# ACEfanatic02/par_raytracer

Hardware: AMD Instinct MI355X
Metric: Mrays/s at 1920x1080x8spp, 1M-tri OBJ (higher is better)
Workload: dtype f32; 1 GPU; C4: synthetic 1,002,528-triangle terrain OBJ (1,024 groups), 1920x1080, 8 spp, bounce_depth 2; seed=1234, triangles=1002528, width=1920, height=1080, spp=8, bounce_depth=2, rays_per_frame=77049910, parallelism=pixel rows sharded in 8-row blocks over 1 GPU(s), pipeline=pool, frames_in_flight=1

## Files before the change

include/prt.h:

```cpp
#ifndef PRT_H_
#define PRT_H_

#include <stddef.h>
#include <stdint.h>

#ifdef __cplusplus
extern "C" {
#endif

#define PRT_ABI_VERSION 5
enum { PRT_ERR_ARGUMENT = -1, PRT_ERR_NO_SCENE = -2, PRT_ERR_HIP = -10, PRT_ERR_IN_FLIGHT = -11, PRT_ERR_EXCEPTION = -12 };


typedef struct prt_material {
    float specular_intensity;
    float index_of_refraction;
    float alpha;
    float ambient_color[4];
    float diffuse_color[4];
    float specular_color[4];
    int32_t ambient_texture;
    int32_t diffuse_texture;
    int32_t specular_texture;
    int32_t alpha_texture;
// ... 180 lines not shown
                                const float * positions, uint32_t position_count, const prt_closest_grads * gout,
                                const prt_point_grads * gin, prt_grad_info * info);
int prt_closest_points_backward_device(prt_ctx * ctx, const prt_point_batch * batch, const int32_t * group, const uint32_t * vertex0,
                                       const float * positions, uint32_t position_count, const prt_closest_grads * gout,
                                       const prt_point_grads * gin, prt_grad_info * info);

typedef struct prt_signed_buffers {
    prt_closest_buffers closest;
    float * signed_dist;
    uint8_t * feature;
} prt_signed_buffers;
int prt_signed_distance(prt_ctx * ctx, const prt_point_batch * batch, const prt_signed_buffers * out, uint32_t flags,
                        prt_counters * counters);
int prt_signed_distance_device(prt_ctx * ctx, const prt_point_batch * batch, const prt_signed_buffers * out, uint32_t flags,
                               prt_counters * counters);

typedef struct prt_sample_request { uint64_t seed; uint64_t first; uint32_t count; } prt_sample_request;
typedef struct prt_sample_buffers {
    float * point;
    float * bw;
    float * normal;
    uint32_t * vertex0;
    int32_t * group;
} prt_sample_buffers;
typedef struct prt_sample_info { double device_ms; double table_ms; double area; uint64_t total_weight;
                                 int32_t unit_exponent; uint32_t live_triangles; } prt_sample_info;
int prt_sample_surface(prt_ctx * ctx, const prt_sample_request * request, const prt_sample_buffers * out, prt_sample_info * info);
int prt_sample_surface_device(prt_ctx * ctx, const prt_sample_request * request, const prt_sample_buffers * out, prt_sample_info * info);

typedef struct prt_sample_grads { const float * point; const float * normal; } prt_sample_grads;
int prt_sample_surface_backward(prt_ctx * ctx, uint32_t count, const int32_t * group, const uint32_t * vertex0, const float * bw,
                                const float * positions, uint32_t position_count, const prt_sample_grads * gout, float * gin_positions,
                                prt_grad_info * info);
int prt_sample_surface_backward_device(prt_ctx * ctx, uint32_t count, const int32_t * group, const uint32_t * vertex0, const float * bw,
                                       const float * positions, uint32_t position_count, const prt_sample_grads * gout, float * gin_positions,
                                       prt_grad_info * info);

typedef struct prt_hemi_batch {
    const float * points;
    const float * normals;
    const float * max_dist;
    uint32_t count;
    uint32_t samples;
    uint64_t seed;
    uint64_t first;
    float ray_bias;
} prt_hemi_batch;
typedef struct prt_hemi_buffers {
    uint32_t * unoccluded;
    float * visibility;
    float * bent;
} prt_hemi_buffers;
int prt_hemisphere_visibility(prt_ctx * ctx, const prt_hemi_batch * batch, const prt_hemi_buffers * out, uint32_t flags,
                              prt_counters * counters);
int prt_hemisphere_visibility_device(prt_ctx * ctx, const prt_hemi_batch * batch, const prt_hemi_buffers * out, uint32_t flags,
                                     prt_counters * counters);

typedef struct prt_multi prt_multi;
prt_multi * prt_multi_create(const int * device_ids, int n_dev);
void prt_multi_destroy(prt_multi * m);
const char * prt_multi_last_error(const prt_multi * m);
int prt_multi_device_count(const prt_multi * m);
int prt_multi_depth(const prt_multi * m);
prt_ctx * prt_multi_context(prt_multi * m, int i);
int prt_multi_upload_scene(prt_multi * m, const prt_scene_desc * scene);
int prt_multi_update_geometry(prt_multi * m, const prt_geometry_update * update);
int prt_multi_render(prt_multi * m, const prt_camera * cam, const prt_params * params, uint32_t width, uint32_t height,
                     float * rgba_out, prt_counters * counters);
int prt_multi_submit(prt_multi * m, const prt_camera * cam, const prt_params * params, uint32_t width, uint32_t height,
                     float * rgba_out, uint64_t * ticket);
int prt_multi_wait(prt_multi * m, uint64_t ticket, prt_counters * counters);

typedef struct prt_scene_info {
    uint32_t triangle_count;
    uint32_t bvh_node_count;
    uint32_t bvh_max_depth;
    uint32_t bvh_node_bytes;
    uint32_t tri_record_bytes;
    uint32_t shade_record_bytes;
    uint64_t device_bytes;
    double bvh_build_ms;
} prt_scene_info;
int prt_get_scene_info(const prt_ctx * ctx, prt_scene_info * info);

typedef struct prt_render_stats {
    uint64_t node_visits, tri_tests;
    uint64_t wave_node_steps, wave_tri_steps, wave_leaf_visits, wave_refills;
    uint64_t deepest_stack;
    uint64_t phase_cycles[5];
    uint64_t parked_rays, parked_shadow_rays;
    uint64_t elided_shadow_rays;
    uint64_t variance_close_calls;
    uint32_t stack_lds_entries, stack_bound;
} prt_render_stats;
int prt_get_render_stats(const prt_ctx * ctx, prt_render_stats * stats);

enum {
    PRT_REGION_ROUND = 0,
    PRT_REGION_TOPUP,
    PRT_REGION_TOPUP_PASS,
    PRT_REGION_TRACE_OUTER,
    PRT_REGION_REFILL,
    PRT_REGION_WALK_PASS,
    PRT_REGION_NODE_STEP,
    PRT_REGION_NODE_DESCEND,
    PRT_REGION_NODE_POP,
    PRT_REGION_NODE_PUSH,
    PRT_REGION_LEAF,
    PRT_REGION_TRI,
    PRT_REGION_FINISH,
    PRT_REGION_PARK,
    PRT_REGION_SHADE_PASS,
    PRT_REGION_SHADE_HIT,
    PRT_REGION_SHADE_MISS,
    PRT_REGION_RADIANCE_STORE,
    PRT_REGION_SHADOW_BLOCK,
    PRT_REGION_SHADOW_EMIT,
    PRT_REGION_WALK_LOOP,
    PRT_REGION_WALK_NEXT_CHILD,
    PRT_REGION_WALK_ENTER,
    PRT_REGION_WALK_RETURN_UP,
    PRT_REGION_FRAME_SAVE,
    PRT_REGION_FRAME_LOAD,
    PRT_REGION_WALK_CHILD_RAY,
    PRT_REGION_OUTPUTS,
    PRT_REGION_WAVE,
    PRT_REGION_LEAF_RAY,
    PRT_REGION_COUNT
};
int prt_get_region_stats(const prt_ctx * ctx, uint64_t * out, uint32_t n);

int prt_debug_check_bvh(const prt_scene_desc * scene, uint64_t * out);
int prt_debug_check_bvh_lbvh(prt_ctx * ctx, const prt_scene_desc * scene, uint64_t * out);
int prt_debug_lbvh_tree(prt_ctx * ctx, uint32_t n_tris, const float * verts9, int32_t * left, int32_t * right, uint32_t * first,
                        uint32_t * last, float * node_box, float * leaf_box, uint32_t * sorted_ids, uint64_t * sorted_keys);
int prt_debug_check_refit(prt_ctx * ctx, const prt_scene_desc * moved_scene, uint64_t * out);

int prt_debug_device_kat(prt_ctx * ctx, int kind, const void * in, size_t in_bytes, void * out, size_t out_bytes,
                         uint32_t n, const prt_camera * cam);

int prt_debug_throw(prt_ctx * ctx, int kind);

#ifdef __cplusplus
}
#endif
#endif
```

par_raytracer_amd/api.py:

```python
from __future__ import annotations

import ctypes as C
from typing import Optional, Sequence, Tuple

import numpy as np

from . import capi
from .capi import PrtCamera, PrtCounters, PrtParams, PrtSceneDesc, PrtGradInfo, PrtSceneInfo, PrtUpdateInfo


class HostScene:

    def __init__(self, directory: str, obj_name: str = "sponza.obj", light_mode: int = 0,
                 camera_position: Sequence[float] = (0.0, 0.0, 0.0)):
        lib = capi.host_lib()
        cp = (C.c_float * 3)(*[float(v) for v in camera_position])
        self._lib = lib
        self._h = lib.prt_host_load_obj(directory.encode(), obj_name.encode(), int(light_mode), cp)
        if not self._h:
            raise RuntimeError("prt_host_load_obj failed: %s" % lib.prt_host_last_error().decode())

    @property
    def handle(self):
        return self._h
# ... 112 lines not shown

        d.positions = ptr("positions", C.c_float); d.position_count = a["positions"].size // 3
        d.normals = ptr("normals", C.c_float); d.normal_count = a["normals"].size // 3
        d.texcoords = ptr("texcoords", C.c_float); d.texcoord_count = a["texcoords"].size // 2
        d.tangents = ptr("tangents", C.c_float)
        d.idx_positions = ptr("idx_positions", C.c_uint32)
        d.idx_texcoords = ptr("idx_texcoords", C.c_uint32)
        d.idx_normals = ptr("idx_normals", C.c_uint32)
        d.index_count = a["idx_positions"].size
        d.groups = ptr("groups", capi.PrtGroup); d.group_count = a["groups"].size // C.sizeof(capi.PrtGroup)
        d.materials = ptr("materials", capi.PrtMaterial); d.material_count = a["materials"].size // C.sizeof(capi.PrtMaterial)
        d.lights = ptr("lights", capi.PrtLight); d.light_count = a["lights"].size // C.sizeof(capi.PrtLight)
        d.spheres = ptr("spheres", capi.PrtBSphere); d.sphere_count = a["spheres"].size // C.sizeof(capi.PrtBSphere)
        d.sphere_group = ptr("sphere_group", C.c_int32)
        dims = a["texture_dims"].reshape(-1, 3)
        self._tex = (capi.PrtTexture * max(1, len(dims)))()
        off = 0
        base = a["texture_bytes"].ctypes.data
        for i, (sx, sy, ch) in enumerate(dims):
            self._tex[i].size_x, self._tex[i].size_y, self._tex[i].channels = int(sx), int(sy), int(ch)
            self._tex[i].texels = C.cast(base + off, C.POINTER(C.c_uint8))
            off += int(sx) * int(sy) * int(ch)
        d.textures = C.cast(self._tex, C.POINTER(capi.PrtTexture)) if len(dims) else C.cast(None, C.POINTER(capi.PrtTexture))
        d.texture_count = len(dims)
        self._desc = d

    @property
    def desc(self):
        return C.pointer(self._desc)


def make_camera(fov: float, width: int, height: int, position: Sequence[float], facing: Sequence[float]) -> PrtCamera:
    cam = PrtCamera()
    p = (C.c_float * 3)(*[float(v) for v in position])
    f = (C.c_float * 3)(*[float(v) for v in facing])
    capi.host_lib().prt_host_make_camera(float(fov), int(width), int(height), p, f, C.byref(cam))
    return cam


def default_params(spp: int, seed: int = 1234, bounce_depth: Optional[int] = None, reflection_samples: Optional[int] = None,
                   spec_samples: Optional[int] = None, pipeline: int = 0, max_spp: int = 0,
                   variance_threshold: float = 0.0) -> PrtParams:
    p = PrtParams()
    capi.host_lib().prt_host_default_params(int(spp), int(seed), C.byref(p))
    if bounce_depth is not None:
        p.bounce_depth = int(bounce_depth)
    if reflection_samples is not None:
        p.reflection_samples = int(reflection_samples)
    if spec_samples is not None:
        p.spec_samples = int(spec_samples)
    p.pipeline = int(pipeline)
    p.max_spp = int(max_spp)
    p.variance_threshold = float(variance_threshold)
    return p


class Renderer:

    def __init__(self, device_id: int = 0):
        lib = capi.hip_lib()
        self._lib = lib
        self._ctx = lib.prt_create(int(device_id))
        if not self._ctx:
            raise RuntimeError("prt_create(%d) failed: %s" % (device_id, lib.prt_last_error(None).decode()))
        self.device_id = device_id

    def _check(self, rc: int, what: str):
        if rc != 0:
            raise RuntimeError("%s failed (%d): %s" % (what, rc, self._lib.prt_last_error(self._ctx).decode()))

    def set_option(self, name: str, value=None) -> None:
        v = None if value is None else str(value).encode()
        self._check(self._lib.prt_set_option(self._ctx, name.encode(), v), "prt_set_option(%s)" % name)

    def upload(self, scene) -> PrtSceneInfo:
        desc = scene.desc if isinstance(scene, (HostScene, FlatDesc)) else scene
        self._check(self._lib.prt_upload_scene(self._ctx, desc), "prt_upload_scene")
        return self.scene_info()

    def scene_info(self) -> PrtSceneInfo:
        info = PrtSceneInfo()
        self._check(self._lib.prt_get_scene_info(self._ctx, C.byref(info)), "prt_get_scene_info")
        return info

    def render_stats(self) -> "capi.PrtRenderStats":
        st = capi.PrtRenderStats()
        self._check(self._lib.prt_get_render_stats(self._ctx, C.byref(st)), "prt_get_render_stats")
        return st

    def region_stats(self) -> dict:
        n = 2 * len(capi.REGION_NAMES)
        out = (C.c_uint64 * n)()
        got = self._lib.prt_get_region_stats(self._ctx, out, n)
        if got != n:
            raise RuntimeError("prt_get_region_stats: the library has %d words, capi.REGION_NAMES %d" % (got, n))
        return {name: (int(out[2 * k]), int(out[2 * k + 1])) for k, name in enumerate(capi.REGION_NAMES)}

    def render(self, cam: PrtCamera, params: PrtParams, width: int, height: int, start_idx: int = 0,
               end_idx: Optional[int] = None) -> Tuple[np.ndarray, PrtCounters]:
        if end_idx is None:
            end_idx = width * height
        out = np.empty((end_idx - start_idx, 4), dtype=np.float32)
        counters = PrtCounters()
        self._check(self._lib.prt_render(self._ctx, C.byref(cam), C.byref(params), width, height, start_idx, end_idx,
                                         out.ctypes.data_as(C.c_void_p), C.byref(counters)), "prt_render")
        return out, counters

    def render_pixels(self, cam: PrtCamera, params: PrtParams, width: int, height: int, pixel_ids) -> Tuple[np.ndarray, PrtCounters]:
        ids = np.ascontiguousarray(pixel_ids, dtype=np.uint32).reshape(-1)
        out = np.empty((ids.size, 4), dtype=np.float32)
        counters = PrtCounters()
        self._check(self._lib.prt_render_pixel_list(self._ctx, C.byref(cam), C.byref(params), width, height,
                                                    ids.ctypes.data_as(C.c_void_p), ids.size,
                                                    out.ctypes.data_as(C.c_void_p), C.byref(counters)), "prt_render_pixel_list")
        return out, counters

    def render_lattice(self, cam, params, width: int, height: int, lattice: int) -> Tuple[np.ndarray, PrtCounters]:
        xs = np.arange(0, width, lattice, dtype=np.uint32)
        ys = np.arange(0, height, lattice, dtype=np.uint32)
        ids = (ys[:, None] * np.uint32(width) + xs[None, :]).reshape(-1)
        out, ctr = self.render_pixels(cam, params, width, height, ids)
        return out.reshape(len(ys), len(xs), 4), ctr

    def render_device(self, cam, params, width, height, start_idx, end_idx, d_ptr: int,
                      want_counters: bool = True) -> Optional[PrtCounters]:
        counters = PrtCounters() if want_counters else None
        self._check(self._lib.prt_render_device(self._ctx, C.byref(cam), C.byref(params), width, height, start_idx,
                                                end_idx, C.c_void_p(d_ptr),
                                                C.byref(counters) if want_counters else None), "prt_render_device")
        return counters

    def shard_rows(self, height: int, block_rows: int, rank: int, nranks: int) -> int:
        return int(self._lib.prt_shard_rows(height, block_rows, rank, nranks))

    def render_shard_device(self, cam, params, width, height, block_rows, rank, nranks, d_ptr: int,
                            want_counters: bool = True) -> Optional[PrtCounters]:
        counters = PrtCounters() if want_counters else None
        self._check(self._lib.prt_render_shard_device(self._ctx, C.byref(cam), C.byref(params), width, height,
                                                      block_rows, rank, nranks, C.c_void_p(d_ptr),
                                                      C.byref(counters) if want_counters else None),
                    "prt_render_shard_device")
        return counters

    def render_shard(self, cam, params, width, height, block_rows, rank, nranks) -> Tuple[np.ndarray, PrtCounters]:
        rows = self.shard_rows(height, block_rows, rank, nranks)
        out = np.empty((rows, width, 4), dtype=np.float32)
        counters = PrtCounters()
        self._check(self._lib.prt_render_shard(self._ctx, C.byref(cam), C.byref(params), width, height, block_rows,
                                               rank, nranks, out.ctypes.data_as(C.c_void_p), C.byref(counters)),
                    "prt_render_shard")
        return out, counters

    def device_kat(self, kind: int, records: np.ndarray, out_shape, out_dtype, cam: Optional[PrtCamera] = None) -> np.ndarray:
        rec = np.ascontiguousarray(records)
        out = np.zeros(out_shape, dtype=out_dtype)
        self._check(self._lib.prt_debug_device_kat(self._ctx, int(kind), rec.ctypes.data_as(C.c_void_p), rec.nbytes,
                                                   out.ctypes.data_as(C.c_void_p), out.nbytes, rec.shape[0],
                                                   C.byref(cam) if cam is not None else None), "prt_debug_device_kat")
        return out

    def _arrays(self, first):
        def fits(got, shape):
            return len(got) == len(shape) and all(s is None or s == g for g, s in zip(got, shape))

        def shown(shape):
            return "(%s)" % ", ".join("n" if s is None else str(s) for s in shape) if None in shape else str(shape)
# ... 352 lines not shown
```

par_raytracer_amd/capi.py:

```python
from __future__ import annotations

import ctypes as C
import os
from typing import Optional

import numpy as np

PKG_DIR = os.path.dirname(os.path.abspath(__file__))
REPO_ROOT = os.path.dirname(PKG_DIR)

c_float3 = C.c_float * 3
c_float4 = C.c_float * 4


class PrtMaterial(C.Structure):
    _fields_ = [("specular_intensity", C.c_float), ("index_of_refraction", C.c_float), ("alpha", C.c_float),
                ("ambient_color", c_float4), ("diffuse_color", c_float4), ("specular_color", c_float4),
                ("ambient_texture", C.c_int32), ("diffuse_texture", C.c_int32), ("specular_texture", C.c_int32),
                ("alpha_texture", C.c_int32), ("bump_texture", C.c_int32)]


class PrtLight(C.Structure):
    _fields_ = [("type", C.c_int32), ("color", c_float4), ("position", c_float3), ("facing", c_float3),
                ("falloff", C.c_float)]


class PrtGroup(C.Structure):
    _fields_ = [("first_index", C.c_uint32), ("index_count", C.c_uint32), ("material", C.c_int32)]


class PrtBSphere(C.Structure):
    _fields_ = [("center", c_float3), ("radius", C.c_float), ("c0", C.c_uint32), ("c1", C.c_uint32)]


class PrtTexture(C.Structure):
    _fields_ = [("size_x", C.c_uint32), ("size_y", C.c_uint32), ("channels", C.c_uint32),
                ("texels", C.POINTER(C.c_uint8))]


class PrtSceneDesc(C.Structure):
    _fields_ = [("positions", C.POINTER(C.c_float)), ("position_count", C.c_uint32),
                ("normals", C.POINTER(C.c_float)), ("normal_count", C.c_uint32),
                ("texcoords", C.POINTER(C.c_float)), ("texcoord_count", C.c_uint32),
                ("tangents", C.POINTER(C.c_float)),
                ("idx_positions", C.POINTER(C.c_uint32)), ("idx_texcoords", C.POINTER(C.c_uint32)),
                ("idx_normals", C.POINTER(C.c_uint32)), ("index_count", C.c_uint32),
                ("groups", C.POINTER(PrtGroup)), ("group_count", C.c_uint32),
                ("materials", C.POINTER(PrtMaterial)), ("material_count", C.c_uint32),
                ("textures", C.POINTER(PrtTexture)), ("texture_count", C.c_uint32),
                ("lights", C.POINTER(PrtLight)), ("light_count", C.c_uint32),
                ("spheres", C.POINTER(PrtBSphere)), ("sphere_group", C.POINTER(C.c_int32)),
                ("sphere_count", C.c_uint32)]


class PrtCamera(C.Structure):
    _fields_ = [("tan_a2", C.c_float), ("aspect", C.c_float), ("inv_width", C.c_float), ("inv_height", C.c_float),
                ("position", c_float3), ("forward", c_float3), ("right", c_float3), ("up", c_float3)]


class PrtParams(C.Structure):
    _fields_ = [("ray_bias", C.c_float), ("reflection_samples", C.c_uint32), ("spec_samples", C.c_uint32),
                ("bounce_depth", C.c_uint32), ("background_color", c_float4), ("spp", C.c_uint32),
                ("pipeline", C.c_uint32), ("seed", C.c_uint64), ("max_spp", C.c_uint32), ("variance_threshold", C.c_float)]


class PrtCounters(C.Structure):
    _fields_ = [("ray_count", C.c_uint64), ("node_visits", C.c_uint64), ("tri_tests", C.c_uint64),
                ("shaded_hits", C.c_uint64), ("render_ms", C.c_double), ("trace_kernel_ms", C.c_double),
                ("trace_kernel_launches", C.c_uint32), ("pipeline", C.c_uint32)]

    def as_dict(self):
        return {n: getattr(self, n) for n, _ in self._fields_}


class PrtSceneInfo(C.Structure):
    _fields_ = [("triangle_count", C.c_uint32), ("bvh_node_count", C.c_uint32), ("bvh_max_depth", C.c_uint32),
                ("bvh_node_bytes", C.c_uint32), ("tri_record_bytes", C.c_uint32), ("shade_record_bytes", C.c_uint32),
                ("device_bytes", C.c_uint64), ("bvh_build_ms", C.c_double)]

    def as_dict(self):
        return {n: getattr(self, n) for n, _ in self._fields_}


class PrtRenderStats(C.Structure):
    _fields_ = [("node_visits", C.c_uint64), ("tri_tests", C.c_uint64), ("wave_node_steps", C.c_uint64),
                ("wave_tri_steps", C.c_uint64), ("wave_leaf_visits", C.c_uint64), ("wave_refills", C.c_uint64),
                ("deepest_stack", C.c_uint64), ("phase_cycles", C.c_uint64 * 5), ("parked_rays", C.c_uint64),
                ("parked_shadow_rays", C.c_uint64), ("elided_shadow_rays", C.c_uint64), ("variance_close_calls", C.c_uint64), ("stack_lds_entries", C.c_uint32), ("stack_bound", C.c_uint32)]


class PrtRayBatch(C.Structure):
    _fields_ = [("origins", C.c_void_p), ("directions", C.c_void_p), ("tmax", C.c_void_p), ("count", C.c_uint32),
                ("ray_bias", C.c_float)]


class PrtHitBuffers(C.Structure):
    _fields_ = [("t", C.c_void_p), ("bw", C.c_void_p), ("vertex0", C.c_void_p), ("group", C.c_void_p),
                ("position", C.c_void_p), ("normal", C.c_void_p), ("occluded", C.c_void_p)]


class PrtPointBatch(C.Structure):
    _fields_ = [("points", C.c_void_p), ("max_dist2", C.c_void_p), ("count", C.c_uint32)]


class PrtClosestBuffers(C.Structure):
    _fields_ = [("dist2", C.c_void_p), ("point", C.c_void_p), ("bw", C.c_void_p), ("vertex0", C.c_void_p), ("group", C.c_void_p)]


class PrtSignedBuffers(C.Structure):
    _fields_ = [("closest", PrtClosestBuffers), ("signed_dist", C.c_void_p), ("feature", C.c_void_p)]


class PrtGeometryUpdate(C.Structure):
    _fields_ = [("positions", C.c_void_p), ("position_count", C.c_uint32), ("normals", C.c_void_p), ("normal_count", C.c_uint32),
                ("tangents", C.c_void_p), ("spheres", C.POINTER(PrtBSphere)), ("sphere_group", C.POINTER(C.c_int32)),
                ("sphere_count", C.c_uint32)]


class PrtUpdateInfo(C.Structure):
    _fields_ = [("device_ms", C.c_double), ("levels", C.c_uint32), ("node_count", C.c_uint32), ("abs_max", C.c_float)]

    def as_dict(self):
        return {n: getattr(self, n) for n, _ in self._fields_}


class PrtHitGrads(C.Structure):
    _fields_ = [("t", C.c_void_p), ("bw", C.c_void_p), ("position", C.c_void_p), ("normal", C.c_void_p)]


class PrtQueryGrads(C.Structure):
    _fields_ = [("positions", C.c_void_p), ("origins", C.c_void_p), ("directions", C.c_void_p)]


class PrtClosestGrads(C.Structure):
    _fields_ = [("dist2", C.c_void_p), ("point", C.c_void_p), ("bw", C.c_void_p)]


class PrtPointGrads(C.Structure):
    _fields_ = [("positions", C.c_void_p), ("points", C.c_void_p)]


class PrtGradInfo(C.Structure):
    _fields_ = [("device_ms", C.c_double), ("hit_rays", C.c_uint32), ("skipped_rays", C.c_uint32), ("unit_exponent", C.c_int32),
                ("max_contribution", C.c_float)]

    def as_dict(self):
        return {n: getattr(self, n) for n, _ in self._fields_}


class PrtSampleRequest(C.Structure):
    _fields_ = [("seed", C.c_uint64), ("first", C.c_uint64), ("count", C.c_uint32)]


class PrtSampleBuffers(C.Structure):
    _fields_ = [("point", C.c_void_p), ("bw", C.c_void_p), ("normal", C.c_void_p), ("vertex0", C.c_void_p), ("group", C.c_void_p)]


class PrtSampleInfo(C.Structure):
    _fields_ = [("device_ms", C.c_double), ("table_ms", C.c_double), ("area", C.c_double), ("total_weight", C.c_uint64),
                ("unit_exponent", C.c_int32), ("live_triangles", C.c_uint32)]

    def as_dict(self):
        return {n: getattr(self, n) for n, _ in self._fields_}


class PrtSampleGrads(C.Structure):
    _fields_ = [("point", C.c_void_p), ("normal", C.c_void_p)]


class PrtHemiBatch(C.Structure):
    _fields_ = [("points", C.c_void_p), ("normals", C.c_void_p), ("max_dist", C.c_void_p), ("count", C.c_uint32), ("samples", C.c_uint32),
                ("seed", C.c_uint64), ("first", C.c_uint64), ("ray_bias", C.c_float)]


class PrtHemiBuffers(C.Structure):
    _fields_ = [("unoccluded", C.c_void_p), ("visibility", C.c_void_p), ("bent", C.c_void_p)]


QUERY_CLOSEST, QUERY_OCCLUDED = 0, 1
PIPELINE_DEFAULT, PIPELINE_MEGAKERNEL, PIPELINE_WAVEFRONT, PIPELINE_PERSISTENT, PIPELINE_POOL = 0, 1, 2, 3, 4
FLAG_COUNT_VISITS = 0x100
FLAG_TRYOUT = 0x200
BUILD_EXPERIMENTAL, BUILD_BVH4 = 1, 2

PRT_SYMBOLS = ["prt_create", "prt_destroy", "prt_last_error", "prt_abi_version", "prt_set_option", "prt_build_flags", "prt_upload_scene", "prt_render",
               "prt_render_device", "prt_shard_rows", "prt_render_shard_device", "prt_render_shard", "prt_render_pixel_list", "prt_get_scene_info", "prt_get_render_stats", "prt_debug_check_bvh", "prt_debug_check_bvh_lbvh", "prt_debug_lbvh_tree", "prt_debug_device_kat",
               "prt_multi_create", "prt_multi_destroy", "prt_multi_last_error", "prt_multi_device_count", "prt_multi_context",
               "prt_multi_upload_scene", "prt_multi_render", "prt_multi_depth", "prt_multi_submit", "prt_multi_wait", "prt_debug_throw",
               "prt_trace_rays", "prt_trace_rays_device", "prt_get_region_stats",
               "prt_update_geometry", "prt_update_geometry_device", "prt_multi_update_geometry", "prt_debug_check_refit",
               "prt_trace_rays_backward", "prt_trace_rays_backward_device",
               "prt_closest_points", "prt_closest_points_device",
               "prt_closest_points_backward", "prt_closest_points_backward_device",
               "prt_signed_distance", "prt_signed_distance_device",
               "prt_sample_surface", "prt_sample_surface_device",
               "prt_sample_surface_backward", "prt_sample_surface_backward_device",
               "prt_hemisphere_visibility", "prt_hemisphere_visibility_device"]
REGION_NAMES = ["round", "topup", "topup_pass", "trace_outer", "refill", "walk_pass", "node_step", "node_descend", "node_pop", "node_push", "leaf",
                "tri", "finish", "park", "shade_pass", "shade_hit", "shade_miss", "radiance_store", "shadow_block", "shadow_emit", "walk_loop",
                "walk_next_child", "walk_enter", "walk_return_up", "frame_save", "frame_load", "walk_child_ray", "outputs", "wave", "leaf_ray"]
PRT_HOST_SYMBOLS = ["prt_host_load_obj", "prt_host_free_scene", "prt_host_scene_desc", "prt_host_scene_hierarchy_seconds",
                    "prt_host_scene_parse_seconds", "prt_host_last_error", "prt_host_make_camera",
                    "prt_host_default_params", "prt_host_render", "prt_host_render_error", "prt_host_write_image", "prt_host_tonemap",
                    "prt_host_load_texture", "prt_host_free_texture", "prt_host_debug_throw"]


class LibraryMissing(RuntimeError):
    pass


def _load(path: str, what: str) -> C.CDLL:
    if not os.path.exists(path):
        raise LibraryMissing("%s not built: %s is missing.  Run `make` (or __graft_entry__.build()) at the repo root; "
                             "there is no fallback implementation." % (what, path))
    return C.CDLL(path, mode=C.RTLD_GLOBAL)


_hip: Optional[C.CDLL] = None
_host: Optional[C.CDLL] = None


def hip_lib() -> C.CDLL:
    global _hip
    if _hip is None:
        lib = _load(os.path.join(PKG_DIR, os.path.basename(os.environ.get("PRT_HIP_LIB", "libprt_hip.so"))), "HIP extension")
        lib.prt_create.restype = C.c_void_p
        lib.prt_create.argtypes = [C.c_int]
        lib.prt_destroy.argtypes = [C.c_void_p]
        lib.prt_last_error.restype = C.c_char_p
        lib.prt_last_error.argtypes = [C.c_void_p]
        lib.prt_abi_version.restype = C.c_int
        lib.prt_build_flags.restype = C.c_int
        lib.prt_set_option.argtypes = [C.c_void_p, C.c_char_p, C.c_char_p]
        lib.prt_upload_scene.argtypes = [C.c_void_p, C.POINTER(PrtSceneDesc)]
        lib.prt_render.argtypes = [C.c_void_p, C.POINTER(PrtCamera), C.POINTER(PrtParams), C.c_uint32, C.c_uint32,
                                   C.c_uint32, C.c_uint32, C.c_void_p, C.POINTER(PrtCounters)]
        lib.prt_render_device.argtypes = [C.c_void_p, C.POINTER(PrtCamera), C.POINTER(PrtParams), C.c_uint32, C.c_uint32,
                                          C.c_uint32, C.c_uint32, C.c_void_p, C.POINTER(PrtCounters)]
        lib.prt_shard_rows.restype = C.c_uint32
        lib.prt_shard_rows.argtypes = [C.c_uint32] * 4
        lib.prt_render_shard_device.argtypes = [C.c_void_p, C.POINTER(PrtCamera), C.POINTER(PrtParams), C.c_uint32,
                                                C.c_uint32, C.c_uint32, C.c_uint32, C.c_uint32, C.c_void_p,
                                                C.POINTER(PrtCounters)]
        lib.prt_render_shard.argtypes = lib.prt_render_shard_device.argtypes
        lib.prt_render_pixel_list.argtypes = [C.c_void_p, C.POINTER(PrtCamera), C.POINTER(PrtParams), C.c_uint32, C.c_uint32,
                                              C.c_void_p, C.c_uint32, C.c_void_p, C.POINTER(PrtCounters)]
        lib.prt_get_scene_info.argtypes = [C.c_void_p, C.POINTER(PrtSceneInfo)]
        lib.prt_get_render_stats.argtypes = [C.c_void_p, C.POINTER(PrtRenderStats)]
        if hasattr(lib, "prt_get_region_stats"):
            lib.prt_get_region_stats.argtypes = [C.c_void_p, C.POINTER(C.c_uint64), C.c_uint32]
        lib.prt_debug_check_bvh.argtypes = [C.POINTER(PrtSceneDesc), C.POINTER(C.c_uint64)]
        lib.prt_debug_check_bvh_lbvh.argtypes = [C.c_void_p, C.POINTER(PrtSceneDesc), C.POINTER(C.c_uint64)]
        if hasattr(lib, "prt_debug_lbvh_tree"):
            lib.prt_debug_lbvh_tree.argtypes = [C.c_void_p, C.c_uint32] + [C.c_void_p] * 9
        lib.prt_debug_device_kat.argtypes = [C.c_void_p, C.c_int, C.c_void_p, C.c_size_t, C.c_void_p, C.c_size_t, C.c_uint32,
                                             C.POINTER(PrtCamera)]
        lib.prt_multi_create.restype = C.c_void_p
        lib.prt_multi_create.argtypes = [C.POINTER(C.c_int), C.c_int]
        lib.prt_multi_destroy.argtypes = [C.c_void_p]
        lib.prt_multi_last_error.restype = C.c_char_p
        lib.prt_multi_last_error.argtypes = [C.c_void_p]
        lib.prt_multi_device_count.argtypes = [C.c_void_p]
        lib.prt_multi_context.restype = C.c_void_p
        lib.prt_multi_context.argtypes = [C.c_void_p, C.c_int]
        lib.prt_multi_upload_scene.argtypes = [C.c_void_p, C.POINTER(PrtSceneDesc)]
        lib.prt_multi_render.argtypes = [C.c_void_p, C.POINTER(PrtCamera), C.POINTER(PrtParams), C.c_uint32, C.c_uint32,
                                         C.c_void_p, C.POINTER(PrtCounters)]
        lib.prt_multi_depth.argtypes = [C.c_void_p]
        lib.prt_multi_submit.argtypes = [C.c_void_p, C.POINTER(PrtCamera), C.POINTER(PrtParams), C.c_uint32, C.c_uint32,
                                         C.c_void_p, C.POINTER(C.c_uint64)]
        lib.prt_multi_wait.argtypes = [C.c_void_p, C.c_uint64, C.POINTER(PrtCounters)]
        lib.prt_debug_throw.argtypes = [C.c_void_p, C.c_int]
        lib.prt_trace_rays.argtypes = [C.c_void_p, C.c_int, C.POINTER(PrtRayBatch), C.POINTER(PrtHitBuffers), C.c_uint32,
                                       C.POINTER(PrtCounters)]
        lib.prt_trace_rays_device.argtypes = lib.prt_trace_rays.argtypes
        if hasattr(lib, "prt_update_geometry"):
            lib.prt_update_geometry.argtypes = [C.c_void_p, C.POINTER(PrtGeometryUpdate), C.POINTER(PrtUpdateInfo)]
            lib.prt_update_geometry_device.argtypes = lib.prt_update_geometry.argtypes
            lib.prt_multi_update_geometry.argtypes = [C.c_void_p, C.POINTER(PrtGeometryUpdate)]
            lib.prt_debug_check_refit.argtypes = [C.c_void_p, C.POINTER(PrtSceneDesc), C.POINTER(C.c_uint64)]
        if hasattr(lib, "prt_trace_rays_backward"):
            lib.prt_trace_rays_backward.argtypes = [C.c_void_p, C.POINTER(PrtRayBatch), C.c_void_p, C.c_void_p, C.c_void_p, C.c_uint32,
                                                    C.POINTER(PrtHitGrads), C.POINTER(PrtQueryGrads), C.POINTER(PrtGradInfo)]
            lib.prt_trace_rays_backward_device.argtypes = lib.prt_trace_rays_backward.argtypes
        if hasattr(lib, "prt_closest_points"):
            lib.prt_closest_points.argtypes = [C.c_void_p, C.POINTER(PrtPointBatch), C.POINTER(PrtClosestBuffers), C.c_uint32,
                                               C.POINTER(PrtCounters)]
            lib.prt_closest_points_device.argtypes = lib.prt_closest_points.argtypes
        if hasattr(lib, "prt_closest_points_backward"):
            lib.prt_closest_points_backward.argtypes = [C.c_void_p, C.POINTER(PrtPointBatch), C.c_void_p, C.c_void_p, C.c_void_p, C.c_uint32,
                                                        C.POINTER(PrtClosestGrads), C.POINTER(PrtPointGrads), C.POINTER(PrtGradInfo)]
            lib.prt_closest_points_backward_device.argtypes = lib.prt_closest_points_backward.argtypes
        if hasattr(lib, "prt_signed_distance"):
            lib.prt_signed_distance.argtypes = [C.c_void_p, C.POINTER(PrtPointBatch), C.POINTER(PrtSignedBuffers), C.c_uint32,
                                                C.POINTER(PrtCounters)]
            lib.prt_signed_distance_device.argtypes = lib.prt_signed_distance.argtypes
        if hasattr(lib, "prt_sample_surface"):
            lib.prt_sample_surface.argtypes = [C.c_void_p, C.POINTER(PrtSampleRequest), C.POINTER(PrtSampleBuffers), C.POINTER(PrtSampleInfo)]
            lib.prt_sample_surface_device.argtypes = lib.prt_sample_surface.argtypes
            lib.prt_sample_surface_backward.argtypes = [C.c_void_p, C.c_uint32, C.c_void_p, C.c_void_p, C.c_void_p, C.c_void_p, C.c_uint32,
                                                        C.POINTER(PrtSampleGrads), C.c_void_p, C.POINTER(PrtGradInfo)]
            lib.prt_sample_surface_backward_device.argtypes = lib.prt_sample_surface_backward.argtypes
        if hasattr(lib, "prt_hemisphere_visibility"):
            lib.prt_hemisphere_visibility.argtypes = [C.c_void_p, C.POINTER(PrtHemiBatch), C.POINTER(PrtHemiBuffers), C.c_uint32,
                                                      C.POINTER(PrtCounters)]
            lib.prt_hemisphere_visibility_device.argtypes = lib.prt_hemisphere_visibility.argtypes
        _hip = lib
    return _hip


def host_lib() -> C.CDLL:
    global _host
    if _host is None:
        hip_lib()
        lib = _load(os.path.join(PKG_DIR, "libprt_host.so"), "host library")
        lib.prt_host_load_obj.restype = C.c_void_p
        lib.prt_host_load_obj.argtypes = [C.c_char_p, C.c_char_p, C.c_int, C.POINTER(C.c_float)]
        lib.prt_host_free_scene.argtypes = [C.c_void_p]
        lib.prt_host_scene_desc.restype = C.POINTER(PrtSceneDesc)
        lib.prt_host_scene_desc.argtypes = [C.c_void_p]
        lib.prt_host_scene_hierarchy_seconds.restype = C.c_double
        lib.prt_host_scene_hierarchy_seconds.argtypes = [C.c_void_p]
        lib.prt_host_scene_parse_seconds.restype = C.c_double
        lib.prt_host_scene_parse_seconds.argtypes = [C.c_void_p]
        lib.prt_host_last_error.restype = C.c_char_p
        lib.prt_host_make_camera.argtypes = [C.c_float, C.c_uint32, C.c_uint32, C.POINTER(C.c_float), C.POINTER(C.c_float),
                                             C.POINTER(PrtCamera)]
        lib.prt_host_default_params.argtypes = [C.c_uint32, C.c_uint64, C.POINTER(PrtParams)]
        lib.prt_host_render.argtypes = [C.c_void_p, C.POINTER(PrtCamera), C.POINTER(PrtParams), C.c_uint32, C.c_uint32,
                                        C.c_int, C.c_void_p, C.POINTER(PrtCounters)]
        lib.prt_host_render_error.restype = C.c_char_p
# ... 17 lines not shown
```

par_raytracer_amd/csrc/bvh_build.cpp:

```cpp
#include "bvh_build.h"
#include "prt_options.h"

#include <algorithm>
#include <atomic>
#include <cfloat>
#include <cmath>
#include <cstdlib>
#include <cstring>
#include <chrono>
#include <cstdio>
#include <stdexcept>
#include <thread>

namespace prt {
namespace {

struct Box {
    float lo[3], hi[3];
    void reset() { for (int a = 0; a < 3; ++a) { lo[a] = FLT_MAX; hi[a] = -FLT_MAX; } }
    void grow(const Box & b) { for (int a = 0; a < 3; ++a) { lo[a] = std::min(lo[a], b.lo[a]); hi[a] = std::max(hi[a], b.hi[a]); } }
    void grow(const float * p) { for (int a = 0; a < 3; ++a) { lo[a] = std::min(lo[a], p[a]); hi[a] = std::max(hi[a], p[a]); } }
    float half_area() const {
        float dx = hi[0] - lo[0], dy = hi[1] - lo[1], dz = hi[2] - lo[2];
        if (dx < 0.0f) return 0.0f;
// ... 406 lines not shown
                } else if (used) {
                    imask |= 1u << s;
                }
                for (int a = 0; a < 3; ++a) {
                    d[8 + 2 * a + (s >> 2)] |= qlo[a] << (8 * (s & 3u));
                    d[14 + 2 * a + (s >> 2)] |= qhi[a] << (8 * (s & 3u));
                }
            } else {
                for (int a = 0; a < 3; ++a) {
                    d[4 + a] |= qlo[a] << (8 * s);
                    d[7 + a] |= qhi[a] << (8 * s);
                }
                if (!used) d[10 + s] = (uint32_t)~(int32_t)(n_tris << 2);
                else if (leaf) d[10 + s] = (uint32_t)~(int32_t)((b.pool[w.kid[s]].first << 2) | (b.pool[w.kid[s]].count - 1));
                else d[10 + s] = next_child++;
            }
        }
        if (eight) {
            d[3] = g.ebyte[0] << 23 | imask | lmask << 8;
            d[4] = w.child_base;
            d[5] = w.tri_base;
            d[6] = g.ebyte[1] << 23 | c0 | c1 << 8;
            d[7] = g.ebyte[2] << 23 | w.axis;
        } else {
            d[3] = g.ebyte[0] << 23;
            d[14] = g.ebyte[1] << 23;
            d[15] = g.ebyte[2] << 23;
        }
    }
    out->node_count = n_nodes;
    out->max_depth = max_depth;
    out->stack_bound = eight ? max_depth + 2 : 3 * max_depth + 2;
    if (b.opt.debug) fprintf(stderr, "[prt] BVH back end (collapse to %d-wide, quantise, reorder): %.1f ms\n", width, std::chrono::duration<double, std::milli>(std::chrono::steady_clock::now() - t0).count());
}

void build_sah_binary(Builder & b, const float * verts, uint32_t n_tris, uint32_t leaf_max, uint32_t threads, float trav_cost,
                      float * scene_lo, float * scene_hi) {
    if (leaf_max < 1) leaf_max = 1;
    if (leaf_max > 4) leaf_max = 4;
    b.leaf_max = leaf_max;
    b.trav_cost = trav_cost;
    b.prims.resize(n_tris);
    Box scene;
    scene.reset();
    for (uint32_t i = 0; i < n_tris; ++i) {
        Prim & p = b.prims[i];
        p.box.reset();
        p.box.grow(verts + 9 * (size_t)i);
        p.box.grow(verts + 9 * (size_t)i + 3);
        p.box.grow(verts + 9 * (size_t)i + 6);
        for (int a = 0; a < 3; ++a) p.c[a] = 0.5f * p.box.lo[a] + 0.5f * p.box.hi[a];
        p.id = i;
        scene.grow(p.box);
    }
    for (int a = 0; a < 3; ++a) { scene_lo[a] = n_tris ? scene.lo[a] : 0.0f; scene_hi[a] = n_tris ? scene.hi[a] : 0.0f; }
    b.pool.resize(n_tris ? 2 * (size_t)n_tris : 1);
    b.next_node = 1;
    b.max_depth = 0;
    b.threads_free = (int)(threads > 1 ? threads - 1 : 0);
    const auto t_build = std::chrono::steady_clock::now();
    if (n_tris) {
        b.build(0, 0, n_tris, 0);
    } else {
        TmpNode & n = b.pool[0];
        n.box.reset();
        for (int a = 0; a < 3; ++a) n.box.lo[a] = n.box.hi[a] = 0.0f;
        n.left = n.right = -1;
        n.first = 0;
        n.count = 1;
        n.depth = 0;
    }
    if (b.opt.debug) fprintf(stderr, "[prt] binned-SAH binary build, %u triangles, %u threads: %.1f ms\n", n_tris, threads, std::chrono::duration<double, std::milli>(std::chrono::steady_clock::now() - t_build).count());
}

}

void build_bvh_wide(int width, const float * verts, uint32_t n_tris, uint32_t leaf_max, uint32_t threads, BvhWide * out, float trav_cost,
                    const BvhBuildOptions * opt) {
    *out = BvhWide();
    Builder b;
    b.configure(opt);
    build_sah_binary(b, verts, n_tris, leaf_max, threads, trav_cost, out->scene_lo, out->scene_hi);
    finish_wide(b, n_tris, width, out);
}

namespace {
void radix_tree_to_binary(Builder & b, uint32_t n_tris, uint32_t leaf_max, const int32_t * left, const int32_t * right,
                          const uint32_t * first, const uint32_t * last, const float * node_box, const float * leaf_box,
                          const uint32_t * sorted_ids, float * scene_lo, float * scene_hi) {
    if (leaf_max < 1) leaf_max = 1;
    if (leaf_max > 4) leaf_max = 4;
    b.leaf_max = leaf_max;
    b.prims.resize(n_tris);
    Box scene;
    scene.reset();
    for (uint32_t i = 0; i < n_tris; ++i) {
        Prim & p = b.prims[i];
        for (int a = 0; a < 3; ++a) { p.box.lo[a] = leaf_box[6 * (size_t)i + a]; p.box.hi[a] = leaf_box[6 * (size_t)i + 3 + a]; p.c[a] = 0.0f; }
        p.id = sorted_ids[i];
        scene.grow(p.box);
    }
    for (int a = 0; a < 3; ++a) { scene_lo[a] = n_tris ? scene.lo[a] : 0.0f; scene_hi[a] = n_tris ? scene.hi[a] : 0.0f; }
    b.pool.resize(n_tris ? 2 * (size_t)n_tris : 1);
    b.next_node = 1;
    b.max_depth = 0;
    b.threads_free = 0;
    auto make_leaf = [&](TmpNode & n, const Box & box, uint32_t f, uint32_t c, uint32_t depth) {
        n.box = box; n.left = n.right = -1; n.first = f; n.count = c; n.depth = depth;
    };
    if (n_tris == 0) {
        Box zero = { { 0, 0, 0 }, { 0, 0, 0 } };
        make_leaf(b.pool[0], zero, 0, 1, 0);
    } else if (n_tris <= leaf_max || n_tris == 1) {
        make_leaf(b.pool[0], scene, 0, n_tris, 0);
    } else if (b.opt.lbvh_plain) {
        struct Todo { uint32_t tmp; int32_t src; uint32_t depth; };
        std::vector<Todo> todo;
        todo.push_back(Todo{ 0u, 0, 0u });
        while (!todo.empty()) {
            const Todo t = todo.back();
            todo.pop_back();
            TmpNode & n = b.pool[t.tmp];
            if (t.src < 0) {
                const uint32_t pos = (uint32_t)~t.src;
                make_leaf(n, b.prims[pos].box, pos, 1, t.depth);
                continue;
            }
            Box box;
            for (int a = 0; a < 3; ++a) { box.lo[a] = node_box[6 * (size_t)t.src + a]; box.hi[a] = node_box[6 * (size_t)t.src + 3 + a]; }
            const uint32_t cnt = last[t.src] - first[t.src] + 1u;
            if (cnt <= leaf_max) { make_leaf(n, box, first[t.src], cnt, t.depth); continue; }
            n.box = box;
            n.depth = t.depth;
            n.first = n.count = 0;
            const uint32_t l = b.alloc(), r = b.alloc();
            n.left = (int32_t)l;
            n.right = (int32_t)r;
            todo.push_back(Todo{ l, left[t.src], t.depth + 1 });
            todo.push_back(Todo{ r, right[t.src], t.depth + 1 });
        }
    } else {
        uint32_t cluster_max = 64;
        if (b.opt.lbvh_cluster >= 0) cluster_max = (uint32_t)std::max(4ll, std::min(1ll << 20, b.opt.lbvh_cluster));
        for (uint32_t i = 0; i < n_tris; ++i)
            for (int a = 0; a < 3; ++a) b.prims[i].c[a] = 0.5f * b.prims[i].box.lo[a] + 0.5f * b.prims[i].box.hi[a];
        struct Cluster { Box box; float c[3]; uint32_t first, count; };
        std::vector<Cluster> clusters;
        {
            std::vector<int32_t> stack;
            stack.push_back(0);
            while (!stack.empty()) {
                const int32_t src = stack.back();
                stack.pop_back();
                Cluster c;
                if (src < 0) {
                    const uint32_t pos = (uint32_t)~src;
                    c.box = b.prims[pos].box; c.first = pos; c.count = 1;
                } else {
                    const uint32_t cnt = last[src] - first[src] + 1u;
                    if (cnt > cluster_max) { stack.push_back(right[src]); stack.push_back(left[src]); continue; }
                    for (int a = 0; a < 3; ++a) { c.box.lo[a] = node_box[6 * (size_t)src + a]; c.box.hi[a] = node_box[6 * (size_t)src + 3 + a]; }
                    c.first = first[src]; c.count = cnt;
                }
                for (int a = 0; a < 3; ++a) c.c[a] = 0.5f * c.box.lo[a] + 0.5f * c.box.hi[a];
                clusters.push_back(c);
            }
// ... 101 lines not shown
```

par_raytracer_amd/csrc/bvh_build.h:

```cpp
#pragma once

#include <cstdint>
#include <vector>

namespace prt { struct BvhBuildOptions; }

namespace prt {

struct BvhWide {
    std::vector<uint32_t> nodes;
    std::vector<uint32_t> tri_order;
    uint32_t node_dwords = 0;
    uint32_t node_count = 0;
    uint32_t max_depth = 0;
    uint32_t stack_bound = 0;
    float scene_lo[3] = { 0, 0, 0 }, scene_hi[3] = { 0, 0, 0 };
};
enum { BVH4_NODE_DWORDS = 16, BVH8_NODE_DWORDS = 20 };

typedef BvhWide Bvh4Result;

typedef BvhWide Bvh8Result;

void build_bvh_wide(int width, const float * verts, uint32_t n_tris, uint32_t leaf_max, uint32_t threads, BvhWide * out,
                    float trav_cost = 1.0f, const BvhBuildOptions * opt = nullptr);

void build_bvh_wide_from_radix_tree(int width, uint32_t n_tris, uint32_t leaf_max, const int32_t * left, const int32_t * right,
                                    const uint32_t * first, const uint32_t * last, const float * node_box, const float * leaf_box,
                                    const uint32_t * sorted_ids, BvhWide * out, const BvhBuildOptions * opt = nullptr);

const char * validate_bvh_links(const BvhWide & bvh, uint32_t n_tris);

void check_bvh_wide(const float * verts, uint32_t n_tris, const BvhWide & bvh, uint64_t * out);

}
```

par_raytracer_amd/csrc/dev_scene.h:

```cpp
#pragma once

#include "../../include/prt.h"
#include "dev_math.h"

namespace prt {

struct DevMaterial {
    float ambient[3];
    float specular_intensity;
    float diffuse[3];
    float index_of_refraction;
    float specular[3];
    float alpha;
    int flags;
    unsigned int tex[3];
};

enum { DEV_TEX_NONE = 0xFFFFu };

struct DevTexture {
    unsigned int first_texel;
    unsigned int size_x, size_y;
    unsigned int pad;
};

struct DevLight {
    float color[3];
    int type;
    float position[3];
    float falloff;
    float facing[3];
    float pad;
};

struct DevScene {
    const float4 * nodes;
    const float4 * tris;
    const float4 * shade;
    const unsigned int * tri_rank;
    const DevMaterial * materials;
    const DevLight * lights;
    const float4 * diffuse_dirs;
    const float4 * spec_dirs;
    unsigned int light_count;
    unsigned int material_count;
    unsigned int spec_samples;
    unsigned int tri_count;
    unsigned int node_count;
    const DevTexture * textures;
    const unsigned int * texels;
    const float * srgb_lut;
    const float4 * tri_uv;
    const float4 * tri_tan;
    const float4 * ref_spheres;
    unsigned int tie_widen_max;
    unsigned long long * near_tie_unresolved;
};

struct DevCamera {
    f3 position;
    f3 forward;
    f3 right_scaled;
    f3 up_scaled;
    float inv_width, inv_height;
};

struct DevParams {
    float ray_bias;
    unsigned int reflection_samples, spec_samples, bounce_depth;
    f3 background;
    unsigned int spp;
    unsigned long long seed;
    unsigned int width, height;
    float box_pad;
    unsigned int first_pixel, shard_block_rows, shard_rank, shard_nranks;
    const unsigned int * pixel_list;
    int * stack_spill;
    unsigned int stack_lds_entries, stack_spill_stride;
    int * exact_stack;
    unsigned int exact_stack_stride;
    unsigned int local_base;
    unsigned int tile_pixels;
    unsigned int work_reverse_n;
    unsigned int work_scatter_n, work_scatter_mul;
    unsigned int elide_dead_shadow_rays;
    unsigned int max_spp;
    float variance_threshold;
};

PRT_HD unsigned int local_of_work(unsigned int wi, unsigned int width, unsigned int tile_pixels, unsigned int reverse_n = 0u,
                                  unsigned int scatter_n = 0u, unsigned int scatter_mul = 1u) {
    if (reverse_n) wi = reverse_n - 1u - wi;
    if (wi >= tile_pixels) return wi;
    if (scatter_n) wi = (((wi >> 3) * scatter_mul) % scatter_n) * 8u + (wi & 7u);
    const unsigned int band_px = 8u * width;
    const unsigned int b = wi / band_px, q = wi - b * band_px;
    const unsigned int t = q >> 6, i = q & 63u;
    return b * band_px + (i >> 3) * width + t * 8u + (i & 7u);
}

PRT_HD unsigned int pixel_of_local(const DevParams & P, unsigned int lp) {
    lp += P.local_base;
    if (P.pixel_list) return P.pixel_list[lp];
    lp = local_of_work(lp, P.width, P.tile_pixels, P.work_reverse_n, P.work_scatter_n, P.work_scatter_mul);
    if (P.shard_nranks <= 1) return P.first_pixel + lp;
    const unsigned int row = lp / P.width, x = lp - row * P.width;
    const unsigned int blk = row / P.shard_block_rows, r = row - blk * P.shard_block_rows;
    const unsigned int y = (blk * P.shard_nranks + P.shard_rank) * P.shard_block_rows + r;
    return y * P.width + x;
}

struct DevCounters {
    unsigned long long ray_count;
    unsigned long long node_visits;
    unsigned long long tri_tests;
    unsigned long long shaded_hits;
// ... 48 lines not shown
```

par_raytracer_amd/csrc/dev_trace.h:

```cpp
#pragma once

#if defined(PRT_BVH8)
#include "dev_trace8.h"
#else
#include "dev_trace4.h"
#endif

namespace prt {

template <bool ANY_LENGTH, class STK>
PRT_D void trav_start(TravRay & r, f3 o, f3 d, int kind, float pad, const STK & stk) {
    if (ANY_LENGTH) {
        f3 w = (o + d) - o;
        if (w.x == 0.0f && w.y == 0.0f && w.z == 0.0f) w = d;
        float m = fmaxf(fmaxf(fabsf(w.x), fabsf(w.y)), fabsf(w.z));
        if (m < 9.5367431640625e-7f) {
            const int k = -ilogbf(m);
            w = mk3(ldexpf(w.x, k), ldexpf(w.y, k), ldexpf(w.z, k));
            m = ldexpf(m, k);
        }
        const float tiny = m * 9.094947017729282e-13f;
        if (fabsf(w.x) < tiny) w.x = copysignf(tiny, w.x);
        if (fabsf(w.y) < tiny) w.y = copysignf(tiny, w.y);
        if (fabsf(w.z) < tiny) w.z = copysignf(tiny, w.z);
        trav_init(r, o, w, kind, pad, stk);
        r.d = d;
        return;
    }
    trav_init(r, o, d, kind, pad, stk);
}

template <class STK, bool COUNT, bool ANY_LENGTH = false>
PRT_D HitRec resolve_near_ties(const DevScene & sc, f3 o, f3 d, float pad, float min_t, const STK & stk, TraceStats & st) {
    TravRay r;
    HitRec result = hit_miss();
    const f3 qp = o - (o + d);
    float bound = min_t * PRT_TIE_NEAR;
    for (unsigned int widen = 0; ; ++widen) {
        const bool last = widen >= sc.tie_widen_max;
        const float moat = bound * 1.00000095367431640625f;
        bool occupied = false;
        float best = 3.402823466e+38f;
        result.tri = -1;
        unsigned int next_rank = 0;
        RefSphereWalk walk;
        walk.reset();
        for (;;) {
            unsigned int c_rank = 0xFFFFFFFFu;
            int c_tri = -1;
            trav_start<ANY_LENGTH>(r, o, d, TRACE_CLOSEST, pad, stk);
            r.best.t = moat;
            for (;;) {
                while (trav_walking(r)) trav_node_step<STK, COUNT>(sc, r, stk, st, pad);
                if (trav_done(r)) break;
                unsigned int first, count;
                trav_leaf_range(r, first, count);
                for (unsigned int i = 0; i < count; ++i) {
                    const unsigned int ti = first + i;
                    const float4 * tp = sc.tris + 3 * (size_t)ti;
                    const float4 r0 = tp[0], r1 = tp[1], r2 = tp[2];
                    float t, dd, v, w;
                    if (!tri_geom(o, qp, mk3(r0.x, r0.y, r0.z), mk3(r0.w, r1.x, r1.y), mk3(r1.z, r1.w, r2.x), mk3(r2.y, r2.z, r2.w), t, dd, v, w)) continue;
                    const float th = t * (1.0f / dd);
                    if (th > bound) { if (th <= moat) occupied = true; continue; }
                    const unsigned int rk = sc.tri_rank[ti];
                    if (rk >= next_rank && rk < c_rank) { c_rank = rk; c_tri = (int)ti; }
                }
                trav_leaf_next(r, stk);
            }
            if (c_tri < 0 || (occupied && !last)) break;
            const float4 * tp = sc.tris + 3 * (size_t)c_tri;
            const float4 r0 = tp[0], r1 = tp[1], r2 = tp[2];
            float t, v, w;
            if (walk.offers(sc, o, d, c_rank, best) &&
                tri_test_ref(o, qp, mk3(r0.x, r0.y, r0.z), mk3(r0.w, r1.x, r1.y), mk3(r1.z, r1.w, r2.x), mk3(r2.y, r2.z, r2.w), best, t, v, w)) {
                best = t;
                result.t = t; result.v = v; result.w = w; result.tri = c_tri;
            }
            next_rank = c_rank + 1u;
        }
        if (!occupied) break;
        if (last) {
            if (sc.near_tie_unresolved) atomicAdd(sc.near_tie_unresolved, 1ull);
            break;
        }
        bound = moat * PRT_TIE_NEAR;
    }
    return result;
}

template <class STK, bool COUNT, bool ANY_LENGTH = false>
PRT_D HitRec trace_ray(const DevScene & sc, f3 o, f3 d, int kind, float pad, const STK & stk, TraceStats & st) {
    TravRay r;
    trav_start<ANY_LENGTH>(r, o, d, kind, pad, stk);
    for (;;) {
        while (trav_walking(r)) trav_node_step<STK, COUNT>(sc, r, stk, st, pad);
        if (trav_done(r)) break;
        if (trav_leaf<STK, COUNT>(sc, r, stk, st)) return r.best;
    }
    if (trav_wants_resolve(r, stk)) return resolve_near_ties<STK, COUNT, ANY_LENGTH>(sc, o, d, pad, r.best.t, stk, st);
    return r.best;
}

PRT_D bool ray_overflows(float scene_max, f3 o, f3 d) {
    const float D = fmaxf(fmaxf(fabsf(d.x), fabsf(d.y)), fabsf(d.z)), O = fmaxf(fmaxf(fabsf(o.x), fabsf(o.y)), fabsf(o.z));
    const float s = fmaxf(scene_max, 1.17549435e-38f);
    const int es = ilogbf(s) + 1, eo = ilogbf(fmaxf(O, s)) + 2;
    const int ed = ilogbf(fmaxf(fmaxf(D, O * 1.1920929e-7f), 1.17549435e-38f)) + 2;
    const int top = (ed > eo ? ed : eo) + 2 * es + 5, mixed = ed + eo + es + 4;
    return (top > mixed ? top : mixed) >= 127;
}

template <bool COUNT>
PRT_D HitRec scan_closest(const DevScene & sc, const unsigned int * slot_of_rank, f3 o, f3 d, TraceStats & st) {
    const f3 qp = o - (o + d);
    HitRec h = hit_miss();
    RefSphereWalk walk;
    walk.reset();
    for (unsigned int rank = 0; rank < sc.tri_count; ++rank) {
        if (!walk.offers(sc, o, d, rank, h.t)) {
            if (walk.skip_until > rank) rank = walk.skip_until - 1u;
            continue;
        }
        const unsigned int ti = slot_of_rank[rank];
        const float4 * tp = sc.tris + 3 * (size_t)ti;
        const float4 r0 = tp[0], r1 = tp[1], r2 = tp[2];
        float t, v, w;
        if (COUNT) st.tris++;
        if (tri_test_ref(o, qp, mk3(r0.x, r0.y, r0.z), mk3(r0.w, r1.x, r1.y), mk3(r1.z, r1.w, r2.x), mk3(r2.y, r2.z, r2.w), h.t, t, v, w)) {
            h.t = t; h.v = v; h.w = w; h.tri = (int)ti;
        }
    }
    return h;
}

template <bool COUNT>
PRT_D HitRec scan_any_below(const DevScene & sc, f3 o, f3 d, float tmax, TraceStats & st) {
    const f3 qp = o - (o + d);
    HitRec h = hit_miss();
    for (unsigned int ti = 0; ti < sc.tri_count; ++ti) {
        const float4 * tp = sc.tris + 3 * (size_t)ti;
        const float4 r0 = tp[0], r1 = tp[1], r2 = tp[2];
        float t, dd, v, w;
        if (COUNT) st.tris++;
        if (!tri_geom(o, qp, mk3(r0.x, r0.y, r0.z), mk3(r0.w, r1.x, r1.y), mk3(r1.z, r1.w, r2.x), mk3(r2.y, r2.z, r2.w), t, dd, v, w)) continue;
        if (t > 3.402823466e+38f * dd) continue;
        const float th = t * (1.0f / dd);
        if (th < tmax) { h.t = th; h.tri = (int)ti; return h; }
    }
    return h;
}

template <class STK, bool COUNT>
PRT_D HitRec query_any_below(const DevScene & sc, f3 o, f3 d, float tmax, float pad, const STK & stk, TraceStats & st) {
    TravRay r;
    trav_start<true>(r, o, d, TRACE_ANY, pad, stk);
    r.best.t = tmax;
    for (;;) {
        while (trav_walking(r)) trav_node_step<STK, COUNT>(sc, r, stk, st, pad);
        if (trav_done(r)) break;
        if (trav_leaf<STK, COUNT>(sc, r, stk, st)) break;
    }
    return r.best;
}

template <class STK, bool COUNT>
PRT_D HitRec query_any_unculled(const DevScene & sc, f3 o, f3 d, float tmax, float pad, const STK & stk, TraceStats & st) {
    TravRay r;
    trav_start<true>(r, o, d, TRACE_ANY, pad, stk);
    r.best.t = __uint_as_float(0x7F800000u);
    const f3 qp = o - (o + d);
    HitRec h = hit_miss();
    for (;;) {
        while (trav_walking(r)) trav_node_step<STK, COUNT>(sc, r, stk, st, pad);
        if (trav_done(r)) break;
        unsigned int first, count;
        trav_leaf_range(r, first, count);
// ... 17 lines not shown
```

par_raytracer_amd/csrc/dev_trace4.h:

```cpp
#pragma once

#include "dev_trace_common.h"

namespace prt {

struct TravRay {
    f3 o, d;
    float ix, iy, iz;
    float pnx, pny, pnz;
    HitRec best;
    int node, sp, kind;
};


enum { TRAV_SENTINEL = (int)0x80000000, TRAV_FLAG_NEAR = 1, TRAV_FLAG_OVERFLOW = 2, TRAV_SENTINEL_LAST = (int)0x80000003 };
PRT_D bool trav_done(int node) { return node <= TRAV_SENTINEL_LAST; }

typedef int StackEntry;
enum { STACK_ENTRY_INTS = 1, BVH_NODE_BYTES = 64, STACK_LDS_CAP_DEFAULT = 24 };

template <int BLOCK>
struct LdsStack {
    int * col;
    unsigned int cap;
    PRT_D void attach(int * lds, unsigned int tid) { col = lds + tid; }
    PRT_D int * frame_col() const { return col; }
    PRT_D bool push(int sp, int v) const {
        if ((unsigned int)sp < cap) { col[sp * BLOCK] = v; return true; }
        return false;
    }
    PRT_D int pop(int sp) const { return col[sp * BLOCK]; }
    PRT_D void flag(int bit) const { col[0] |= bit; }
};

template <int BLOCK>
struct LdsSpillStack {
    int * col;
    unsigned int cap;
    PRT_D void attach(int * lds, unsigned int tid) { col = lds + tid; }
    PRT_D int * frame_col() const { return col; }
    PRT_D void set_spill(int * base, unsigned int lanes) { spill = base; spill_stride = lanes; }
    int * spill;
    unsigned int spill_stride;
    PRT_D size_t spill_index(int sp) const {
        return (size_t)((unsigned int)sp - cap) * spill_stride + (blockIdx.x * (unsigned int)BLOCK + threadIdx.x);
    }
    PRT_D bool push(int sp, int v) const {
        if ((unsigned int)sp < cap) col[sp * BLOCK] = v;
        else spill[spill_index(sp)] = v;
        return true;
    }
    PRT_D int pop(int sp) const {
        if ((unsigned int)sp < cap) return col[sp * BLOCK];
        return spill[spill_index(sp)];
    }
    PRT_D void flag(int bit) const { col[0] |= bit; }
};

struct GlobalStack {
    int * col;
    size_t stride;
    PRT_D void attach(int * base, size_t lane, size_t lanes) { col = base + lane; stride = lanes; }
    PRT_D bool push(int sp, int v) const { col[(size_t)sp * stride] = v; return true; }
    PRT_D int pop(int sp) const { return col[(size_t)sp * stride]; }
    PRT_D void flag(int bit) const { col[0] |= bit; }
};

PRT_D void trav_idle(TravRay & r) { r.node = TRAV_SENTINEL; r.sp = 0; r.kind = 0; }
PRT_D bool trav_walking(const TravRay & r) { return r.node >= 0; }
PRT_D bool trav_done(const TravRay & r) { return trav_done(r.node); }

template <class STK> PRT_D int trav_end_flags(const TravRay & r, const STK &) { return trav_done(r.node) ? (r.node & 3) : 0; }
template <class STK> PRT_D bool trav_wants_resolve(const TravRay & r, const STK & stk) { return r.kind == TRACE_CLOSEST && (trav_end_flags(r, stk) & TRAV_FLAG_NEAR) != 0 && r.best.tri >= 0; }
template <class STK> PRT_D bool trav_needs_slow_path(const TravRay & r, const STK & stk) { return (trav_end_flags(r, stk) & TRAV_FLAG_OVERFLOW) != 0 || trav_wants_resolve(r, stk); }

template <class STK>
PRT_D void trav_pop(TravRay & r, const STK & stk) {
    r.sp--;
    r.node = stk.pop(r.sp);
}
PRT_D void trav_leaf_range(const TravRay & r, unsigned int & first, unsigned int & count) {
    const unsigned int leaf = (unsigned int)~r.node;
    first = leaf >> 2;
    count = (leaf & 3u) + 1u;
}
template <class STK> PRT_D void trav_leaf_next(TravRay & r, const STK & stk) { trav_pop(r, stk); }
template <class STK>
PRT_D void trav_push(TravRay & r, const STK & stk, int link) {
    if (stk.push(r.sp, link)) r.sp++;
    else stk.flag(TRAV_FLAG_OVERFLOW);
}

template <class STK>
PRT_D void trav_init(TravRay & r, f3 o, f3 d, int kind, float pad, const STK & stk) {
    r.o = o;
    r.d = d;
    const float tiny = 1e-30f;
    float dx = fabsf(d.x) < tiny ? (d.x < 0.0f ? -tiny : tiny) : d.x;
    float dy = fabsf(d.y) < tiny ? (d.y < 0.0f ? -tiny : tiny) : d.y;
    float dz = fabsf(d.z) < tiny ? (d.z < 0.0f ? -tiny : tiny) : d.z;
    r.ix = 1.0f / dx; r.iy = 1.0f / dy; r.iz = 1.0f / dz;
    r.pnx = (dx < 0.0f ? o.x - pad : o.x + pad) * r.ix;
    r.pny = (dy < 0.0f ? o.y - pad : o.y + pad) * r.iy;
    r.pnz = (dz < 0.0f ? o.z - pad : o.z + pad) * r.iz;
    r.best = hit_miss();
    r.kind = kind;
    stk.push(0, TRAV_SENTINEL);
    r.sp = 1;
    r.node = 0;
}

PRT_D void cswap(float & ka, float & kb, int & la, int & lb) {
    const bool sw = kb < ka;
    const float k0 = sw ? kb : ka, k1 = sw ? ka : kb;
    const int l0 = sw ? lb : la, l1 = sw ? la : lb;
    ka = k0; kb = k1; la = l0; lb = l1;
}

template <class STK, bool COUNT>
PRT_D void trav_node_step(const DevScene & sc, TravRay & r, const STK & stk, TraceStats & st, float pad) {
    const uint4 * np = reinterpret_cast<const uint4 *>(reinterpret_cast<const char *>(sc.nodes) + ((unsigned int)r.node << 6));
    const uint4 w0 = np[0], w1 = np[1], w2 = np[2], w3 = np[3];
    if (COUNT) { st.nodes++; if (first_active_lane()) st.wnodes++; if ((unsigned int)r.sp > st.max_sp) st.max_sp = (unsigned int)r.sp; }
    const float kx = __uint_as_float(w0.w) * r.ix;
    const float ky = __uint_as_float(w3.z) * r.iy;
    const float kz = __uint_as_float(w3.w) * r.iz;
    const float ox = __uint_as_float(w0.x), oy = __uint_as_float(w0.y), oz = __uint_as_float(w0.z);
    const float pad2 = pad + pad;
    const float cnx = __builtin_fmaf(ox, r.ix, -r.pnx), cfx = __builtin_fmaf(pad2, fabsf(r.ix), cnx);
    const float cny = __builtin_fmaf(oy, r.iy, -r.pny), cfy = __builtin_fmaf(pad2, fabsf(r.iy), cny);
    const float cnz = __builtin_fmaf(oz, r.iz, -r.pnz), cfz = __builtin_fmaf(pad2, fabsf(r.iz), cnz);
    const bool sx = r.ix < 0.0f, sy = r.iy < 0.0f, sz = r.iz < 0.0f;
    const unsigned int qnx = sx ? w1.w : w1.x, qfx = sx ? w1.x : w1.w;
    const unsigned int qny = sy ? w2.x : w1.y, qfy = sy ? w1.y : w2.x;
    const unsigned int qnz = sz ? w2.y : w1.z, qfz = sz ? w1.z : w2.y;
    float key[4];
    int link[4] = { (int)w2.z, (int)w2.w, (int)w3.x, (int)w3.y };
    const float inf = __uint_as_float(0x7F800000u);
#pragma unroll
    for (int k = 0; k < 4; ++k) {
        const float nx = __builtin_fmaf((float)((qnx >> (8 * k)) & 0xFFu), kx, cnx);
        const float fx = __builtin_fmaf((float)((qfx >> (8 * k)) & 0xFFu), kx, cfx);
        const float ny = __builtin_fmaf((float)((qny >> (8 * k)) & 0xFFu), ky, cny);
        const float fy = __builtin_fmaf((float)((qfy >> (8 * k)) & 0xFFu), ky, cfy);
        const float nz = __builtin_fmaf((float)((qnz >> (8 * k)) & 0xFFu), kz, cnz);
        const float fz = __builtin_fmaf((float)((qfz >> (8 * k)) & 0xFFu), kz, cfz);
        const float tmin = fmaxf(fmaxf(fmaxf(nx, ny), nz), 0.0f);
        const float tmax = fminf(fminf(fminf(fx, fy), fz), r.best.t);
        key[k] = tmin <= tmax ? tmin : inf;
    }
    cswap(key[0], key[1], link[0], link[1]);
    cswap(key[2], key[3], link[2], link[3]);
    cswap(key[0], key[2], link[0], link[2]);
    cswap(key[1], key[3], link[1], link[3]);
    cswap(key[1], key[2], link[1], link[2]);
    if (key[0] < inf) {
        if (COUNT && first_active_lane()) st.wdescend++;
        if (COUNT) {
            const unsigned long long p3 = __ballot(key[3] < inf), p2 = __ballot(key[2] < inf), p1 = __ballot(key[1] < inf);
            if (first_active_lane()) st.wpush += (unsigned int)(p3 != 0ull) + (unsigned int)(p2 != 0ull) + (unsigned int)(p1 != 0ull);
        }
        if (key[3] < inf) trav_push(r, stk, link[3]);
        if (key[2] < inf) trav_push(r, stk, link[2]);
        if (key[1] < inf) trav_push(r, stk, link[1]);
        r.node = link[0];
    } else {
        if (COUNT && r.best.tri >= 0) st.culled++;
        if (COUNT && first_active_lane()) st.wpop++;
        trav_pop(r, stk);
    }
}

template <class STK, bool COUNT>
PRT_D bool trav_leaf(const DevScene & sc, TravRay & r, const STK & stk, TraceStats & st) {
    const f3 qp = r.o - (r.o + r.d);
    const unsigned int leaf = (unsigned int)~r.node;
    const unsigned int first = leaf >> 2, count = (leaf & 3u) + 1u;
    if (COUNT) { if (first_active_lane()) st.wleaves++; }
    int next_node = stk.pop(r.sp - 1);
    bool flagged = false;
    for (unsigned int i = 0; i < count; ++i) {
        const unsigned int ti = first + i;
        const float4 * tp = reinterpret_cast<const float4 *>(reinterpret_cast<const char *>(sc.tris) + ti * 48u);
        const float4 r0 = tp[0], r1 = tp[1], r2 = tp[2];
#if defined(__HIP_DEVICE_COMPILE__)
        asm volatile("" :: "v"(r0.x), "v"(r0.y), "v"(r0.z));
#endif
        if (COUNT) { st.tris++; if (first_active_lane()) st.wtris++; }
        float t, v, w;
        bool near;
        const bool hit = tri_test(r.o, r.d, qp, mk3(r0.x, r0.y, r0.z), mk3(r0.w, r1.x, r1.y), mk3(r1.z, r1.w, r2.x),
                                  mk3(r2.y, r2.z, r2.w), r.best.t, t, v, w, near);
// ... 20 lines not shown
```

par_raytracer_amd/csrc/dev_trace8.h:

```cpp
#pragma once

#include "dev_trace_common.h"

namespace prt {

typedef int2 StackEntry;
enum { STACK_ENTRY_INTS = 2, BVH_NODE_BYTES = 80, STACK_LDS_CAP_DEFAULT = 13 };

struct TravRay {
    f3 o, d;
    float ix, iy, iz;
    float pnx, pny, pnz;
    HitRec best;
    int node;
    unsigned int tbase;
    unsigned int tbits;
    int sp, kind;
};

enum { TRAV_SENTINEL = (int)0x80000000, TRAV_FLAG_NEAR = 1, TRAV_FLAG_OVERFLOW = 2, TRAV_SENTINEL_LAST = (int)0x80000003 };

template <int BLOCK>
struct LdsStack {
    int * col;
    unsigned int cap;
    PRT_D void attach(int * lds, unsigned int tid) { col = lds + tid; }
    PRT_D int * frame_col() const { return col; }
    PRT_D bool put(int sp, int2 v) const {
        if ((unsigned int)sp < cap) { col[(2 * sp) * BLOCK] = v.x; col[(2 * sp + 1) * BLOCK] = v.y; return true; }
        return false;
    }
    PRT_D int2 get(int sp) const { return make_int2(col[(2 * sp) * BLOCK], col[(2 * sp + 1) * BLOCK]); }
    PRT_D void flag(int bit) const { col[0] |= bit; }
    PRT_D int marker() const { return col[0]; }
};

template <int BLOCK>
struct LdsSpillStack {
    int * col;
    unsigned int cap;
    int2 * spill;
    unsigned int spill_stride;
    PRT_D void attach(int * lds, unsigned int tid) { col = lds + tid; }
    PRT_D int * frame_col() const { return col; }
    PRT_D void set_spill(int * base, unsigned int lanes) { spill = reinterpret_cast<int2 *>(base); spill_stride = lanes; }
    PRT_D size_t spill_index(int sp) const {
        return (size_t)((unsigned int)sp - cap) * spill_stride + (blockIdx.x * (unsigned int)BLOCK + threadIdx.x);
    }
    PRT_D bool put(int sp, int2 v) const {
        if ((unsigned int)sp < cap) { col[(2 * sp) * BLOCK] = v.x; col[(2 * sp + 1) * BLOCK] = v.y; }
        else spill[spill_index(sp)] = v;
        return true;
    }
    PRT_D int2 get(int sp) const {
        if ((unsigned int)sp < cap) return make_int2(col[(2 * sp) * BLOCK], col[(2 * sp + 1) * BLOCK]);
        return spill[spill_index(sp)];
    }
    PRT_D void flag(int bit) const { col[0] |= bit; }
    PRT_D int marker() const { return col[0]; }
};

struct GlobalStack {
    int2 * col;
    size_t stride;
    PRT_D void attach(int * base, size_t lane, size_t lanes) { col = reinterpret_cast<int2 *>(base) + lane; stride = lanes; }
    PRT_D bool put(int sp, int2 v) const { col[(size_t)sp * stride] = v; return true; }
    PRT_D int2 get(int sp) const { return col[(size_t)sp * stride]; }
    PRT_D void flag(int bit) const { col[0].x |= bit; }
    PRT_D int marker() const { return col[0].x; }
};

PRT_D void trav_idle(TravRay & r) { r.node = TRAV_SENTINEL; r.tbits = 0u; r.tbase = 0u; r.sp = 0; r.kind = 0; }
PRT_D bool trav_walking(const TravRay & r) { return (r.tbits & 0xFFu) == 0u && r.node >= 0; }
PRT_D bool trav_done(const TravRay & r) { return (r.tbits & 0xFFu) == 0u && r.node < 0; }

template <class STK> PRT_D int trav_end_flags(const TravRay & r, const STK & stk) {
    return ((r.kind & TRACE_ANY) && r.best.tri >= 0) ? 0 : (stk.marker() & 3);
}
template <class STK> PRT_D bool trav_wants_resolve(const TravRay & r, const STK & stk) {
    return !(r.kind & TRACE_ANY) && r.best.tri >= 0 && (stk.marker() & TRAV_FLAG_NEAR) != 0;
}
template <class STK> PRT_D bool trav_needs_slow_path(const TravRay & r, const STK & stk) {
    const int f = trav_end_flags(r, stk);
    return (f & TRAV_FLAG_OVERFLOW) != 0 || (!(r.kind & TRACE_ANY) && r.best.tri >= 0 && (f & TRAV_FLAG_NEAR) != 0);
}

template <class STK>
PRT_D void trav_init(TravRay & r, f3 o, f3 d, int kind, float pad, const STK & stk) {
    r.o = o;
    r.d = d;
    const float tiny = 1e-30f;
    float dx = fabsf(d.x) < tiny ? (d.x < 0.0f ? -tiny : tiny) : d.x;
    float dy = fabsf(d.y) < tiny ? (d.y < 0.0f ? -tiny : tiny) : d.y;
    float dz = fabsf(d.z) < tiny ? (d.z < 0.0f ? -tiny : tiny) : d.z;
    r.ix = 1.0f / dx; r.iy = 1.0f / dy; r.iz = 1.0f / dz;
    r.pnx = (dx < 0.0f ? o.x - pad : o.x + pad) * r.ix;
    r.pny = (dy < 0.0f ? o.y - pad : o.y + pad) * r.iy;
    r.pnz = (dz < 0.0f ? o.z - pad : o.z + pad) * r.iz;
    r.best = hit_miss();
    const int oct = (dx < 0.0f ? 1 : 0) | (dy < 0.0f ? 2 : 0) | (dz < 0.0f ? 4 : 0);
    r.kind = kind | oct << 4;
    stk.put(0, make_int2(TRAV_SENTINEL, 0));
    r.sp = 1;
    r.node = 0;
    r.tbase = 0u;
    r.tbits = 0u;
}

template <class STK, bool COUNT>
PRT_D void trav_node_step(const DevScene & sc, TravRay & r, const STK & stk, TraceStats & st, float pad) {
    const uint4 * np = reinterpret_cast<const uint4 *>(reinterpret_cast<const char *>(sc.nodes) + (unsigned int)r.node * (unsigned int)BVH_NODE_BYTES);
    const uint4 q0 = np[0], q1 = np[1], q2 = np[2], q3 = np[3], q4 = np[4];
    if (COUNT) { st.nodes++; if (first_active_lane()) st.wnodes++; if ((unsigned int)r.sp > st.max_sp) st.max_sp = (unsigned int)r.sp; }
    const float kx = __uint_as_float(q0.w & 0x7F800000u) * r.ix;
    const float ky = __uint_as_float(q1.z & 0x7F800000u) * r.iy;
    const float kz = __uint_as_float(q1.w & 0x7F800000u) * r.iz;
    const float pad2 = pad + pad;
    const float cnx = __builtin_fmaf(__uint_as_float(q0.x), r.ix, -r.pnx), cfx = __builtin_fmaf(pad2, fabsf(r.ix), cnx);
    const float cny = __builtin_fmaf(__uint_as_float(q0.y), r.iy, -r.pny), cfy = __builtin_fmaf(pad2, fabsf(r.iy), cny);
    const float cnz = __builtin_fmaf(__uint_as_float(q0.z), r.iz, -r.pnz), cfz = __builtin_fmaf(pad2, fabsf(r.iz), cnz);
    const bool sx = r.ix < 0.0f, sy = r.iy < 0.0f, sz = r.iz < 0.0f;
    const unsigned int qnx[2] = { sx ? q3.z : q2.x, sx ? q3.w : q2.y }, qfx[2] = { sx ? q2.x : q3.z, sx ? q2.y : q3.w };
    const unsigned int qny[2] = { sy ? q4.x : q2.z, sy ? q4.y : q2.w }, qfy[2] = { sy ? q2.z : q4.x, sy ? q2.w : q4.y };
    const unsigned int qnz[2] = { sz ? q4.z : q3.x, sz ? q4.w : q3.y }, qfz[2] = { sz ? q3.x : q4.z, sz ? q3.y : q4.w };
    unsigned int m = 0u;
#pragma unroll
    for (int j = 7; j >= 0; --j) {
        const int h = j >> 2, k = j & 3;
        const float nx = __builtin_fmaf((float)((qnx[h] >> (8 * k)) & 0xFFu), kx, cnx);
        const float fx = __builtin_fmaf((float)((qfx[h] >> (8 * k)) & 0xFFu), kx, cfx);
        const float ny = __builtin_fmaf((float)((qny[h] >> (8 * k)) & 0xFFu), ky, cny);
        const float fy = __builtin_fmaf((float)((qfy[h] >> (8 * k)) & 0xFFu), ky, cfy);
        const float nz = __builtin_fmaf((float)((qnz[h] >> (8 * k)) & 0xFFu), kz, cnz);
        const float fz = __builtin_fmaf((float)((qfz[h] >> (8 * k)) & 0xFFu), kz, cfz);
        const float tmin = fmaxf(fmaxf(fmaxf(nx, ny), nz), 0.0f);
        const float tmax = fminf(fminf(fminf(fx, fy), fz), r.best.t);
#if defined(__HIP_DEVICE_COMPILE__)
        asm("v_cmp_le_f32 vcc, %1, %2\n\tv_addc_co_u32 %0, vcc, %0, %0, vcc" : "+v"(m) : "v"(tmin), "v"(tmax) : "vcc");
#else
        m = (m << 1) | (tmin <= tmax ? 1u : 0u);
#endif
    }
    const unsigned int imask = q0.w & 0xFFu;
    r.tbase = q1.y;
    r.tbits = (m & ~imask) | (q0.w & 0xFF00u) | (q1.z << 16);
    const unsigned int mi = m & imask;
    unsigned int gbase = q1.x, gbits = imask | mi << 8 | (q1.w & 3u) << 16;
    int at = r.sp;
    if (COUNT) {
        const unsigned long long down = __ballot(mi != 0u), all = __ballot(true);
        if (first_active_lane()) { st.wdescend += down != 0ull; st.wpop += down != all; }
    }
    if (mi == 0u) {
        if (COUNT && r.best.tri >= 0 && (m & ~imask) == 0u) st.culled++;
        at = r.sp - 1;
        const int2 e = stk.get(at);
        if (e.x <= TRAV_SENTINEL_LAST) {
            r.node = TRAV_SENTINEL;
            r.sp = at;
            return;
        }
        gbase = (unsigned int)e.x;
        gbits = (unsigned int)e.y;
    }
    const unsigned int rest8 = (gbits >> 8) & 0xFFu;
    const bool backwards = (((unsigned int)r.kind >> 4) >> ((gbits >> 16) & 3u)) & 1u;
    const unsigned int s = backwards ? 31u - (unsigned int)__clz((int)rest8) : (unsigned int)(__ffs((int)rest8) - 1);
    r.node = (int)(gbase + (unsigned int)__popc(gbits & ((1u << s) - 1u) & 0xFFu));
    gbits &= ~(0x100u << s);
    if (COUNT) {
        const unsigned long long pushing = __ballot(((gbits >> 8) & 0xFFu) != 0u);
        if (first_active_lane()) st.wpush += pushing != 0ull;
    }
    if ((gbits >> 8) & 0xFFu) {
        if (stk.put(at, make_int2((int)gbase, (int)gbits))) r.sp = at + 1;
        else { stk.flag(TRAV_FLAG_OVERFLOW); r.sp = at; }
    } else {
        r.sp = at;
    }
}

PRT_D void trav_leaf_range(const TravRay & r, unsigned int & first, unsigned int & count) {
    const unsigned int s = (unsigned int)(__ffs((int)(r.tbits & 0xFFu)) - 1);
    const unsigned int below = (1u << s) - 1u;
    const unsigned int ones = (unsigned int)__popc(r.tbits & (below << 8 | below << 16));
    const unsigned int twos = (unsigned int)__popc(r.tbits & (below << 24));
    first = r.tbase + ones + 2u * twos;
// ... 39 lines not shown
```

par_raytracer_amd/csrc/kernels_pool.h:

```cpp
#pragma once

#include "kernels_wave.h"

namespace prt {

struct PoolBuffers {
    float4 * cq;
    float4 * hits;
    float4 * sq;
    unsigned int * head;
    unsigned int cap, scap;
    unsigned int topup_min;
    unsigned int topup_max;
    float4 * park;
    float4 * spark;
    unsigned int * park_count;
    unsigned int park_cap, spark_cap;
    unsigned int adopt;
    unsigned int lcap;
    unsigned int * fin;
    float4 * scratch;
    float4 * jobsum;
    float4 * final_rgb;
    unsigned long long * wave_times;
// ... 299 lines not shown
                if (cnt <= want) fetch_done = true; else cnt = want;
                const DevCamera cam = A.cam;
                region_count<COUNT>(rg, PRT_REGION_TOPUP);
                for (unsigned int k = ulane; k < cnt; k += ULANES) {
                    region_count<COUNT>(rg, PRT_REGION_TOPUP_PASS);
                    const unsigned int sid = base + k;
                    const unsigned int gsid = B.sample_base + sid;
                    SampleState S;
                    Frame fr;
                    u64 * ring = RING && RINGMEM != 0 ? B.ring + (size_t)sid * B.ring_step : nullptr;
                    if (ADAPT) {
                        sample_begin<RING>(cam, P, pixel_of_local(P, gsid), 0u, S, fr, ring, B.ring_stride);
                        Q.jobsum[sid] = make_float4(0.0f, 0.0f, 0.0f, as_f(0));
                    } else {
                        sample_begin<RING>(cam, P, pixel_of_local(P, gsid / P.spp), gsid % P.spp, S, fr, ring, B.ring_stride);
                    }
                    B.rng[sid] = make_ulonglong2(S.rng.chain, S.rng.prev);
                    if (RING && RINGMEM != 0) B.rng_aux[sid] = make_ulonglong2(S.rng.seed0, (u64)S.rng.k);
                    co[n_c + k] = make_float4(fr.ray_o.x, fr.ray_o.y, fr.ray_o.z, as_f((int)sid));
                    cd[n_c + k] = make_float4(fr.ray_d.x, fr.ray_d.y, fr.ray_d.z, as_f((int)WF_PENDING_FRESH_BIT << 8));
                    ct[n_c + k] = make_float4(1.0f, 1.0f, 1.0f, 0.0f);
                }
                n_c += cnt;
            }
            }
          }
        }
        if (COUNT && fetch_done && wt_dry == 0ull) wt_dry = wall_clock64();
        const unsigned int total = n_c + n_s;
        if (total == 0u && n_f == 0u) {
            if (fetch_done) break;
            continue;
        }
        pool_sync<SHARED>();
        if (lead_wave) rays += total;
        const unsigned long long ph_t1 = COUNT ? __builtin_readcyclecounter() : 0ull;

        {
            const PoolArgs A = pool_args(args);
            const DevScene & sc = A.sc;
            const DevParams & P = A.P;
            const WaveBuffers & B = A.B;
            const int keep_min = A.keep_min, node_min = A.node_min, node_frac = A.node_frac;
            PRT_POOL_LISTS(A);
            const DevLight * lights = sc.light_count <= (unsigned int)LDS_LIGHTS ? s_lights : sc.lights;
            TravRay r;
            trav_idle(r);
            int ray = -1;
            float4 payload = make_float4(0, 0, 0, 0);
            int sample = 0;
            unsigned int next = 0;
            bool dry = total == 0u;
            for (;;) {
                region_count<COUNT>(rg, PRT_REGION_TRACE_OUTER);
                const unsigned long long idle = __ballot(ray < 0);
                if (idle != 0ull && !dry) {
                    if (COUNT && lane == 0) st.wrefills++;
                    const unsigned int prefix = __builtin_amdgcn_mbcnt_hi((unsigned int)(idle >> 32), __builtin_amdgcn_mbcnt_lo((unsigned int)idle, 0u));
                    const unsigned int n_idle = (unsigned int)__popcll(idle);
                    if (SHARED) {
                        unsigned int b = 0;
                        if (lane == 0) b = atomicAdd(&s_ctl[PCTL_TRACE_NEXT], n_idle);
                        next = (unsigned int)__builtin_amdgcn_readfirstlane((int)b);
                        if (next > total) next = total;
                    }
                    const unsigned int avail = total - next;
                    const unsigned int take = n_idle < avail ? n_idle : avail;
                    if (ray < 0 && prefix < take) {
                        region_count<COUNT>(rg, PRT_REGION_REFILL);
                        const unsigned int idx = next + prefix;
                        float4 ro, rd;
                        int kind;
                        if (idx < n_c) {
                            ro = co[idx];
                            rd = cd[idx];
                            kind = WF_KIND_CLOSEST;
                        } else {
                            const unsigned int j = idx - n_c;
                            ro = sq_o[j];
                            payload = sq_c[j];
                            if (payload.w < 0.0f) {
                                const DevLight & L = lights[(unsigned int)(-payload.w) - 1u];
                                const f3 lv = mk3(L.facing[0], L.facing[1], L.facing[2]) * -1.0f;
                                rd = make_float4(lv.x, lv.y, lv.z, 0.0f);
                                kind = WF_KIND_SHADOW_ANY;
                            } else {
                                rd = sq_d[j];
                                kind = WF_KIND_SHADOW_DIST;
                            }
                        }
                        sample = as_i(ro.w);
                        const f3 d = mk3(rd.x, rd.y, rd.z);
                        const f3 ob = mk3(ro.x, ro.y, ro.z) + d * P.ray_bias;
                        trav_init(r, ob, d, kind == WF_KIND_SHADOW_ANY ? TRACE_ANY : TRACE_CLOSEST, P.box_pad, stack);
                        ray = (int)idx;
                    }
                    next += take;
                    dry = next == total;
                }
                const int leave_below = dry ? 1 : keep_min;
                if (__ballot(ray >= 0) == 0ull) break;

                while (ray >= 0) {
                    region_count<COUNT>(rg, PRT_REGION_WALK_PASS);
                    const int walkers = __popcll(__ballot(trav_walking(r)));
                    const int wfrac = (walkers * node_frac) >> 3;
                    const int nmin = node_min < wfrac ? node_min : wfrac;
                    const unsigned int with_ray = COUNT ? (unsigned int)__popcll(__ballot(true)) : 0u;
                    while (trav_walking(r)) {
                        trav_node_step<Stack, COUNT>(sc, r, stack, st, P.box_pad);
                        if (COUNT && first_active_lane()) { st.wrays += with_ray; if (dry) { dry_steps += 1ull; dry_rays += with_ray; } }
                        if (__popcll(__ballot(trav_walking(r))) < nmin) break;
                    }
                    bool fin = trav_done(r);
                    if (!fin && !trav_walking(r)) fin = trav_leaf<Stack, COUNT>(sc, r, stack, st);
                    if (fin) {
                        region_count<COUNT>(rg, PRT_REGION_FINISH);
                        if (EXACT && trav_wants_resolve(r, stack)) r.best = resolve_near_ties<Stack, COUNT>(sc, r.o, r.d, P.box_pad, r.best.t, stack, st);
                        if (!EXACT && trav_needs_slow_path(r, stack)) {
                            region_count<COUNT>(rg, PRT_REGION_PARK);
                            if (ADAPT && (unsigned int)ray < n_c && ((unsigned int)as_i(cd[ray].w) >> 8 & POOL_SPEC_PENDING_BIT)) {
                                hits[ray] = make_float4(0.0f, 0.0f, 0.0f, as_f(POOL_CANCELLED_MARK));
                            } else if ((unsigned int)ray < n_c) {
                                const unsigned int slot = atomicAdd(A.Q.park_count, 1u);
                                if (slot < A.Q.park_cap) {
                                    const float4 t4 = ct[ray];
                                    A.Q.park[slot] = co[ray];
                                    A.Q.park[(size_t)A.Q.park_cap + slot] = cd[ray];
                                    A.Q.park[2u * (size_t)A.Q.park_cap + slot] = make_float4(t4.x, t4.y, t4.z, as_f(POOL_PARK_CLOSEST));
                                }
                                hits[ray] = make_float4(0.0f, 0.0f, 0.0f, as_f(POOL_PARKED_MARK));
                            } else {
                                const unsigned int slot = atomicAdd(A.Q.park_count + 1, 1u);
                                if (slot < A.Q.spark_cap) {
                                    A.Q.spark[slot] = sq_o[(unsigned int)ray - n_c];
                                    A.Q.spark[(size_t)A.Q.spark_cap + slot] = payload;
                                    A.Q.spark[2u * (size_t)A.Q.spark_cap + slot] = make_float4(r.d.x, r.d.y, r.d.z, 0.0f);
                                }
                                if (ADAPT) {
                                    float * const w = &A.Q.jobsum[sample].w;
                                    *w = as_f(as_i(*w) | (int)0x80000000);
                                }
                            }
                        } else if ((unsigned int)ray < n_c) {
                            hits[ray] = make_float4(r.best.t, r.best.v, r.best.w, as_f(r.best.tri));
                        } else {
                            const bool lit = r.best.tri < 0 || (payload.w >= 0.0f && r.best.t * r.best.t <= payload.w);
                            if (lit) {
                                accum_add(B.accum + sample, mk3(payload.x, payload.y, payload.z));
                            }
                        }
                        ray = -1;
                        break;
                    }
                    if (__popcll(__ballot(true)) < leave_below) break;
                }
            }
        }
        pool_sync<SHARED>();
        const unsigned long long ph_t2 = COUNT ? __builtin_readcyclecounter() : 0ull;

        {
            const PoolArgs A = pool_args(args);
            const DevScene & sc = A.sc;
            const DevParams & P = A.P;
            const WaveBuffers & B = A.B;
            const PoolBuffers & Q = A.Q;
            PRT_POOL_LISTS(A);
            unsigned int * const fin = ADAPT ? Q.fin + (size_t)wave * cap : nullptr;
            ShadeTables tb;
            tb.diffuse = LDSTAB ? s_diffuse : sc.diffuse_dirs;
            tb.materials = sc.material_count <= (unsigned int)LDS_MATS ? s_mats : sc.materials;
            tb.lights = sc.light_count <= (unsigned int)LDS_LIGHTS ? s_lights : sc.lights;
            const int nxt = cur ^ 1;
            PoolEmit<ADAPT, SHARED, COUNT, FORKS, FORKS ? BLOCK : 0> emit;
            emit.may_fork = false; emit.col = stack.frame_col(); emit.m_l = 0;
            emit.rg = rg;
// ... 240 lines not shown
                if (ADAPT) n_spec = emit.s_cnt[3];
                if (FORKS) {
                    n_l = emit.s_cnt[3];
                    if (threadIdx.x == 0) s_ctl[PCTL_FORK_RES] = 0u;
                }
            } else {
                n_c = emit.m_c;
                n_s = emit.m_s;
                n_f = emit.m_f;
                if (FORKS) n_l = emit.m_l;
            }
            cur = nxt;
        }
        if (!SHARED) pool_fence();
        if (COUNT) {
            const unsigned long long ph_t3 = __builtin_readcyclecounter();
            ph_topup += ph_t1 - ph_t0; ph_trace += ph_t2 - ph_t1; ph_shade += ph_t3 - ph_t2;
        }
    }

    if (lane == 0) {
        atomicAdd(&s_red[0], rays);
        atomicAdd(&s_red[1], (unsigned long long)shaded_w);
        if (elided_w) atomicAdd(&ctr->elided_shadow_rays, (unsigned long long)elided_w);
    }
    __syncthreads();
    if (threadIdx.x == 0) {
        if (s_red[0]) atomicAdd(&ctr->ray_count, s_red[0]);
        if (s_red[1]) atomicAdd(&ctr->shaded_hits, s_red[1]);
    }
    if (COUNT) {
        trace_stats_flush<true>(ctr, st);
        atomicAdd(&ctr->culled, (unsigned long long)st.culled);
        atomicAdd(&ctr->wave_node_step_rays, (unsigned long long)st.wrays);
        atomicAdd(&ctr->region[2 * PRT_REGION_NODE_DESCEND], (unsigned long long)st.wdescend);
        atomicAdd(&ctr->region[2 * PRT_REGION_NODE_POP], (unsigned long long)st.wpop);
        atomicAdd(&ctr->region[2 * PRT_REGION_NODE_PUSH], (unsigned long long)st.wpush);
        for (unsigned int k = threadIdx.x; k < 2u * PRT_REGION_COUNT; k += BLOCK) if (s_rg[k]) atomicAdd(&ctr->region[k], (unsigned long long)s_rg[k]);
        if (dry_steps) { atomicAdd(&ctr->drain_node_steps, dry_steps); atomicAdd(&ctr->drain_node_step_rays, dry_rays); }
        if (lane == 0) {
            atomicAdd(&ctr->phase_cycles[0], ph_topup);
            atomicAdd(&ctr->phase_cycles[1], ph_trace);
            atomicAdd(&ctr->phase_cycles[2], ph_shade);
            const unsigned long long ph_all = __builtin_readcyclecounter() - ph_begin;
            atomicAdd(&ctr->phase_cycles[3], ph_all);
            if (!EXACT) {
                unsigned long long * const wt = ((PoolArgsPtr)args)->Q.wave_times;
                if (wt) {
                    unsigned long long * const w3 = as_global(wt) + 3u * (size_t)(slot_id >> 6);
                    w3[0] = wt_begin; w3[1] = wt_dry; w3[2] = wall_clock64();
                }
                atomicMax(&ctr->wave_cycles_max, ph_all);
                atomicAdd(&ctr->wave_cycles_sum, ph_all);
                atomicAdd(&ctr->wave_count, 1ull);
            }
            if (ADAPT) atomicAdd(&ctr->phase_cycles[4], ph_final);
        }
    }
}

#undef PRT_POOL_LISTS

template <bool COUNT>
__global__ __launch_bounds__(256) void k_pool_parked_shadows(const PoolArgs * args, DevCounters * ctr) {
    const PoolArgs A = pool_args(args);
    const DevScene & sc = A.sc;
    const DevParams & P = A.P;
    const unsigned int gid = blockIdx.x * blockDim.x + threadIdx.x;
    const unsigned int n = A.Q.park_count[1] < A.Q.spark_cap ? A.Q.park_count[1] : A.Q.spark_cap;
    if (gid == 0) {
        atomicMax(&ctr->park_peak[0], (unsigned long long)A.Q.park_count[0]);
        atomicMax(&ctr->park_peak[1], (unsigned long long)A.Q.park_count[1]);
        if (A.Q.park_count[0] > A.Q.park_cap) atomicMax(&ctr->park_over[0], (unsigned long long)A.Q.park_count[0]);
        if (A.Q.park_count[1] > A.Q.spark_cap) atomicMax(&ctr->park_over[1], (unsigned long long)A.Q.park_count[1]);
    }
    TraceStats st;
    GlobalStack slow;
    slow.attach(P.exact_stack, gid, P.exact_stack_stride);
    for (unsigned int i = gid; i < n; i += gridDim.x * blockDim.x) {
        const float4 ro = A.Q.spark[i], pay = A.Q.spark[(size_t)A.Q.spark_cap + i], rd = A.Q.spark[2u * (size_t)A.Q.spark_cap + i];
        const int sample = as_i(ro.w);
        const f3 d = mk3(rd.x, rd.y, rd.z);
        const f3 ob = mk3(ro.x, ro.y, ro.z) + d * P.ray_bias;
        const HitRec h = trace_ray<GlobalStack, COUNT>(sc, ob, d, pay.w < 0.0f ? TRACE_ANY : TRACE_CLOSEST, P.box_pad, slow, st);
        if (shadow_lit(h, pay.w)) accum_add(A.B.accum + sample, mk3(pay.x, pay.y, pay.z));
    }
    if (COUNT) trace_stats_flush<false>(ctr, st);
}

}
```

par_raytracer_amd/csrc/kernels_wave.h:

```cpp
#pragma once

#include "../../include/prt_key.h"
#include "dev_shade.h"
#include "dev_texture.h"
#include "dev_wave_loop.h"

namespace prt {

enum { WF_KIND_CLOSEST = 0, WF_KIND_SHADOW_ANY = 1, WF_KIND_SHADOW_DIST = 2 };
enum { WF_STAGE_REFL = 0, WF_STAGE_SPEC = 1, WF_STAGE_ALPHA = 2, WF_STAGE_DONE = 3 };
enum { WF_PENDING_FRESH_BIT = 0x400000 };
enum { WF_PENDING_LEAF_BIT = 0x200000 };

struct WaveBuffers {
    Accum * accum;
    ulonglong2 * rng;
    ulonglong2 * rng_aux;
    u64 * ring;
    unsigned int ring_step, ring_stride;
    float4 * frames;
    float4 * rq_o[2];
    float4 * rq_d[2];
    float4 * rq_t[2];
    float4 * hits;
    float4 * sq_o;
    float4 * sq_c;
    float4 * sq_d;
    unsigned int * counts;
    unsigned int * overflow;
    unsigned int n_samples;
    unsigned int sample_base;
};

PRT_D unsigned int wave_append(unsigned int * counter, bool pred) {
    const unsigned long long mask = __ballot(pred);
    if (mask == 0ull) return 0u;
    const unsigned int n = (unsigned int)__popcll(mask);
    const unsigned int prefix = __builtin_amdgcn_mbcnt_hi((unsigned int)(mask >> 32), __builtin_amdgcn_mbcnt_lo((unsigned int)mask, 0u));
    const int leader = __ffsll((long long)mask) - 1;
    unsigned int base = 0;
    if ((int)lane_id() == leader) base = atomicAdd(counter, n);
    base = (unsigned int)__shfl((int)base, leader);
    return base + prefix;
}

template <int NW>
PRT_D unsigned int block_append(unsigned int * counter, bool pred, unsigned int * s_cnt ) {
    const unsigned long long mask = __ballot(pred);
    const unsigned int n = (unsigned int)__popcll(mask);
    const unsigned int prefix = __builtin_amdgcn_mbcnt_hi((unsigned int)(mask >> 32), __builtin_amdgcn_mbcnt_lo((unsigned int)mask, 0u));
    const unsigned int wave = threadIdx.x >> 6;
    if (lane_id() == 0) s_cnt[wave] = n;
    __syncthreads();
    if (threadIdx.x == 0) {
        unsigned int total = 0;
        for (int w = 0; w < NW; ++w) { const unsigned int c = s_cnt[w]; s_cnt[w] = total; total += c; }
        s_cnt[NW] = total ? atomicAdd(counter, total) : 0u;
    }
    __syncthreads();
    const unsigned int slot = s_cnt[NW] + s_cnt[wave] + prefix;
    __syncthreads();
    return slot;
}

PRT_D float4 shadow_entry_dir(const DevLight * lights, float4 payload, const float4 * sq_d, unsigned int j, int & kind) {
    if (payload.w < 0.0f) {
        const DevLight & L = lights[(unsigned int)(-payload.w) - 1u];
        const f3 lv = mk3(L.facing[0], L.facing[1], L.facing[2]) * -1.0f;
        kind = WF_KIND_SHADOW_ANY;
        return make_float4(lv.x, lv.y, lv.z, 0.0f);
    }
    kind = WF_KIND_SHADOW_DIST;
    return sq_d[j];
}
PRT_D bool shadow_lit(const HitRec & h, float w) { return h.tri < 0 || (w >= 0.0f && h.t * h.t <= w); }

template <bool RING>
__global__ __launch_bounds__(256) void k_raygen(DevCamera cam, DevParams P, WaveBuffers B) {
    const unsigned int sid = blockIdx.x * blockDim.x + threadIdx.x;
    if (sid >= B.n_samples) return;
    const unsigned int gsid = B.sample_base + sid;
    const unsigned int pixel = pixel_of_local(P, gsid / P.spp);
    const unsigned int samp = gsid % P.spp;
    SampleState S;
    Frame cur;
    u64 * ring = RING ? B.ring + (size_t)sid * B.ring_step : nullptr;
    sample_begin<RING>(cam, P, pixel, samp, S, cur, ring, B.ring_stride);
    B.rng[sid] = make_ulonglong2(S.rng.chain, S.rng.prev);
    if (RING) B.rng_aux[sid] = make_ulonglong2(S.rng.seed0, (u64)S.rng.k);
    B.rq_o[0][sid] = make_float4(cur.ray_o.x, cur.ray_o.y, cur.ray_o.z, as_f((int)sid));
    B.rq_d[0][sid] = make_float4(cur.ray_d.x, cur.ray_d.y, cur.ray_d.z, as_f((int)WF_PENDING_FRESH_BIT << 8));
    B.rq_t[0][sid] = make_float4(1.0f, 1.0f, 1.0f, 0.0f);
}

struct TraceEntry {
    f3 ob, d;
    int kind, sample;
};
PRT_D TraceEntry trace_entry(const DevScene & sc, const DevParams & P, const WaveBuffers & B, int cur, unsigned int n_closest,
                             unsigned int idx, float4 & payload) {
    float4 ro, rd;
    TraceEntry e;
    if (idx < n_closest) {
        ro = B.rq_o[cur][idx];
        rd = B.rq_d[cur][idx];
        e.kind = WF_KIND_CLOSEST;
    } else {
        const unsigned int j = idx - n_closest;
        ro = B.sq_o[j];
        payload = B.sq_c[j];
        rd = shadow_entry_dir(sc.lights, payload, B.sq_d, j, e.kind);
    }
    e.sample = as_i(ro.w);
    e.d = mk3(rd.x, rd.y, rd.z);
    e.ob = mk3(ro.x, ro.y, ro.z) + e.d * P.ray_bias;
    return e;
}
PRT_D int trace_entry_mode(const TraceEntry & e) { return e.kind == WF_KIND_SHADOW_ANY ? TRACE_ANY : TRACE_CLOSEST; }
PRT_D void trace_entry_emit(const WaveBuffers & B, unsigned int n_closest, unsigned int idx, const HitRec & best, float4 payload, int sample) {
    if (idx < n_closest) B.hits[idx] = make_float4(best.t, best.v, best.w, as_f(best.tri));
    else if (shadow_lit(best, payload.w)) accum_add(B.accum + sample, mk3(payload.x, payload.y, payload.z));
}

template <int BLOCK, bool COUNT>
struct TraceJob : RaySteps<BLOCK, COUNT> {
    const DevParams & P;
    const WaveBuffers & B;
    int cur;
    unsigned int n_closest;
    float4 payload;
    int sample;
    PRT_D bool start(unsigned int idx, TravRay & r, const LdsStack<BLOCK> & stack) {
        const TraceEntry e = trace_entry(this->sc, P, B, cur, n_closest, idx, payload);
        sample = e.sample;
        trav_init(r, e.ob, e.d, trace_entry_mode(e), this->pad, stack);
        return true;
    }
    PRT_D void finish(unsigned int idx, const TravRay & r, const LdsStack<BLOCK> & stack) const {
        if (trav_needs_slow_path(r, stack)) B.overflow[atomicAdd(B.counts + 3, 1u)] = idx;
        else trace_entry_emit(B, n_closest, idx, r.best, payload, sample);
    }
};

template <int BLOCK, bool COUNT>
__global__ __launch_bounds__(BLOCK, 6) void k_trace(DevScene sc, DevParams P, WaveBuffers B, int cur, unsigned int n_closest,
                                                  unsigned int n_shadow, int keep_min, int node_min, unsigned int chunk, int multi_light,
                                                  DevCounters * ctr) {
    extern __shared__ int s_stack[];
    LdsStack<BLOCK> stack;
    stack.attach(s_stack, threadIdx.x);
    stack.cap = P.stack_lds_entries;
    TraceStats st;
    TraceJob<BLOCK, COUNT> job = { { sc, P.box_pad }, P, B, cur, n_closest, make_float4(0, 0, 0, 0), 0 };
    wave_loop<BLOCK, COUNT>(job, stack, st, B.counts + 2, n_closest + n_shadow, keep_min, node_min, chunk);
    if (COUNT) {
        trace_stats_flush<true>(ctr, st);
        atomicAdd(&ctr->culled, (unsigned long long)st.culled);
    }
}

template <bool COUNT>
__global__ __launch_bounds__(256) void k_trace_exact(DevScene sc, DevParams P, WaveBuffers B, int cur, unsigned int n_closest,
                                                         int multi_light, DevCounters * ctr) {
    exact_list_walk<COUNT>(B.overflow, B.counts[3], P.exact_stack, P.exact_stack_stride, ctr, [&](unsigned int idx, const GlobalStack & slow, TraceStats & st) {
        float4 payload = make_float4(0, 0, 0, 0);
        const TraceEntry e = trace_entry(sc, P, B, cur, n_closest, idx, payload);
        const HitRec best = trace_ray<GlobalStack, COUNT>(sc, e.ob, e.d, trace_entry_mode(e), P.box_pad, slow, st);
        trace_entry_emit(B, n_closest, idx, best, payload, e.sample);
    });
}

struct WFrame {
    f3 hit_p, hit_n, ray_d, T_in, hit_pos, kd, ks;
    float alpha, w_diffuse;
    int mat, stage, idx;
};

template <int STRIDE>
struct LdsF {
    int * p;
    PRT_D operator float() const { return as_f(*p); }
    PRT_D LdsF & operator=(float v) { *p = as_i(v); return *this; }
    PRT_D LdsF & operator=(const LdsF & o) { *p = *o.p; return *this; }
};
template <int STRIDE>
struct LdsI {
    int * p;
    PRT_D operator int() const { return *p; }
    PRT_D LdsI & operator=(int v) { *p = v; return *this; }
    PRT_D LdsI & operator=(const LdsI & o) { *p = *o.p; return *this; }
    PRT_D int operator++(int) { const int v = *p; *p = v + 1; return v; }
};
template <int STRIDE>
struct LdsF3 {
    int * p;
    PRT_D operator f3() const { return mk3(as_f(p[0]), as_f(p[STRIDE]), as_f(p[2 * STRIDE])); }
    PRT_D LdsF3 & operator=(f3 v) { p[0] = as_i(v.x); p[STRIDE] = as_i(v.y); p[2 * STRIDE] = as_i(v.z); return *this; }
    PRT_D LdsF3 & operator=(const LdsF3 & o) { return *this = (f3)o; }
};
struct NoF3 {
    PRT_D NoF3 & operator=(f3) { return *this; }
    PRT_D operator f3() const { return mk3(0.0f, 0.0f, 0.0f); }
};
template <int STRIDE, bool POS> struct WFramePos { LdsF3<STRIDE> hit_pos; PRT_D void place(int * col) { hit_pos.p = col + 23 * STRIDE; } };
template <int STRIDE> struct WFramePos<STRIDE, false> { NoF3 hit_pos; PRT_D void place(int *) {} };
template <int STRIDE, bool POS>
struct WFrameLds : WFramePos<STRIDE, POS> {
    LdsF3<STRIDE> hit_p, hit_n, ray_d, T_in, kd, ks;
    LdsF<STRIDE> alpha, w_diffuse;
    LdsI<STRIDE> mat, stage, idx;
    PRT_D explicit WFrameLds(int * col) {
        hit_p.p = col; hit_n.p = col + 3 * STRIDE; ray_d.p = col + 6 * STRIDE; T_in.p = col + 9 * STRIDE;
        kd.p = col + 12 * STRIDE; ks.p = col + 15 * STRIDE;
        alpha.p = col + 18 * STRIDE; w_diffuse.p = col + 19 * STRIDE;
        mat.p = col + 20 * STRIDE; stage.p = col + 21 * STRIDE; idx.p = col + 22 * STRIDE;
        this->place(col);
    }
};
enum { WFRAME_LDS_DWORDS = 26, WFRAME_LDS_DWORDS_NOPOS = 23 };
enum { WFL_HIT_P = 0, WFL_HIT_N = 3, WFL_RAY_D = 6, WFL_T_IN = 9, WFL_KD = 12, WFL_KS = 15, WFL_W_DIFFUSE = 19, WFL_MAT = 20 };
enum { WF_FORK_GROUP = 6 };

template <bool POS, bool TEX, class FrameT>
PRT_D void wframe_save(const WaveBuffers & B, int level, unsigned int s, const FrameT & fr) {
    WFrame f;
    f.hit_p = fr.hit_p; f.hit_n = fr.hit_n; f.ray_d = fr.ray_d; f.T_in = fr.T_in; f.hit_pos = fr.hit_pos; f.kd = fr.kd; f.ks = fr.ks;
    f.alpha = fr.alpha; f.w_diffuse = fr.w_diffuse; f.mat = fr.mat; f.stage = fr.stage; f.idx = fr.idx;
    constexpr int FR4 = TEX ? 7 : POS ? 5 : 4;
    float4 * p = B.frames + ((size_t)level * FR4) * B.n_samples + s;
    p[0] = make_float4(f.hit_p.x, f.hit_p.y, f.hit_p.z, as_f(f.mat));
    p[(size_t)B.n_samples] = make_float4(f.hit_n.x, f.hit_n.y, f.hit_n.z, as_f(f.stage | (f.idx << 8)));
    p[(size_t)B.n_samples * 2] = make_float4(f.ray_d.x, f.ray_d.y, f.ray_d.z, f.alpha);
    p[(size_t)B.n_samples * 3] = make_float4(f.T_in.x, f.T_in.y, f.T_in.z, f.w_diffuse);
    if (POS) p[(size_t)B.n_samples * 4] = make_float4(f.hit_pos.x, f.hit_pos.y, f.hit_pos.z, 0.0f);
    if (TEX) {
        p[(size_t)B.n_samples * 5] = make_float4(f.kd.x, f.kd.y, f.kd.z, 0.0f);
        p[(size_t)B.n_samples * 6] = make_float4(f.ks.x, f.ks.y, f.ks.z, 0.0f);
    }
}

template <bool POS, bool TEX, class FrameT>
PRT_D void wframe_load(const WaveBuffers & B, int level, unsigned int s, FrameT & fr) {
    WFrame f;
    constexpr int FR4 = TEX ? 7 : POS ? 5 : 4;
    const float4 * p = B.frames + ((size_t)level * FR4) * B.n_samples + s;
    const float4 a = p[0], b = p[(size_t)B.n_samples], c = p[(size_t)B.n_samples * 2], d = p[(size_t)B.n_samples * 3];
    f.hit_p = mk3(a.x, a.y, a.z); f.mat = as_i(a.w);
    f.hit_n = mk3(b.x, b.y, b.z); f.stage = as_i(b.w) & 0xFF; f.idx = as_i(b.w) >> 8;
    f.ray_d = mk3(c.x, c.y, c.z); f.alpha = c.w;
    f.T_in = mk3(d.x, d.y, d.z); f.w_diffuse = d.w;
// ... 451 lines not shown
```

par_raytracer_amd/csrc/prt_api.hip:

```cpp
#include <hip/hip_runtime.h>

#include <algorithm>
#include <chrono>
#include <cmath>
#include <cstdio>
#include <cstring>
#include <condition_variable>
#include <mutex>
#include <new>
#include <stdexcept>
#include <string>
#include <thread>
#include <vector>

#include "../../include/prt.h"
#include "bvh_build.h"
#include "prt_options.h"
#include "dev_scene.h"
#include "tex_upload.h"
#include "kernels_wave.h"
#include "kernels_pool.h"
#include "kernels_resolve.h"
#include "bvh_lbvh.h"
#include "kernels_debug.h"
// ... 13 lines not shown
#ifndef PRT_ADAPT_WAVES
#define PRT_ADAPT_WAVES 4
#endif
#ifndef PRT_POOL_FORK_DEFAULT
#define PRT_POOL_FORK_DEFAULT 1
#endif
#ifndef PRT_POOL_SHARED_DEFAULT
#define PRT_POOL_SHARED_DEFAULT 1
#endif
#ifndef PRT_POOL_BLOCK
#define PRT_POOL_BLOCK 256
#endif
#ifndef PRT_QGRAD_MERGE_DEFAULT
#define PRT_QGRAD_MERGE_DEFAULT 1
#endif
#ifndef PRT_DEEP_WAVES
#define PRT_DEEP_WAVES PRT_POOL_WAVES
#endif
#ifndef PRT_POOL_WAVES
#define PRT_POOL_WAVES 5
#endif

enum { BVH_WIDTH = BVH_NODE_BYTES == 4 * BVH8_NODE_DWORDS ? 8 : 4 };

namespace {

std::string g_create_error;

#define HIP_TRY(ctx, call)                                                                                   \
    do {                                                                                                     \
        hipError_t e_ = (call);                                                                              \
        if (e_ != hipSuccess) {                                                                              \
            (ctx)->error = std::string(#call) + ": " + hipGetErrorString(e_);                                \
            return -10;                                                                                      \
        }                                                                                                    \
    } while (0)

template <typename T>
struct DevBuf {
    T * p = nullptr;
    size_t n = 0;
    bool borrowed = false;
    void borrow(const DevBuf & o) { release(); p = o.p; n = o.n; borrowed = o.p != nullptr; }
    hipError_t ensure(size_t count) {
        if (count <= n && p) return hipSuccess;
        if (p && !borrowed) (void)hipFree(p);
        borrowed = false;
        p = nullptr;
        n = 0;
        hipError_t e = hipMalloc((void **)&p, std::max<size_t>(count, 1) * sizeof(T));
        if (e == hipSuccess) n = count;
        return e;
    }
    hipError_t upload(const std::vector<T> & v) {
        hipError_t e = ensure(v.size());
        if (e != hipSuccess || v.empty()) return e;
        return hipMemcpy(p, v.data(), v.size() * sizeof(T), hipMemcpyHostToDevice);
    }
    void release() {
        if (p && !borrowed) (void)hipFree(p);
        borrowed = false;
        p = nullptr;
        n = 0;
    }
    size_t bytes() const { return n * sizeof(T); }
};

}

enum { PRT_MAX_CHAINS = 8 };

struct prt_ctx {
    int device = 0;
    PrtOptions opt;
    hipStream_t stream = nullptr;
    hipEvent_t ev[4] = { nullptr, nullptr, nullptr, nullptr };
    std::string error;
    bool has_scene = false;

    DevBuf<float4> nodes, tris, shade, diffuse_dirs, spec_dirs;
    DevBuf<unsigned int> tri_rank;
    DevBuf<DevMaterial> materials;
    DevBuf<DevLight> lights;
    DevScene scene;
    prt_scene_info info;
    float scene_abs_max = 0.0f;
    bool any_translucent = false;
    bool point_lights = false;
    bool textured = false;
    struct TuneEntry { uint64_t key[6]; unsigned int pipeline; };
    std::vector<TuneEntry> tuned;
    uint64_t scene_epoch = 0;
    DevBuf<DevTexture> textures;
    std::vector<DevTexture> kat_textures;
    DevBuf<unsigned int> texels;
    DevBuf<float> srgb_lut;
    DevBuf<float4> tri_uv, tri_tan;
    DevBuf<float4> ref_spheres;
    std::vector<float> material_ns;
    unsigned int spec_table_samples = 0;

    DevBuf<float4> sample_rgb;
    DevBuf<float4> frame_out;
    DevBuf<DevCounters> counters;
    DevBuf<unsigned long long> ring_ws;
    DevBuf<unsigned int> pixel_list;
    struct ChainWs {
        DevBuf<float4> f4;
        DevBuf<ulonglong2> rng;
        DevBuf<unsigned int> counts;
        DevBuf<unsigned int> overflow;
        DevBuf<int> slow_stack;
        hipStream_t stream = nullptr;
        hipEvent_t ev_t0 = nullptr, ev_t1 = nullptr, ev_done = nullptr, ev_first = nullptr;
        unsigned int * host_counts = nullptr;
    } chain[PRT_MAX_CHAINS];
    DevBuf<unsigned int> wf_counts;
    DevBuf<float4> pool_f4;
    prt_render_stats last_stats;
    uint64_t last_regions[2 * PRT_REGION_COUNT] = {};
    DevBuf<float4> pool_park;
    size_t pool_park_cap = 1u << 18, pool_spark_cap = 1u << 18;
    DevCounters * host_counters = nullptr;
    DevBuf<unsigned int> pool_fin;
    DevBuf<PoolArgs> pool_args;
    DevBuf<unsigned long long> wave_times;
    unsigned int wave_times_n = 0;
    DevBuf<float4> adapt_f4;
    int cu_count = 0;
    int reserved_cus = 0;
    unsigned int stack_bound = 0;
    DevBuf<int> stack_spill;
    std::vector<uint32_t> q_tri_order;
    std::vector<prt_group> q_groups;
    DevBuf<uint2> q_leaf_map;
    DevBuf<unsigned int> q_slot_of_rank;
    DevBuf<unsigned int> q_work;
    DevBuf<unsigned int> q_slow;
    DevBuf<int> q_exact_stack;
    DevBuf<float> q_io;
    DevBuf<unsigned char> q_occ;
    DevBuf<unsigned char> q_hemi_flags;
    std::vector<uint32_t> rf_idx_positions, rf_idx_normals;
    std::vector<unsigned int> rf_level_first;
    uint32_t rf_position_count = 0, rf_normal_count = 0;
    bool rf_bumped = false;
    DevBuf<unsigned int> rf_table;
    DevBuf<RefitBox> rf_boxes;
    DevBuf<unsigned int> rf_bounds;
    DevBuf<float> rf_in;
    DevBuf<unsigned int> qg_idx;
    DevBuf<unsigned int> qg_runs;
    DevBuf<long long> qg_acc;
    DevBuf<unsigned int> qg_words;
    DevBuf<float> qg_io;
    uint64_t geom_generation = 0;
    uint64_t sg_generation = 0;
    DevBuf<unsigned int> sg_adj;
    DevBuf<long long> sg_acc;
    uint32_t sg_edge_count = 0;
    uint64_t sm_generation = 0;
    DevBuf<unsigned int> sm_slot_of_input;
    DevBuf<double> sm_weight;
    DevBuf<unsigned long long> sm_prefix, sm_tile_sum, sm_words;
    unsigned long long sm_host_words[SAMPLE_WORDS] = {};
    unsigned long long sm_read_words[SAMPLE_WORDS] = {};
// ... 450 lines not shown
}

void launch_resolve(hipStream_t stream, const void * samples, float4 * out, unsigned int n_px, unsigned int spp, ResolveMap map) {
    const unsigned int grid2 = (unsigned int)(((unsigned long long)n_px * spp + 255ull) / 256ull);
    switch (spp) {
        case 2: hipLaunchKernelGGL((k_resolve_pow2<2, true>), dim3(grid2), dim3(256), 0, stream, samples, out, n_px, map); break;
        case 4: hipLaunchKernelGGL((k_resolve_pow2<4, true>), dim3(grid2), dim3(256), 0, stream, samples, out, n_px, map); break;
        case 8: hipLaunchKernelGGL((k_resolve_pow2<8, true>), dim3(grid2), dim3(256), 0, stream, samples, out, n_px, map); break;
        case 16: hipLaunchKernelGGL((k_resolve_pow2<16, true>), dim3(grid2), dim3(256), 0, stream, samples, out, n_px, map); break;
        case 32: hipLaunchKernelGGL((k_resolve_pow2<32, true>), dim3(grid2), dim3(256), 0, stream, samples, out, n_px, map); break;
        case 64: hipLaunchKernelGGL((k_resolve_pow2<64, true>), dim3(grid2), dim3(256), 0, stream, samples, out, n_px, map); break;
        default: hipLaunchKernelGGL(k_resolve<true>, dim3((n_px + 255) / 256), dim3(256), 0, stream, samples, out, n_px, spp, map);
    }
}

int build_bvh_lbvh(prt_ctx * ctx, const float * verts, uint32_t n_tris, uint32_t leaf_max, BvhWide * bvh) {
    float lo[3], hi[3];
    lbvh_scene_bounds(verts, n_tris, lo, hi);
    LbvhTree tree;
    double device_ms = 0.0;
    HIP_TRY(ctx, build_lbvh_tree(verts, n_tris, lo, hi, ctx->stream, &tree, &device_ms));
    build_bvh_wide_from_radix_tree(BVH_WIDTH, n_tris, leaf_max, tree.left.data(), tree.right.data(), tree.first.data(), tree.last.data(),
                                   tree.node_box.data(), tree.leaf_box.data(), tree.sorted_ids.data(), bvh, &ctx->opt.bvh);
    if (ctx->opt.debug_util) fprintf(stderr, "[prt] LBVH: %u triangles, radix tree on the device in %.2f ms\n", n_tris, device_ms);
    return 0;
}

int render_pixels(prt_ctx * ctx, const prt_camera * cam_in, const prt_params * params, uint32_t width, uint32_t height,
                  const PixelSet & px, float4 * d_out, prt_counters * counters);

int render_pixels_once(prt_ctx * ctx, const prt_camera * cam_in, const prt_params * params, uint32_t width, uint32_t height,
                       const PixelSet & px, float4 * d_out, prt_counters * counters, bool * park_overflow) {
    *park_overflow = false;
    if (!ctx->has_scene) { ctx->error = "prt_render: no scene uploaded"; return -2; }
    if (!cam_in || !params || !width || !height) { ctx->error = "prt_render: null camera / params or empty image"; return -1; }
    if (params->spp == 0 || params->spp > 65535) { ctx->error = "prt_render: spp must be in 1..65535 (prt_key.h packs the sample in 16 bits)"; return -1; }
    if (params->bounce_depth > 16) { ctx->error = "prt_render: bounce_depth > 16 not supported"; return -1; }
    if ((uint64_t)width * height >= (1ull << 32)) { ctx->error = "prt_render: image has 2^32 pixels or more"; return -1; }
    if (px.n_pixels == 0) {
        if (counters) { memset(counters, 0, sizeof(*counters)); counters->pipeline = params->pipeline & PRT_PIPELINE_MASK; }
        return 0;
    }
    HIP_TRY(ctx, hipSetDevice(ctx->device));
    hipStream_t stream = ctx->stream;

    if (std::max(1u, params->spec_samples) != ctx->spec_table_samples) {
        HIP_TRY(ctx, hipStreamSynchronize(stream));
        int rc = build_spec_table(ctx, params->spec_samples);
        if (rc) return rc;
        HIP_TRY(ctx, hipDeviceSynchronize());
    }

    DevCamera cam;
    cam.position = ld3(cam_in->position);
    cam.forward = ld3(cam_in->forward);
    cam.right_scaled = ld3(cam_in->right) * cam_in->tan_a2 * cam_in->aspect;
    cam.up_scaled = ld3(cam_in->up) * cam_in->tan_a2;
    cam.inv_width = cam_in->inv_width;
    cam.inv_height = cam_in->inv_height;

    DevParams P;
    P.ray_bias = params->ray_bias;
    P.reflection_samples = params->reflection_samples;
    P.spec_samples = params->spec_samples;
    P.bounce_depth = params->bounce_depth;
    P.background = mk3(params->background_color[0], params->background_color[1], params->background_color[2]);
    P.spp = params->spp;
    P.seed = params->seed;
    const bool adaptive = params->max_spp > params->spp;
    P.max_spp = adaptive ? params->max_spp : params->spp;
    P.variance_threshold = params->variance_threshold > 0.0f ? params->variance_threshold : 0.01f;
    P.width = width;
    P.height = height;
    float extent = ctx->scene_abs_max;
    for (int a = 0; a < 3; ++a) extent = std::max(extent, fabsf(cam_in->position[a]));
    P.box_pad = extent * (1.0f / 65536.0f);
    P.first_pixel = px.first_pixel;
    P.shard_block_rows = std::max(1u, px.block_rows);
    P.shard_rank = px.rank;
    P.shard_nranks = std::max(1u, px.nranks);
    P.pixel_list = px.d_pixel_list;
    const PrtOptions & opt = ctx->opt;
    ctx->scene.tie_widen_max = (unsigned int)std::max(0ll, std::min(64ll, opt.tie_widen_max));
    P.elide_dead_shadow_rays = opt.trace_dead_shadow_rays ? 0u : 1u;
    P.tile_pixels = 0;
    if (!px.d_pixel_list && width % 8u == 0u && !opt.no_tiles) {
        const bool rows = px.nranks > 1 ? std::max(1u, px.block_rows) % 8u == 0u : px.first_pixel % width == 0u;
        if (rows) P.tile_pixels = px.n_pixels / (8u * width) * (8u * width);
    }

    P.work_reverse_n = (opt.work_reverse > 0 && !px.d_pixel_list) ? px.n_pixels : 0u;
    P.work_scatter_n = 0; P.work_scatter_mul = 1;
    if (opt.work_scatter > 0 && !px.d_pixel_list && P.tile_pixels >= 64u) {
        const unsigned int n = P.tile_pixels / 8u;
        unsigned long long mul = std::max<unsigned long long>(3ull, (unsigned long long)((double)n * 0.6180339887));
        mul = std::min<unsigned long long>(mul, 0xFFFFFFFFull / n);
        if (!(mul & 1ull)) mul -= 1ull;
        auto gcd = [](unsigned long long a, unsigned long long b) { while (b) { const unsigned long long t = a % b; a = b; b = t; } return a; };
        while (mul > 1ull && gcd(mul, n) != 1ull) mul -= 2ull;
        if (mul > 1ull) { P.work_scatter_n = n; P.work_scatter_mul = (unsigned int)mul; }
    }
    const bool count_visits = (params->pipeline & PRT_FLAG_COUNT_VISITS) != 0;
    const bool ring = adaptive || ctx->any_translucent || ctx->textured || max_rng_draws(P.bounce_depth, P.reflection_samples, P.spec_samples) > 15;

    unsigned int pipeline = params->pipeline & PRT_PIPELINE_MASK;
    if (adaptive) {
        if (pipeline != PRT_PIPELINE_DEFAULT && pipeline != PRT_PIPELINE_POOL) { ctx->error = "prt_render: adaptive sampling (max_spp > spp) runs on PRT_PIPELINE_POOL (or DEFAULT) only"; return -1; }
        if (params->max_spp > 4096) { ctx->error = "prt_render: max_spp above 4096 is not supported"; return -1; }
        pipeline = PRT_PIPELINE_POOL;
    }
    if (pipeline == PRT_PIPELINE_DEFAULT) {
        const unsigned long long ns = (unsigned long long)px.n_pixels * params->spp;
        if (opt.pool_max_samples >= 0) {
            pipeline = ns <= (unsigned long long)opt.pool_max_samples ? PRT_PIPELINE_POOL : PRT_PIPELINE_WAVEFRONT;
        } else if (!(params->pipeline & PRT_FLAG_TRYOUT) || ns <= (1ull << 20)) {
            pipeline = PRT_PIPELINE_POOL;
        } else {
            prt_ctx::TuneEntry e;
            e.key[0] = ctx->scene_epoch;
            e.key[1] = (uint64_t)px.n_pixels | (uint64_t)params->spp << 32;
            e.key[2] = (uint64_t)width | (uint64_t)height << 32;
            e.key[3] = (uint64_t)params->bounce_depth | (uint64_t)params->reflection_samples << 32;
            e.key[4] = (uint64_t)params->spec_samples | (uint64_t)px.nranks << 32;
            e.key[5] = (uint64_t)px.block_rows | (uint64_t)(px.d_pixel_list ? 1 : 0) << 32;
            for (const prt_ctx::TuneEntry & t : ctx->tuned)
                if (!memcmp(t.key, e.key, sizeof(e.key))) pipeline = t.pipeline;
            if (pipeline == PRT_PIPELINE_DEFAULT) {
                PixelSet trial = px;
                const bool whole = ns <= (64ull << 20);
                if (!whole) trial.n_pixels = (uint32_t)std::max<unsigned long long>(64, ((32ull << 20) / params->spp) / 64 * 64);
                const unsigned int cand[2] = { PRT_PIPELINE_POOL, PRT_PIPELINE_WAVEFRONT };
                double ms[2] = { 0.0, 0.0 };
                prt_counters c;
                for (int run = 0; run < 4; ++run) {
                    prt_params pp = *params;
                    pp.pipeline = (params->pipeline & ~(uint32_t)PRT_PIPELINE_MASK) | cand[run & 1];
                    int rc = render_pixels(ctx, cam_in, &pp, width, height, trial, d_out, &c);
                    if (rc) return rc;
                    ms[run & 1] = c.render_ms;
                }
                e.pipeline = ms[0] <= 0.97 * ms[1] ? PRT_PIPELINE_POOL : PRT_PIPELINE_WAVEFRONT;
                if (ctx->tuned.size() >= 64) ctx->tuned.erase(ctx->tuned.begin());
                ctx->tuned.push_back(e);
                if (opt.debug_util) fprintf(stderr, "[prt] default pipeline try-out: pool %.3f ms, wavefront %.3f ms\n", ms[0], ms[1]);
                (void)whole;
                pipeline = e.pipeline;
            }
        }
    }
    if (pipeline == PRT_PIPELINE_MEGAKERNEL || pipeline == PRT_PIPELINE_PERSISTENT) {
        ctx->error = "prt_render: the experimental pipelines (MEGAKERNEL, PERSISTENT) are not built into this library";
        return -1;
    }
    if (pipeline != PRT_PIPELINE_WAVEFRONT && pipeline != PRT_PIPELINE_POOL) { ctx->error = "prt_render: unknown pipeline"; return -1; }

    const bool ring_eff = ring || pipeline == PRT_PIPELINE_POOL;

    const unsigned int unit_spp = adaptive ? 1u : P.spp;
    const unsigned long long total_samples = (unsigned long long)px.n_pixels * unit_spp;
    unsigned int pass_pixels = px.n_pixels;
    {
        const unsigned long long lv = std::max(1u, P.bounce_depth), fr4 = ctx->textured ? 7 : ring_eff ? 5 : 4, nl = std::max(1u, ctx->scene.light_count);
        unsigned long long per_sample = 32 + (ring ? 128 : 0);
        if (pipeline == PRT_PIPELINE_WAVEFRONT) per_sample += (lv * fr4 + 7 + 3 * nl) * 16 + (ring ? 32 : 16) + 4 * (1 + nl);
        if (pipeline == PRT_PIPELINE_POOL) per_sample += lv * fr4 * 16 + 32;
        if (adaptive) per_sample += ((unsigned long long)P.max_spp + 2) * 16;
// ... 598 lines not shown
        for (uint32_t slot = 0; slot < n_tris; ++slot) {
            const uint32_t t = ctx->q_tri_order[slot];
            for (uint32_t c = 0; c < 3; ++c) {
                table[(size_t)slot * REFIT_TABLE_WORDS + c] = ctx->rf_idx_positions[3 * (size_t)t + c];
                table[(size_t)slot * REFIT_TABLE_WORDS + 3 + c] = ctx->rf_idx_normals[3 * (size_t)t + c];
            }
        }
        hipError_t e = ctx->rf_table.upload(table);
        if (e != hipSuccess) { ctx->rf_table.release(); ctx->error = std::string("prt_update_geometry: table upload: ") + hipGetErrorString(e); return -10; }
    }
    HIP_TRY(ctx, ctx->rf_boxes.ensure(n_nodes));
    HIP_TRY(ctx, ctx->rf_bounds.ensure(2));
    const bool with_tangents = u->tangents && ctx->rf_bumped && ctx->tri_tan.p;
    RefitArgs A;
    memset(&A, 0, sizeof(A));
    A.positions = u->positions;
    A.normals = u->normals;
    A.tangents = with_tangents ? u->tangents : nullptr;
    if (!device) {
        const size_t np = 3 * (size_t)u->position_count, nn = u->normals ? 3 * (size_t)u->normal_count : 0;
        const size_t nt = with_tangents ? 3 * (size_t)ctx->rf_normal_count : 0;
        HIP_TRY(ctx, ctx->rf_in.ensure(np + nn + nt));
        float * p = ctx->rf_in.p;
        HIP_TRY(ctx, hipMemcpyAsync(p, u->positions, np * sizeof(float), hipMemcpyHostToDevice, stream));
        A.positions = p; p += np;
        if (nn) { HIP_TRY(ctx, hipMemcpyAsync(p, u->normals, nn * sizeof(float), hipMemcpyHostToDevice, stream)); A.normals = p; p += nn; }
        if (nt) { HIP_TRY(ctx, hipMemcpyAsync(p, u->tangents, nt * sizeof(float), hipMemcpyHostToDevice, stream)); A.tangents = p; }
    }
    A.table = ctx->rf_table.p;
    A.n_tris = n_tris;
    A.node_count = n_nodes;
    A.nodes = ctx->nodes.p; A.tris = ctx->tris.p; A.shade = ctx->shade.p;
    A.tri_tan = with_tangents ? ctx->tri_tan.p : nullptr;
    A.boxes = ctx->rf_boxes.p;
    A.bounds = ctx->rf_bounds.p;

    HIP_TRY(ctx, hipEventRecord(ctx->ev[0], stream));
    HIP_TRY(ctx, hipMemsetAsync(A.bounds, 0, 2 * sizeof(unsigned int), stream));
    {
        const unsigned int want = (3u * n_tris + 255u) / 256u;
        const unsigned int grid = std::max(1u, std::min(want, (unsigned int)std::max(1, ctx->cu_count) * 8u));
        hipLaunchKernelGGL(k_refit_bounds, dim3(grid), dim3(256), 0, stream, A);
        HIP_TRY(ctx, hipGetLastError());
    }
    unsigned int bounds[2] = { 0u, 0u };
    HIP_TRY(ctx, hipMemcpyAsync(bounds, A.bounds, sizeof(bounds), hipMemcpyDeviceToHost, stream));
    HIP_TRY(ctx, hipStreamSynchronize(stream));
    if (bounds[1]) { ctx->error = "prt_update_geometry: vertex coordinate is not finite or exceeds 1e18"; return -1; }
    float abs_max;
    memcpy(&abs_max, &bounds[0], 4);

#define REFIT_TRY(call)                                                                                      \
    do {                                                                                                     \
        hipError_t e_ = (call);                                                                              \
        if (e_ != hipSuccess) {                                                                              \
            ctx->error = std::string(#call) + ": " + hipGetErrorString(e_);                                  \
            ctx->has_scene = false;                                                                          \
            return -10;                                                                                      \
        }                                                                                                    \
    } while (0)
    const bool had_spheres = ctx->scene.ref_spheres != nullptr;
    const size_t old_sphere_bytes = had_spheres ? ctx->ref_spheres.bytes() : 0;
    hipLaunchKernelGGL(k_refit_records, dim3((n_tris + 255u) / 256u), dim3(256), 0, stream, A);
    REFIT_TRY(hipGetLastError());
    for (uint32_t l = levels; l-- > 0;) {
        const unsigned int first = ctx->rf_level_first[l], count = ctx->rf_level_first[l + 1] - first;
        hipLaunchKernelGGL(k_refit_level<BVH_WIDTH>, dim3((count + 63u) / 64u), dim3(64), 0, stream, A, first, count);
        REFIT_TRY(hipGetLastError());
    }
    REFIT_TRY(hipMemcpyAsync(ctx->tri_rank.p, rank.data(), rank.size() * sizeof(unsigned int), hipMemcpyHostToDevice, stream));
    ctx->q_slot_of_rank.release();
    if (!ref_spheres.empty()) {
        REFIT_TRY(ctx->ref_spheres.ensure(ref_spheres.size()));
        REFIT_TRY(hipMemcpyAsync(ctx->ref_spheres.p, ref_spheres.data(), ref_spheres.size() * sizeof(float4), hipMemcpyHostToDevice, stream));
    }
    REFIT_TRY(hipEventRecord(ctx->ev[1], stream));
    REFIT_TRY(hipStreamSynchronize(stream));
    float ms = 0.0f;
    REFIT_TRY(hipEventElapsedTime(&ms, ctx->ev[0], ctx->ev[1]));
#undef REFIT_TRY
    ctx->scene.ref_spheres = ref_spheres.empty() ? nullptr : ctx->ref_spheres.p;
    ctx->info.device_bytes = ctx->info.device_bytes - old_sphere_bytes + (ref_spheres.empty() ? 0 : ctx->ref_spheres.bytes());
    ctx->scene_abs_max = abs_max;
    ctx->tuned.clear();
    ctx->geom_generation++;
    if (info) { info->device_ms = ms; info->abs_max = abs_max; }
    return 0;
}


unsigned int grad_grid(const prt_ctx * ctx, uint32_t count) {
    return std::max(1u, std::min((count + 255u) / 256u, (unsigned int)std::max(1, ctx->cu_count) * 8u));
}

int grad_prepare(prt_ctx * ctx, const char * what, size_t np, bool want_positions) {
    if (ctx->rf_idx_positions.size() != 3 * (size_t)ctx->scene.tri_count) { ctx->error = std::string(what) + ": the scene's index buffer is not available"; return -2; }
    if (!ctx->qg_idx.p || !ctx->qg_runs.p) {
        std::vector<unsigned int> runs(2 * ctx->q_groups.size());
        for (size_t g = 0; g < ctx->q_groups.size(); ++g) { runs[2 * g] = ctx->q_groups[g].first_index; runs[2 * g + 1] = ctx->q_groups[g].index_count; }
        HIP_TRY(ctx, ctx->qg_idx.upload(ctx->rf_idx_positions));
        HIP_TRY(ctx, ctx->qg_runs.upload(runs));
        HIP_TRY(ctx, hipDeviceSynchronize());
    }
    HIP_TRY(ctx, ctx->qg_words.ensure(QGRAD_WORDS));
    if (want_positions) HIP_TRY(ctx, ctx->qg_acc.ensure(np));
    return 0;
}

struct GradScan { unsigned int words[QGRAD_WORDS]; float m; int unit_exponent; };

int grad_scan_verdict(prt_ctx * ctx, const char * what, const char * queries, uint32_t count, hipStream_t stream, GradScan * out) {
    HIP_TRY(ctx, hipGetLastError());
    memset(out, 0, sizeof(*out));
    HIP_TRY(ctx, hipMemcpyAsync(out->words, ctx->qg_words.p, sizeof(out->words), hipMemcpyDeviceToHost, stream));
    HIP_TRY(ctx, hipStreamSynchronize(stream));
    if (out->words[QGRAD_W_INVALID]) {
        char msg[240];
        snprintf(msg, sizeof(msg), "%s: %u %s name a triangle the scene does not have (group out of range, vertex0 not a multiple of 3 or past its "
                 "group's run)", what, out->words[QGRAD_W_INVALID], queries);
        ctx->error = msg;
        return -1;
    }
    memcpy(&out->m, &out->words[QGRAD_W_MAX], 4);
    out->unit_exponent = out->m > 0.0f ? qgrad_unit_exponent(out->m, count) : 0;
    return 0;
}

int grad_resolve(prt_ctx * ctx, bool adds, float * g_positions, uint32_t position_count, int unit_exponent, hipStream_t stream) {
    const size_t np = 3 * (size_t)position_count;
    if (adds) {
        QGradArgs R;
        memset(&R, 0, sizeof(R));
        R.g_positions = g_positions; R.acc = ctx->qg_acc.p; R.position_count = position_count; R.unit_exponent = unit_exponent;
        hipLaunchKernelGGL(k_qgrad_resolve, dim3((unsigned int)((np + 255) / 256)), dim3(256), 0, stream, R);
        HIP_TRY(ctx, hipGetLastError());
    } else if (g_positions && np) {
        HIP_TRY(ctx, hipMemsetAsync(g_positions, 0, np * sizeof(float), stream));
    }
    HIP_TRY(ctx, hipEventRecord(ctx->ev[1], stream));
    return 0;
}

int grad_fill_info(prt_ctx * ctx, const GradScan & scan, prt_grad_info * info) {
    if (!info) return 0;
    float ms = 0.0f;
    HIP_TRY(ctx, hipEventElapsedTime(&ms, ctx->ev[0], ctx->ev[1]));
    info->device_ms = ms;
    info->hit_rays = scan.words[QGRAD_W_HIT];
    info->skipped_rays = scan.words[QGRAD_W_SKIPPED];
    info->unit_exponent = scan.unit_exponent;
    info->max_contribution = scan.m;
    return 0;
}

struct RayGrad {
    typedef QGradArgs Args;
    const prt_ray_batch * b;
    const int32_t * group;
    const uint32_t * vertex0;
    const float * positions;
    const prt_hit_grads * gout;
    const prt_query_grads * gin;
    static const char * required() { return "null origins, directions, group, vertex0 or positions"; }
    static const char * items() { return "rays"; }
    bool complete() const { return b->origins && b->directions && group && vertex0 && positions; }
    float * want_positions() const { return gin ? gin->positions : nullptr; }
// ... 602 lines not shown
    ctx->q_tri_order.clear();
    ctx->q_groups.clear();
    ctx->rf_table.release();
    ctx->qg_idx.release(); ctx->qg_runs.release(); ctx->qg_acc.release();
    ctx->sg_adj.release(); ctx->sg_acc.release();
    ctx->sg_edge_count = 0;
    ctx->sm_slot_of_input.release(); ctx->sm_weight.release(); ctx->sm_prefix.release(); ctx->sm_tile_sum.release();
    ctx->sm_generation = 0;
    ctx->rf_idx_positions.clear();
    ctx->rf_idx_normals.clear();
    ctx->rf_level_first.clear();
    const uint32_t n_tris = s->index_count / 3;
    if (n_tris >= (1u << 26)) { ctx->error = "prt_upload_scene: 2^26 triangles or more (the traversal addresses nodes and triangles by 32-bit byte offsets)"; return -1; }

    std::vector<int32_t> tri_material(n_tris, 0);
    std::vector<uint8_t> covered(n_tris, 0);
    for (uint32_t g = 0; g < s->group_count; ++g) {
        const prt_group & pg = s->groups[g];
        if (pg.first_index % 3 || pg.index_count % 3 || (uint64_t)pg.first_index + pg.index_count > s->index_count) {
            ctx->error = "prt_upload_scene: group index range is not a whole run of triangles inside the index buffers";
            return -1;
        }
        if (pg.material < 0 || (uint32_t)pg.material >= s->material_count) { ctx->error = "prt_upload_scene: group material out of range"; return -1; }
        for (uint32_t t = pg.first_index / 3; t < (pg.first_index + pg.index_count) / 3; ++t) { tri_material[t] = pg.material; covered[t] = 1; }
    }
    for (uint32_t t = 0; t < n_tris; ++t)
        if (!covered[t]) { ctx->error = "prt_upload_scene: triangle not covered by any group"; return -1; }
    for (uint32_t i = 0; i < s->index_count; ++i) {
        if (s->idx_positions[i] >= s->position_count || s->idx_normals[i] >= s->normal_count ||
            s->idx_texcoords[i] >= s->texcoord_count) {
            ctx->error = "prt_upload_scene: vertex index out of range (the reference would read out of bounds here)";
            return -1;
        }
    }
    bool textured = false, bumped = false;
    for (uint32_t m = 0; m < s->material_count; ++m) {
        const prt_material & pm = s->materials[m];
        const int32_t slots[5] = { pm.ambient_texture, pm.diffuse_texture, pm.specular_texture, pm.alpha_texture, pm.bump_texture };
        for (int k = 0; k < 5; ++k) {
            if (slots[k] < 0) continue;
            textured = true;
            if (k == 4) bumped = true;
            if (!s->textures || (uint32_t)slots[k] >= s->texture_count) { ctx->error = "prt_upload_scene: material texture slot out of range"; return -1; }
            const prt_texture & t = s->textures[slots[k]];
            if (!t.texels || t.size_x < 2 || t.size_y < 2 || t.channels < 1 || t.channels > 4) {
                ctx->error = "prt_upload_scene: texture needs texels, 1..4 channels and at least 2 x 2 texels";
                return -1;
            }
        }
    }
    if (textured && s->texture_count >= DEV_TEX_NONE) { ctx->error = "prt_upload_scene: more than 65534 textures"; return -1; }
    if (bumped && !s->tangents) { ctx->error = "prt_upload_scene: a material has a bump map but the scene has no tangents"; return -1; }

    auto t0 = std::chrono::steady_clock::now();
    std::vector<float> verts((size_t)n_tris * 9);
    for (uint32_t t = 0; t < n_tris; ++t)
        for (int c = 0; c < 3; ++c) memcpy(&verts[(size_t)t * 9 + 3 * c], s->positions + 3 * (size_t)s->idx_positions[3 * t + c], 12);
    for (size_t i = 0; i < verts.size(); ++i)
        if (!(fabsf(verts[i]) < 1e18f)) { ctx->error = "prt_upload_scene: vertex coordinate is not finite or exceeds 1e18"; return -1; }
    BvhWide bvh;
    unsigned int hw = std::max(1u, std::thread::hardware_concurrency());
    unsigned int leaf_max = BVH_LEAF_MAX;
    if (ctx->opt.leaf_max >= 0) leaf_max = (unsigned int)std::max(1ll, std::min(4ll, ctx->opt.leaf_max));
    const float trav_cost = (float)ctx->opt.sah_trav_cost;
    if (ctx->opt.bvh_builder_lbvh) {
        int rc = build_bvh_lbvh(ctx, verts.data(), n_tris, leaf_max, &bvh);
        if (rc) return rc;
    } else {
        build_bvh_wide(BVH_WIDTH, verts.data(), n_tris, leaf_max, std::min(hw, 16u), &bvh, trav_cost, &ctx->opt.bvh);
    }
    double build_ms = std::chrono::duration<double, std::milli>(std::chrono::steady_clock::now() - t0).count();
    if (const char * bad = validate_bvh_links(bvh, n_tris)) { ctx->error = std::string("prt_upload_scene: the builder produced a broken tree - ") + bad; return -9; }

    std::vector<uint32_t> rank_of_input;
    std::vector<float4> ref_spheres;
    reference_ranks(s->groups, s->group_count, s->spheres, s->sphere_group, s->sphere_count, n_tris, rank_of_input, ref_spheres);

    const uint32_t n_rec = n_tris + 1;
    std::vector<float4> tris((size_t)n_rec * 3, make_float4(0, 0, 0, 0)), shade((size_t)n_rec * 4, make_float4(0, 0, 0, 0));
    std::vector<unsigned int> rank(n_rec, 0);
    std::vector<float4> tri_uv(textured ? (size_t)n_rec * 2 : 0, make_float4(0, 0, 0, 0));
    std::vector<float4> tri_tan(bumped ? (size_t)n_rec * 3 : 0, make_float4(0, 0, 0, 0));
    float abs_max = 0.0f;
    for (uint32_t slot = 0; slot < n_tris; ++slot) {
        const uint32_t t = bvh.tri_order[slot];
        const f3 a = ld3(&verts[(size_t)t * 9]), b = ld3(&verts[(size_t)t * 9 + 3]), c = ld3(&verts[(size_t)t * 9 + 6]);
        const f3 ab = b - a, ac = c - a;
        const f3 n = cross3(ab, ac);
        tris[(size_t)slot * 3 + 0] = make_float4(a.x, a.y, a.z, ab.x);
        tris[(size_t)slot * 3 + 1] = make_float4(ab.y, ab.z, ac.x, ac.y);
        tris[(size_t)slot * 3 + 2] = make_float4(ac.z, n.x, n.y, n.z);
        const float * n0 = s->normals + 3 * (size_t)s->idx_normals[3 * t + 0];
        const float * n1 = s->normals + 3 * (size_t)s->idx_normals[3 * t + 1];
        const float * n2 = s->normals + 3 * (size_t)s->idx_normals[3 * t + 2];
        const float * u0 = s->texcoords + 2 * (size_t)s->idx_texcoords[3 * t + 0];
        const float * u1 = s->texcoords + 2 * (size_t)s->idx_texcoords[3 * t + 1];
        const float * u2 = s->texcoords + 2 * (size_t)s->idx_texcoords[3 * t + 2];
        float mbits;
        int32_t mi = tri_material[t];
        memcpy(&mbits, &mi, 4);
        shade[(size_t)slot * 4 + 0] = make_float4(n0[0], n0[1], n0[2], n1[0]);
        shade[(size_t)slot * 4 + 1] = make_float4(n1[1], n1[2], n2[0], n2[1]);
        shade[(size_t)slot * 4 + 2] = make_float4(n2[2], n.x, n.y, n.z);
        shade[(size_t)slot * 4 + 3] = make_float4(0.0f, 0.0f, 0.0f, mbits);
        if (textured) tex_pack_uv(u0, u1, u2, &tri_uv[(size_t)slot * 2]);
        if (bumped) {
            const float * g0 = s->tangents + 3 * (size_t)s->idx_normals[3 * t + 0];
            const float * g1 = s->tangents + 3 * (size_t)s->idx_normals[3 * t + 1];
            const float * g2 = s->tangents + 3 * (size_t)s->idx_normals[3 * t + 2];
            tex_pack_tangents(g0, g1, g2, &tri_tan[(size_t)slot * 3]);
        }
        rank[slot] = rank_of_input[t];
        for (int k = 0; k < 9; ++k) abs_max = std::max(abs_max, fabsf(verts[(size_t)t * 9 + k]));
    }

    std::vector<DevMaterial> mats(s->material_count);
    ctx->material_ns.resize(s->material_count);
    ctx->any_translucent = false;
    for (uint32_t m = 0; m < s->material_count; ++m) {
        const prt_material & pm = s->materials[m];
        DevMaterial & d = mats[m];
        memset(&d, 0, sizeof(d));
        for (int k = 0; k < 3; ++k) { d.ambient[k] = pm.ambient_color[k]; d.diffuse[k] = pm.diffuse_color[k]; d.specular[k] = pm.specular_color[k]; }
        d.specular_intensity = pm.specular_intensity;
        d.index_of_refraction = pm.index_of_refraction;
        d.alpha = pm.alpha;
        tex_pack_material_slots(pm, d);
        ctx->material_ns[m] = pm.specular_intensity;
        if (!(pm.alpha >= 1.0f)) ctx->any_translucent = true;
    }
    std::vector<DevTexture> dev_tex;
    std::vector<unsigned int> texel_pool;
    std::vector<float> lut;
    if (textured) {
        if (!tex_expand_rgba8(s->textures, s->texture_count, dev_tex, texel_pool)) { ctx->error = "prt_upload_scene: more than 2^32 texels"; return -1; }
        tex_fill_srgb_lut(lut);
    }
    ctx->kat_textures = dev_tex;
    std::vector<DevLight> lights(std::max(1u, s->light_count));
    memset(lights.data(), 0, lights.size() * sizeof(DevLight));
    for (uint32_t l = 0; l < s->light_count; ++l) {
        const prt_light & pl = s->lights[l];
        DevLight & d = lights[l];
        d.type = pl.type;
        for (int k = 0; k < 3; ++k) { d.color[k] = pl.color[k]; d.position[k] = pl.position[k]; d.facing[k] = pl.facing[k]; }
        d.falloff = pl.falloff;
    }
    ctx->point_lights = false;
    for (uint32_t l = 0; l < s->light_count; ++l) ctx->point_lights = ctx->point_lights || s->lights[l].type == PRT_LIGHT_POINT;
    std::vector<float4> ddirs(1024);
    for (uint32_t i = 0; i < 1024; ++i) ddirs[i] = diffuse_tangent_dir(i);

    std::vector<float4> nodes4(bvh.nodes.size() / 4);
    memcpy(nodes4.data(), bvh.nodes.data(), bvh.nodes.size() * sizeof(uint32_t));
    ctx->stack_bound = bvh.stack_bound;

    HIP_TRY(ctx, ctx->nodes.upload(nodes4));
    HIP_TRY(ctx, ctx->tris.upload(tris));
    HIP_TRY(ctx, ctx->shade.upload(shade));
    HIP_TRY(ctx, ctx->tri_rank.upload(rank));
    HIP_TRY(ctx, ctx->materials.upload(mats));
    HIP_TRY(ctx, ctx->lights.upload(lights));
    HIP_TRY(ctx, ctx->diffuse_dirs.upload(ddirs));
    if (!ref_spheres.empty()) HIP_TRY(ctx, ctx->ref_spheres.upload(ref_spheres));
    ctx->textured = textured;
    if (textured) {
        HIP_TRY(ctx, ctx->textures.upload(dev_tex));
        HIP_TRY(ctx, ctx->texels.upload(texel_pool));
        HIP_TRY(ctx, ctx->srgb_lut.upload(lut));
        HIP_TRY(ctx, ctx->tri_uv.upload(tri_uv));
        if (bumped) HIP_TRY(ctx, ctx->tri_tan.upload(tri_tan));
    }

    DevScene & sc = ctx->scene;
    sc.nodes = ctx->nodes.p;
    sc.tris = ctx->tris.p;
    sc.shade = ctx->shade.p;
    sc.tri_rank = ctx->tri_rank.p;
    sc.materials = ctx->materials.p;
    sc.lights = ctx->lights.p;
    sc.diffuse_dirs = ctx->diffuse_dirs.p;
    sc.light_count = s->light_count;
    sc.material_count = s->material_count;
    sc.tri_count = n_tris;
    sc.node_count = bvh.node_count;
    sc.textures = textured ? ctx->textures.p : nullptr;
    sc.texels = textured ? ctx->texels.p : nullptr;
    sc.srgb_lut = textured ? ctx->srgb_lut.p : nullptr;
    sc.tri_uv = textured ? ctx->tri_uv.p : nullptr;
    sc.tri_tan = bumped ? ctx->tri_tan.p : nullptr;
    sc.ref_spheres = ref_spheres.empty() ? nullptr : ctx->ref_spheres.p;
    sc.tie_widen_max = 8;
    sc.near_tie_unresolved = &ctx->counters.p->near_tie_unresolved;
    ctx->spec_table_samples = 0;
    int rc = build_spec_table(ctx, 1);
    if (rc) return rc;

    ctx->scene_abs_max = abs_max;
    prt_scene_info & info = ctx->info;
    info.triangle_count = n_tris;
    info.bvh_node_count = bvh.node_count;
    info.bvh_max_depth = bvh.max_depth;
    info.bvh_node_bytes = BVH_NODE_BYTES;
    info.tri_record_bytes = 48;
    info.shade_record_bytes = 64;
    info.device_bytes = ctx->nodes.bytes() + ctx->tris.bytes() + ctx->shade.bytes() + ctx->tri_rank.bytes() +
                        ctx->materials.bytes() + ctx->lights.bytes() + ctx->diffuse_dirs.bytes() + ctx->spec_dirs.bytes() +
                        (textured ? ctx->textures.bytes() + ctx->texels.bytes() + ctx->srgb_lut.bytes() + ctx->tri_uv.bytes() : 0) +
                        (bumped ? ctx->tri_tan.bytes() : 0) + (ref_spheres.empty() ? 0 : ctx->ref_spheres.bytes());
    info.bvh_build_ms = build_ms;
    ctx->q_tri_order.swap(bvh.tri_order);
    ctx->q_groups.assign(s->groups, s->groups + s->group_count);
    ctx->rf_idx_positions.assign(s->idx_positions, s->idx_positions + s->index_count);
    ctx->rf_idx_normals.assign(s->idx_normals, s->idx_normals + s->index_count);
    ctx->rf_position_count = s->position_count;
    ctx->rf_normal_count = s->normal_count;
    ctx->rf_bumped = bumped;
    if (!refit_level_table<BVH_WIDTH>(bvh.nodes.data(), bvh.node_count, &ctx->rf_level_first)) ctx->rf_level_first.clear();
    HIP_TRY(ctx, hipDeviceSynchronize());
    ctx->has_scene = true;
    ctx->scene_epoch++;
    ctx->geom_generation++;
    ctx->tuned.clear();
    return 0;
    PRT_API_CATCH_RC(ctx, "prt_upload_scene")
}

int prt_get_scene_info(const prt_ctx * ctx, prt_scene_info * info) {
    PRT_API_TRY
    if (!ctx || !info) return -1;
    if (!ctx->has_scene) return -2;
    *info = ctx->info;
    return 0;
    PRT_API_CATCH_RC(nullptr, "prt_get_scene_info")
}

int prt_render_device(prt_ctx * ctx, const prt_camera * cam, const prt_params * params, uint32_t width, uint32_t height,
                      uint32_t start_idx, uint32_t end_idx, void * d_rgba_out, prt_counters * counters) {
    PRT_API_TRY
    if (!ctx) return -1;
    if ((!d_rgba_out && end_idx != start_idx) || end_idx < start_idx || (uint64_t)end_idx > (uint64_t)width * height) {
        ctx->error = "prt_render: bad output pointer or pixel range";
        return -1;
    }
    PixelSet px = { end_idx - start_idx, start_idx, 1, 0, 1, nullptr };
    return render_pixels(ctx, cam, params, width, height, px, (float4 *)d_rgba_out, counters);
    PRT_API_CATCH_RC(ctx, "prt_render_device")
}

int prt_render(prt_ctx * ctx, const prt_camera * cam, const prt_params * params, uint32_t width, uint32_t height,
               uint32_t start_idx, uint32_t end_idx, float * rgba_out, prt_counters * counters) {
    PRT_API_TRY
    if (!ctx) return -1;
    if ((!rgba_out && end_idx != start_idx) || end_idx < start_idx) { ctx->error = "prt_render: bad output pointer or pixel range"; return -1; }
    HIP_TRY(ctx, hipSetDevice(ctx->device));
    const size_t n = end_idx - start_idx;
    HIP_TRY(ctx, ctx->frame_out.ensure(n));
    int rc = prt_render_device(ctx, cam, params, width, height, start_idx, end_idx, ctx->frame_out.p, counters);
    if (rc) return rc;
    if (n) HIP_TRY(ctx, hipMemcpy(rgba_out, ctx->frame_out.p, n * sizeof(float4), hipMemcpyDeviceToHost));
    return 0;
    PRT_API_CATCH_RC(ctx, "prt_render")
}

uint32_t prt_shard_rows(uint32_t height, uint32_t block_rows, uint32_t rank, uint32_t nranks) {
    if (!block_rows || !nranks || rank >= nranks) return 0;
    uint32_t rows = 0;
    for (uint64_t b = rank; b * block_rows < height; b += nranks) rows += std::min<uint64_t>(block_rows, height - b * block_rows);
    return rows;
}

int prt_render_shard_device(prt_ctx * ctx, const prt_camera * cam, const prt_params * params, uint32_t width, uint32_t height,
                            uint32_t block_rows, uint32_t rank, uint32_t nranks, void * d_rgba_out, prt_counters * counters) {
    PRT_API_TRY
    if (!ctx) return -1;
    if (!block_rows || !nranks || rank >= nranks) { ctx->error = "prt_render_shard: bad arguments"; return -1; }
    if (!d_rgba_out && prt_shard_rows(height, block_rows, rank, nranks)) { ctx->error = "prt_render_shard: null output"; return -1; }
    PixelSet px = { prt_shard_rows(height, block_rows, rank, nranks) * width, 0, block_rows, rank, nranks, nullptr };
    if (nranks == 1) { px.block_rows = 1; }
    return render_pixels(ctx, cam, params, width, height, px, (float4 *)d_rgba_out, counters);
    PRT_API_CATCH_RC(ctx, "prt_render_shard_device")
}

int prt_render_shard(prt_ctx * ctx, const prt_camera * cam, const prt_params * params, uint32_t width, uint32_t height,
                     uint32_t block_rows, uint32_t rank, uint32_t nranks, float * rgba_out, prt_counters * counters) {
    PRT_API_TRY
    if (!ctx) return -1;
    const size_t n = (size_t)prt_shard_rows(height, block_rows, rank, nranks) * width;
    if (!rgba_out && n) { ctx->error = "prt_render_shard: null output"; return -1; }
    HIP_TRY(ctx, hipSetDevice(ctx->device));
    HIP_TRY(ctx, ctx->frame_out.ensure(n));
    int rc = prt_render_shard_device(ctx, cam, params, width, height, block_rows, rank, nranks, ctx->frame_out.p, counters);
    if (rc) return rc;
    if (n) HIP_TRY(ctx, hipMemcpy(rgba_out, ctx->frame_out.p, n * sizeof(float4), hipMemcpyDeviceToHost));
    return 0;
    PRT_API_CATCH_RC(ctx, "prt_render_shard")
}

int prt_render_pixel_list(prt_ctx * ctx, const prt_camera * cam, const prt_params * params, uint32_t width, uint32_t height,
                          const uint32_t * pixel_ids, uint32_t n_pixels, float * rgba_out, prt_counters * counters) {
    PRT_API_TRY
    if (!ctx) return -1;
    if ((!pixel_ids || !rgba_out) && n_pixels) { ctx->error = "prt_render_pixel_list: null pixel list or output"; return -1; }
    for (uint32_t i = 0; i < n_pixels; ++i)
        if ((uint64_t)pixel_ids[i] >= (uint64_t)width * height) { ctx->error = "prt_render_pixel_list: pixel id outside the image"; return -1; }
    HIP_TRY(ctx, hipSetDevice(ctx->device));
    HIP_TRY(ctx, ctx->pixel_list.ensure(n_pixels));
    HIP_TRY(ctx, ctx->frame_out.ensure(n_pixels));
    if (n_pixels) HIP_TRY(ctx, hipMemcpyAsync(ctx->pixel_list.p, pixel_ids, (size_t)n_pixels * 4, hipMemcpyHostToDevice, ctx->stream));
    if (n_pixels) HIP_TRY(ctx, hipStreamSynchronize(ctx->stream));
    PixelSet px = { n_pixels, 0, 1, 0, 1, ctx->pixel_list.p };
    int rc = render_pixels(ctx, cam, params, width, height, px, ctx->frame_out.p, counters);
    if (rc) return rc;
    if (n_pixels) HIP_TRY(ctx, hipMemcpy(rgba_out, ctx->frame_out.p, (size_t)n_pixels * sizeof(float4), hipMemcpyDeviceToHost));
    return 0;
    PRT_API_CATCH_RC(ctx, "prt_render_pixel_list")
}

int prt_trace_rays_device(prt_ctx * ctx, int mode, const prt_ray_batch * batch, const prt_hit_buffers * hits, uint32_t flags,
// ... 265 lines not shown
    for (size_t i = 0; i < (size_t)n_tris * 9; ++i)
        if (!(fabsf(verts[i]) < 1e18f)) { ctx->error = "prt_debug_lbvh_tree: vertex coordinate is not finite or exceeds 1e18"; return -1; }
    HIP_TRY(ctx, hipSetDevice(ctx->device));
    float lo[3], hi[3];
    lbvh_scene_bounds(verts, n_tris, lo, hi);
    LbvhTree tree;
    HIP_TRY(ctx, build_lbvh_tree(verts, n_tris, lo, hi, ctx->stream, &tree, nullptr, sorted_keys != nullptr));
    const size_t n = n_tris, ni = tree.left.size();
    if (left) memcpy(left, tree.left.data(), ni * 4);
    if (right) memcpy(right, tree.right.data(), ni * 4);
    if (first) memcpy(first, tree.first.data(), ni * 4);
    if (last) memcpy(last, tree.last.data(), ni * 4);
    if (node_box) memcpy(node_box, tree.node_box.data(), ni * 24);
    if (leaf_box) memcpy(leaf_box, tree.leaf_box.data(), n * 24);
    if (sorted_ids) memcpy(sorted_ids, tree.sorted_ids.data(), n * 4);
    if (sorted_keys) memcpy(sorted_keys, tree.sorted_keys.data(), n * 8);
    return 0;
    PRT_API_CATCH_RC(ctx, "prt_debug_lbvh_tree")
}

}

__global__ void k_assemble_shards(const float4 * staging, float4 * frame, unsigned int width, unsigned int height,
                                  unsigned int block_rows, unsigned int n_dev, unsigned int max_shard_rows) {
    const unsigned int i = blockIdx.x * blockDim.x + threadIdx.x;
    if (i >= width * height) return;
    const unsigned int y = i / width, x = i - y * width;
    const unsigned int b = y / block_rows, g = b % n_dev;
    const unsigned int local_row = (b / n_dev) * block_rows + (y - b * block_rows);
    frame[i] = staging[((size_t)g * max_shard_rows + local_row) * width + x];
}

enum { PRT_MULTI_BLOCK_ROWS = 8, PRT_MULTI_MAX_DEPTH = 4 };

struct MultiLane {
    std::vector<prt_ctx *> ctx;
    std::vector<DevBuf<float4> > shard;
    DevBuf<float4> staging, frame;
    std::vector<hipEvent_t> done;
    bool busy = false;
    uint64_t ticket = 0;
    prt_camera cam;
    prt_params params;
    uint32_t width = 0, height = 0;
    float * rgba_out = nullptr;
    unsigned int pending = 0;
    std::vector<uint64_t> job;
    std::vector<int> rc;
    std::vector<std::string> err;
    std::vector<prt_counters> ctr;
};

struct prt_multi {
    std::vector<int> devices;
    std::vector<MultiLane> lane;
    std::vector<std::thread> workers;
    std::mutex mu;
    std::condition_variable cv_work, cv_done;
    bool quit = false;
    uint64_t next_ticket = 1;
    std::string error;
};

namespace {

prt_ctx * clone_context(prt_ctx * src) {
    prt_ctx * c = prt_create(src->device);
    if (!c) return nullptr;
    c->opt = src->opt;
    c->nodes.borrow(src->nodes); c->tris.borrow(src->tris); c->shade.borrow(src->shade); c->diffuse_dirs.borrow(src->diffuse_dirs);
    c->tri_rank.borrow(src->tri_rank); c->materials.borrow(src->materials); c->lights.borrow(src->lights);
    c->textures.borrow(src->textures); c->texels.borrow(src->texels); c->srgb_lut.borrow(src->srgb_lut);
    c->tri_uv.borrow(src->tri_uv); c->tri_tan.borrow(src->tri_tan); c->ref_spheres.borrow(src->ref_spheres);
    c->scene = src->scene;
    c->scene.near_tie_unresolved = &c->counters.p->near_tie_unresolved;
    c->scene.spec_dirs = nullptr;
    c->spec_table_samples = 0;
    c->material_ns = src->material_ns;
    c->info = src->info;
    c->scene_abs_max = src->scene_abs_max;
    c->any_translucent = src->any_translucent; c->point_lights = src->point_lights; c->textured = src->textured;
    c->kat_textures = src->kat_textures;
    c->stack_bound = src->stack_bound;
    c->pool_park_cap = src->pool_park_cap; c->pool_spark_cap = src->pool_spark_cap;
    c->has_scene = src->has_scene;
    c->scene_epoch = 1;
    return c;
}

void multi_worker(prt_multi * m, unsigned int f, unsigned int g) {
    MultiLane & L = m->lane[f];
    uint64_t seen = 0;
    for (;;) {
        {
            std::unique_lock<std::mutex> lk(m->mu);
            m->cv_work.wait(lk, [&] { return m->quit || L.job[g] != seen; });
            if (m->quit) return;
            seen = L.job[g];
        }
        int rc = 0;
        std::string err;
        prt_counters ctr;
        memset(&ctr, 0, sizeof(ctr));
        try {
            const unsigned int n = (unsigned int)L.ctx.size();
            prt_ctx * c = L.ctx[g], * c0 = L.ctx[0];
            const size_t rows = prt_shard_rows(L.height, PRT_MULTI_BLOCK_ROWS, g, n);
            const uint32_t max_rows = prt_shard_rows(L.height, PRT_MULTI_BLOCK_ROWS, 0, n);
            hipError_t e = hipSetDevice(c->device);
            if (e == hipSuccess) e = L.shard[g].ensure(std::max<size_t>(1, rows * L.width));
            if (e != hipSuccess) { rc = PRT_ERR_HIP; err = std::string("shard buffer: ") + hipGetErrorString(e); }
            if (!rc) {
                rc = prt_render_shard_device(c, &L.cam, &L.params, L.width, L.height, PRT_MULTI_BLOCK_ROWS, g, n, L.shard[g].p, &ctr);
                if (rc) err = prt_last_error(c);
            }
            if (!rc && n > 1) {
                if (rows) e = hipMemcpyPeerAsync(L.staging.p + (size_t)g * max_rows * L.width, c0->device, L.shard[g].p, c->device,
                                                 rows * L.width * sizeof(float4), c->stream);
                if (e == hipSuccess) e = hipEventRecord(L.done[g], c->stream);
                if (e != hipSuccess) { rc = PRT_ERR_HIP; err = std::string("peer copy: ") + hipGetErrorString(e); }
            }
        } catch (...) {
            rc = api_exception(&err, "prt_multi worker");
        }
        {
            std::lock_guard<std::mutex> lk(m->mu);
            L.rc[g] = rc;
            try { L.err[g] = err; } catch (...) {}
            L.ctr[g] = ctr;
            if (--L.pending == 0) m->cv_done.notify_all();
        }
    }
}

void multi_release_lane(MultiLane & L, bool destroy_ctx) {
    for (size_t g = 0; g < L.ctx.size(); ++g) {
        if (!L.ctx[g]) continue;
        (void)hipSetDevice(L.ctx[g]->device);
        if (L.ctx[g]->stream) (void)hipStreamSynchronize(L.ctx[g]->stream);
        if (g < L.shard.size()) L.shard[g].release();
        if (g < L.done.size() && L.done[g]) { (void)hipEventDestroy(L.done[g]); L.done[g] = nullptr; }
    }
    if (!L.ctx.empty() && L.ctx[0]) {
        (void)hipSetDevice(L.ctx[0]->device);
        L.staging.release();
        L.frame.release();
    }
    if (destroy_ctx)
        for (size_t g = 0; g < L.ctx.size(); ++g) { prt_destroy(L.ctx[g]); L.ctx[g] = nullptr; }
}

void multi_quiesce(prt_multi * m) {
    for (MultiLane & L : m->lane)
        for (prt_ctx * c : L.ctx)
            if (c && c->stream) { (void)hipSetDevice(c->device); (void)hipStreamSynchronize(c->stream); }
}

}

extern "C" {

prt_multi * prt_multi_create(const int * device_ids, int n_dev) {
    PRT_API_TRY
    if (!device_ids || n_dev < 1) { g_create_error = "prt_multi_create: no devices"; return nullptr; }
    prt_multi * m = new prt_multi;
    m->devices.assign(device_ids, device_ids + n_dev);
// ... 21 lines not shown
            if (hipSetDevice(c->device) != hipSuccess || hipEventCreateWithFlags(&L.done[(size_t)g], hipEventDisableTiming) != hipSuccess) {
                g_create_error = "prt_multi_create: event creation failed";
                prt_multi_destroy(m);
                return nullptr;
            }
            if (&L == &m->lane[0] && g > 0 && c->device != c0->device) {
                int can = 0;
                if (hipDeviceCanAccessPeer(&can, c0->device, c->device) == hipSuccess && can) {
                    (void)hipSetDevice(c0->device);
                    (void)hipDeviceEnablePeerAccess(c->device, 0);
                    (void)hipGetLastError();
                }
            }
        }
    for (unsigned int f = 0; f < (unsigned int)depth; ++f)
        for (unsigned int g = 0; g < (unsigned int)n_dev; ++g) m->workers.emplace_back(multi_worker, m, f, g);
    return m;
    PRT_API_CATCH_PTR("prt_multi_create")
}

void prt_multi_destroy(prt_multi * m) {
    PRT_API_TRY
    if (!m) return;
    {
        std::unique_lock<std::mutex> lk(m->mu);
        m->cv_done.wait(lk, [&] { for (MultiLane & L : m->lane) if (L.pending) return false; return true; });
        m->quit = true;
    }
    m->cv_work.notify_all();
    for (std::thread & t : m->workers) if (t.joinable()) t.join();
    for (size_t f = m->lane.size(); f-- > 0;) multi_release_lane(m->lane[f], true);
    delete m;
    PRT_API_CATCH_VOID
}

const char * prt_multi_last_error(const prt_multi * m) { return m ? m->error.c_str() : g_create_error.c_str(); }
int prt_multi_device_count(const prt_multi * m) { return m ? (int)m->devices.size() : 0; }
int prt_multi_depth(const prt_multi * m) { return m ? (int)m->lane.size() : 0; }
prt_ctx * prt_multi_context(prt_multi * m, int i) { return m && i >= 0 && (size_t)i < m->devices.size() ? m->lane[0].ctx[(size_t)i] : nullptr; }

int prt_multi_upload_scene(prt_multi * m, const prt_scene_desc * scene) {
    PRT_API_TRY
    if (!m) return -1;
    {
        std::lock_guard<std::mutex> lk(m->mu);
        for (MultiLane & L : m->lane)
            if (L.busy) { m->error = "prt_multi_upload_scene: a frame is still in flight (prt_multi_wait it first)"; return PRT_ERR_IN_FLIGHT; }
    }
    for (size_t f = 1; f < m->lane.size(); ++f)
        for (size_t g = 0; g < m->lane[f].ctx.size(); ++g) { prt_destroy(m->lane[f].ctx[g]); m->lane[f].ctx[g] = nullptr; }
    for (size_t g = 0; g < m->devices.size(); ++g) {
        const int rc = prt_upload_scene(m->lane[0].ctx[g], scene);
        if (rc) { m->error = prt_last_error(m->lane[0].ctx[g]); return rc; }
    }
    for (size_t f = 1; f < m->lane.size(); ++f)
        for (size_t g = 0; g < m->devices.size(); ++g) {
            m->lane[f].ctx[g] = clone_context(m->lane[0].ctx[g]);
            if (!m->lane[f].ctx[g]) { m->error = std::string("prt_multi_upload_scene: ") + g_create_error; return PRT_ERR_HIP; }
        }
    return 0;
    PRT_API_CATCH_RC_MULTI(m, "prt_multi_upload_scene")
}

int prt_multi_update_geometry(prt_multi * m, const prt_geometry_update * update) {
    PRT_API_TRY
    if (!m) return -1;
    {
        std::lock_guard<std::mutex> lk(m->mu);
        for (MultiLane & L : m->lane)
            if (L.busy) { m->error = "prt_multi_update_geometry: a frame is still in flight (prt_multi_wait it first)"; return PRT_ERR_IN_FLIGHT; }
    }
    int rc = 0;
    for (size_t g = 0; g < m->devices.size() && !rc; ++g) {
        rc = prt_update_geometry(m->lane[0].ctx[g], update, nullptr);
        if (rc) m->error = prt_last_error(m->lane[0].ctx[g]);
    }
    for (size_t f = 1; f < m->lane.size(); ++f)
        for (size_t g = 0; g < m->devices.size(); ++g) {
            prt_ctx * src = m->lane[0].ctx[g], * c = m->lane[f].ctx[g];
            if (!src || !c) continue;
            c->ref_spheres.borrow(src->ref_spheres);
            c->scene.ref_spheres = src->scene.ref_spheres;
            c->scene_abs_max = src->scene_abs_max;
            c->info = src->info;
            c->has_scene = src->has_scene;
            c->tuned.clear();
        }
    return rc;
    PRT_API_CATCH_RC_MULTI(m, "prt_multi_update_geometry")
}

#define MULTI_TRY(m, call)                                                                                   \
    do {                                                                                                     \
        hipError_t e_ = (call);                                                                              \
        if (e_ != hipSuccess) { (m)->error = std::string(#call) + ": " + hipGetErrorString(e_); multi_quiesce(m); return PRT_ERR_HIP; } \
    } while (0)

int prt_multi_submit(prt_multi * m, const prt_camera * cam, const prt_params * params, uint32_t width, uint32_t height,
                     float * rgba_out, uint64_t * ticket) {
    PRT_API_TRY
    if (!m || m->devices.empty()) return -1;
    if (!cam || !params || !ticket) { m->error = "prt_multi_submit: null camera, params or ticket"; return -1; }
    if (!rgba_out && width && height) { m->error = "prt_multi_submit: null output"; return -1; }
    const unsigned int n = (unsigned int)m->devices.size();
    MultiLane * L = nullptr;
    {
        std::lock_guard<std::mutex> lk(m->mu);
        for (MultiLane & c : m->lane)
            if (!c.busy && c.ctx[0]) { L = &c; break; }
        if (!L) { m->error = "prt_multi_submit: every lane has a frame in flight (prt_multi_wait the oldest ticket first)"; return PRT_ERR_IN_FLIGHT; }
        L->busy = true;
    }
    const uint32_t max_rows = prt_shard_rows(height, PRT_MULTI_BLOCK_ROWS, 0, n);
    prt_ctx * c0 = L->ctx[0];
    hipError_t e = hipSetDevice(c0->device);
    if (e == hipSuccess && n > 1) e = L->staging.ensure((size_t)n * max_rows * width);
    if (e == hipSuccess && n > 1) e = L->frame.ensure((size_t)width * height);
    if (e != hipSuccess) {
        std::lock_guard<std::mutex> lk(m->mu);
        L->busy = false;
        m->error = std::string("prt_multi_submit: buffers on device 0: ") + hipGetErrorString(e);
        return PRT_ERR_HIP;
    }
    {
        std::lock_guard<std::mutex> lk(m->mu);
        L->cam = *cam; L->params = *params; L->width = width; L->height = height; L->rgba_out = rgba_out;
        L->ticket = m->next_ticket++;
        L->pending = n;
        for (unsigned int g = 0; g < n; ++g) { L->rc[g] = 0; L->err[g].clear(); L->job[g]++; }
        *ticket = L->ticket;
    }
    m->cv_work.notify_all();
    return 0;
    PRT_API_CATCH_RC_MULTI(m, "prt_multi_submit")
}

int prt_multi_wait(prt_multi * m, uint64_t ticket, prt_counters * counters) {
    PRT_API_TRY
    if (!m || m->devices.empty()) return -1;
    const unsigned int n = (unsigned int)m->devices.size();
    MultiLane * L = nullptr;
    {
        std::unique_lock<std::mutex> lk(m->mu);
        for (MultiLane & c : m->lane)
            if (c.busy && c.ticket == ticket) { L = &c; break; }
        if (!L) { m->error = "prt_multi_wait: no frame with this ticket is in flight"; return -1; }
        m->cv_done.wait(lk, [&] { return L->pending == 0; });
    }
    struct Release { prt_multi * m; MultiLane * L; ~Release() { std::lock_guard<std::mutex> lk(m->mu); L->busy = false; } } release = { m, L };
    for (unsigned int g = 0; g < n; ++g)
        if (L->rc[g]) { m->error = L->err[g]; multi_quiesce(m); return L->rc[g]; }
    prt_ctx * c0 = L->ctx[0];
    const size_t n_px = (size_t)L->width * L->height;
    MULTI_TRY(m, hipSetDevice(c0->device));
    if (n == 1) {
        if (n_px) MULTI_TRY(m, hipMemcpy(L->rgba_out, L->shard[0].p, n_px * sizeof(float4), hipMemcpyDeviceToHost));
    } else {
        const uint32_t max_rows = prt_shard_rows(L->height, PRT_MULTI_BLOCK_ROWS, 0, n);
        for (unsigned int g = 0; g < n; ++g) MULTI_TRY(m, hipStreamWaitEvent(c0->stream, L->done[g], 0));
        if (n_px) {
            hipLaunchKernelGGL(k_assemble_shards, dim3((unsigned int)((n_px + 255) / 256)), dim3(256), 0, c0->stream, L->staging.p, L->frame.p,
                               L->width, L->height, (unsigned int)PRT_MULTI_BLOCK_ROWS, n, max_rows);
            MULTI_TRY(m, hipGetLastError());
            MULTI_TRY(m, hipMemcpyAsync(L->rgba_out, L->frame.p, n_px * sizeof(float4), hipMemcpyDeviceToHost, c0->stream));
        }
        MULTI_TRY(m, hipStreamSynchronize(c0->stream));
// ... 40 lines not shown
```

par_raytracer_amd/csrc/prt_options.h:

```cpp
#pragma once

#include <cstdio>
#include <cstdlib>
#include <cstring>
#include <strings.h>

namespace prt {

struct BvhBuildOptions {
    long long sah_bins = -1;
    long long sah_sweep = -1;
    long long collapse = -1;
    long long lbvh_plain = 0;
    long long lbvh_cluster = -1;
    long long width = 8;
    long long axis_rule = 0;
    long long debug = 0;
};

struct PrtOptions {
    long long trace_dead_shadow_rays = 0;
    long long bvh_builder_lbvh = 0;
    long long pool_exact = 0;
    long long tie_widen_max = 8;
    long long debug_util = 0, debug_rounds = 0;
    long long chunk_min = -1, trace_blocks_per_cu = -1, keep_min = -1, node_min = -1, node_frac = -1, chains = -1, shade_block = -1;
    long long pool_blocks_per_cu = -1, pool_cap = -1, pool_topup = -1, pool_max_samples = -1, pool_park_cap = -1;
    long long pool_shared = -1;
    long long pool_fork = -1;
    long long pool_fork_room = -1;
    long long pool_guided = -1;
    long long pool_guided_min = -1;
    long long pool_fair = -1;
    long long work_scatter = 0;
    long long work_reverse = 0;
    long long pool_shared_cap = -1;
    long long pass_samples = -1, pass_mb = -1, stack_cap = -1, no_tiles = 0;
    long long qgrad_merge = -1;
    long long hemi_pass_items = -1;
    long long reserve_cus = 0;
    long long reserve_pattern = 2;
    long long leaf_max = -1;
    double sah_trav_cost = 1.0;
    BvhBuildOptions bvh;
};

namespace detail {
struct OptEntry { const char * name; long long PrtOptions::* field; long long BvhBuildOptions::* bvh_field; };
inline const OptEntry * option_table(size_t * n) {
    static const OptEntry table[] = {
        { "TRACE_DEAD_SHADOW_RAYS", &PrtOptions::trace_dead_shadow_rays, nullptr }, { "POOL_EXACT", &PrtOptions::pool_exact, nullptr },
        { "TIE_WIDEN_MAX", &PrtOptions::tie_widen_max, nullptr },
        { "DEBUG_UTIL", &PrtOptions::debug_util, nullptr }, { "DEBUG_ROUNDS", &PrtOptions::debug_rounds, nullptr },
        { "CHUNK_MIN", &PrtOptions::chunk_min, nullptr }, { "TRACE_BLOCKS_PER_CU", &PrtOptions::trace_blocks_per_cu, nullptr },
        { "KEEP_MIN", &PrtOptions::keep_min, nullptr }, { "NODE_MIN", &PrtOptions::node_min, nullptr }, { "NODE_FRAC", &PrtOptions::node_frac, nullptr },
        { "CHAINS", &PrtOptions::chains, nullptr }, { "SHADE_BLOCK", &PrtOptions::shade_block, nullptr },
        { "POOL_BLOCKS_PER_CU", &PrtOptions::pool_blocks_per_cu, nullptr }, { "POOL_CAP", &PrtOptions::pool_cap, nullptr },
        { "POOL_TOPUP", &PrtOptions::pool_topup, nullptr }, { "POOL_MAX_SAMPLES", &PrtOptions::pool_max_samples, nullptr },
        { "POOL_PARK_CAP", &PrtOptions::pool_park_cap, nullptr }, { "POOL_SHARED", &PrtOptions::pool_shared, nullptr }, { "POOL_FORK", &PrtOptions::pool_fork, nullptr }, { "POOL_FORK_ROOM", &PrtOptions::pool_fork_room, nullptr }, { "POOL_FAIR", &PrtOptions::pool_fair, nullptr }, { "POOL_GUIDED", &PrtOptions::pool_guided, nullptr }, { "POOL_GUIDED_MIN", &PrtOptions::pool_guided_min, nullptr }, { "WORK_REVERSE", &PrtOptions::work_reverse, nullptr }, { "WORK_SCATTER", &PrtOptions::work_scatter, nullptr },
        { "POOL_SHARED_CAP", &PrtOptions::pool_shared_cap, nullptr }, { "PASS_SAMPLES", &PrtOptions::pass_samples, nullptr },
        { "PASS_MB", &PrtOptions::pass_mb, nullptr }, { "STACK_CAP", &PrtOptions::stack_cap, nullptr }, { "NO_TILES", &PrtOptions::no_tiles, nullptr },
        { "QGRAD_MERGE", &PrtOptions::qgrad_merge, nullptr }, { "HEMI_PASS_ITEMS", &PrtOptions::hemi_pass_items, nullptr },
        { "RESERVE_CUS", &PrtOptions::reserve_cus, nullptr }, { "RESERVE_PATTERN", &PrtOptions::reserve_pattern, nullptr }, { "LEAF_MAX", &PrtOptions::leaf_max, nullptr },
        { "SAH_BINS", nullptr, &BvhBuildOptions::sah_bins }, { "SAH_SWEEP", nullptr, &BvhBuildOptions::sah_sweep },
        { "LBVH_PLAIN", nullptr, &BvhBuildOptions::lbvh_plain }, { "LBVH_CLUSTER", nullptr, &BvhBuildOptions::lbvh_cluster },
        { "BVH8_WIDTH", nullptr, &BvhBuildOptions::width }, { "BVH8_AXIS_RULE", nullptr, &BvhBuildOptions::axis_rule },
    };
    *n = sizeof(table) / sizeof(table[0]);
    return table;
}
}

inline int prt_option_set(PrtOptions & o, const char * name, const char * value) {
    if (!name) return -1;
    if (!strncasecmp(name, "PRT_", 4)) name += 4;
    const PrtOptions defaults;
    if (!strcasecmp(name, "BVH_BUILDER")) {
        if (!value || !strcasecmp(value, "sah") || !*value) { o.bvh_builder_lbvh = 0; return 0; }
        if (!strcasecmp(value, "lbvh")) { o.bvh_builder_lbvh = 1; return 0; }
        return -1;
    }
    if (!strcasecmp(name, "BVH_COLLAPSE")) {
        if (!value || !*value) { o.bvh.collapse = -1; return 0; }
        if (!strcasecmp(value, "greedy")) { o.bvh.collapse = 0; return 0; }
        if (!strcasecmp(value, "dp")) { o.bvh.collapse = 1; return 0; }
        return -1;
    }
    if (!strcasecmp(name, "SAH_TRAV_COST")) {
        if (!value) { o.sah_trav_cost = defaults.sah_trav_cost; return 0; }
        char * end = nullptr;
        const double v = strtod(value, &end);
        if (end == value) return -1;
        o.sah_trav_cost = v;
        return 0;
    }
    size_t n = 0;
    const detail::OptEntry * table = detail::option_table(&n);
    for (size_t i = 0; i < n; ++i) {
        if (strcasecmp(name, table[i].name)) continue;
        long long & dst = table[i].field ? o.*(table[i].field) : o.bvh.*(table[i].bvh_field);
        if (!value) { dst = table[i].field ? defaults.*(table[i].field) : defaults.bvh.*(table[i].bvh_field); return 0; }
        char * end = nullptr;
        const long long v = strtoll(value, &end, 10);
        if (end == value) {
            const bool is_flag = table[i].field == &PrtOptions::trace_dead_shadow_rays || table[i].field == &PrtOptions::pool_exact ||
                                 table[i].field == &PrtOptions::debug_util || table[i].field == &PrtOptions::debug_rounds ||
                                 table[i].field == &PrtOptions::no_tiles || table[i].bvh_field == &BvhBuildOptions::lbvh_plain;
            if (!is_flag) return -1;
            dst = 1;
            return 0;
        }
        dst = v;
        return 0;
    }
    return -1;
}

inline void prt_options_from_env(PrtOptions & o) {
    size_t n = 0;
    const detail::OptEntry * table = detail::option_table(&n);
    char key[64];
    for (size_t i = 0; i < n; ++i) {
        snprintf(key, sizeof(key), "PRT_%s", table[i].name);
        if (const char * v = getenv(key)) prt_option_set(o, table[i].name, v);
    }
    if (const char * v = getenv("PRT_BVH_BUILDER")) prt_option_set(o, "BVH_BUILDER", v);
    if (const char * v = getenv("PRT_BVH_COLLAPSE")) prt_option_set(o, "BVH_COLLAPSE", v);
    if (const char * v = getenv("PRT_SAH_TRAV_COST")) prt_option_set(o, "SAH_TRAV_COST", v);
    o.bvh.debug = o.debug_util;
}

}
```

Measured before the change: 7219 Mrays/s.

## Build per-light shadow BVHs excluding light-facing triangles for directional shadow rays

For each directional light, triangles whose geometric normal provably faces the light (with a conservative floating-point margin) are dropped, and a separate wide BVH is built over the remaining potential occluders. That BVH is appended to the node and record arrays, and its root is stored in the light's pad field. Shadow any-hit rays start traversal at this root instead of the main BVH root, aiming to visit fewer nodes and triangles. The trade-off is extra build time, device memory and duplicated triangle records, and correctness depends on the exclusion test being conservative.

Result: faster. 7747 Mrays/s (median of 6 runs) (+7.3%).

```diff
diff --git a/include/prt.h b/include/prt.h
--- a/include/prt.h
+++ b/include/prt.h
@@ -286,6 +286,19 @@
     double bvh_build_ms;
 } prt_scene_info;
 int prt_get_scene_info(const prt_ctx * ctx, prt_scene_info * info);
+
+enum { PRT_MAX_SHADOW_TREES = 4 };
+typedef struct prt_shadow_tree_info {
+    uint32_t built;
+    uint32_t active;
+    uint32_t triangle_count;
+    uint32_t node_count;
+    uint32_t root;
+    uint32_t stack_bound;
+    uint64_t device_bytes;
+    double build_ms;
+} prt_shadow_tree_info;
+int prt_get_shadow_trees(const prt_ctx * ctx, prt_shadow_tree_info * out, uint32_t cap);
 
 typedef struct prt_render_stats {
     uint64_t node_visits, tri_tests;
diff --git a/par_raytracer_amd/api.py b/par_raytracer_amd/api.py
--- a/par_raytracer_amd/api.py
+++ b/par_raytracer_amd/api.py
@@ -218,6 +218,14 @@
         info = PrtSceneInfo()
         self._check(self._lib.prt_get_scene_info(self._ctx, C.byref(info)), "prt_get_scene_info")
         return info
+
+    def shadow_trees(self) -> list:
+        n = self._lib.prt_get_shadow_trees(self._ctx, None, 0)
+        if n < 0:
+            self._check(n, "prt_get_shadow_trees")
+        out = (capi.PrtShadowTreeInfo * max(1, n))()
+        self._check(min(0, self._lib.prt_get_shadow_trees(self._ctx, out, n)), "prt_get_shadow_trees")
+        return [out[i] for i in range(n)]
 
     def render_stats(self) -> "capi.PrtRenderStats":
         st = capi.PrtRenderStats()
diff --git a/par_raytracer_amd/capi.py b/par_raytracer_amd/capi.py
--- a/par_raytracer_amd/capi.py
+++ b/par_raytracer_amd/capi.py
@@ -82,6 +82,17 @@
         return {n: getattr(self, n) for n, _ in self._fields_}
 
 
+class PrtShadowTreeInfo(C.Structure):
+    _fields_ = [("built", C.c_uint32), ("active", C.c_uint32), ("triangle_count", C.c_uint32), ("node_count", C.c_uint32),
+                ("root", C.c_uint32), ("stack_bound", C.c_uint32), ("device_bytes", C.c_uint64), ("build_ms", C.c_double)]
+
+    def as_dict(self):
+        return {n: getattr(self, n) for n, _ in self._fields_}
+
+
+MAX_SHADOW_TREES = 4
+
+
 class PrtRenderStats(C.Structure):
     _fields_ = [("node_visits", C.c_uint64), ("tri_tests", C.c_uint64), ("wave_node_steps", C.c_uint64),
                 ("wave_tri_steps", C.c_uint64), ("wave_leaf_visits", C.c_uint64), ("wave_refills", C.c_uint64),
@@ -184,7 +195,7 @@
 BUILD_EXPERIMENTAL, BUILD_BVH4 = 1, 2
 
 PRT_SYMBOLS = ["prt_create", "prt_destroy", "prt_last_error", "prt_abi_version", "prt_set_option", "prt_build_flags", "prt_upload_scene", "prt_render",
-               "prt_render_device", "prt_shard_rows", "prt_render_shard_device", "prt_render_shard", "prt_render_pixel_list", "prt_get_scene_info", "prt_get_render_stats", "prt_debug_check_bvh", "prt_debug_check_bvh_lbvh", "prt_debug_lbvh_tree", "prt_debug_device_kat",
+               "prt_render_device", "prt_shard_rows", "prt_render_shard_device", "prt_render_shard", "prt_render_pixel_list", "prt_get_scene_info", "prt_get_shadow_trees", "prt_get_render_stats", "prt_debug_check_bvh", "prt_debug_check_bvh_lbvh", "prt_debug_lbvh_tree", "prt_debug_device_kat",
                "prt_multi_create", "prt_multi_destroy", "prt_multi_last_error", "prt_multi_device_count", "prt_multi_context",
                "prt_multi_upload_scene", "prt_multi_render", "prt_multi_depth", "prt_multi_submit", "prt_multi_wait", "prt_debug_throw",
                "prt_trace_rays", "prt_trace_rays_device", "prt_get_region_stats",
@@ -247,6 +258,8 @@
                                               C.c_void_p, C.c_uint32, C.c_void_p, C.POINTER(PrtCounters)]
         lib.prt_get_scene_info.argtypes = [C.c_void_p, C.POINTER(PrtSceneInfo)]
         lib.prt_get_render_stats.argtypes = [C.c_void_p, C.POINTER(PrtRenderStats)]
+        if hasattr(lib, "prt_get_shadow_trees"):
+            lib.prt_get_shadow_trees.argtypes = [C.c_void_p, C.POINTER(PrtShadowTreeInfo), C.c_uint32]
         if hasattr(lib, "prt_get_region_stats"):
             lib.prt_get_region_stats.argtypes = [C.c_void_p, C.POINTER(C.c_uint64), C.c_uint32]
         lib.prt_debug_check_bvh.argtypes = [C.POINTER(PrtSceneDesc), C.POINTER(C.c_uint64)]
diff --git a/par_raytracer_amd/csrc/bvh_build.cpp b/par_raytracer_amd/csrc/bvh_build.cpp
--- a/par_raytracer_amd/csrc/bvh_build.cpp
+++ b/par_raytracer_amd/csrc/bvh_build.cpp
@@ -512,6 +512,99 @@
     b.configure(opt);
     build_sah_binary(b, verts, n_tris, leaf_max, threads, trav_cost, out->scene_lo, out->scene_hi);
     finish_wide(b, n_tris, width, out);
+}
+
+bool shadow_tri_excluded(const float n[3], const float d[3], double origin_max) {
+    const double u = 5.9604644775390625e-8, lo60 = 8.673617379884035e-19, hi60 = 1152921504606846976.0;
+    const double D = std::max(std::max(fabs((double)d[0]), fabs((double)d[1])), fabs((double)d[2]));
+    const double N1 = fabs((double)n[0]) + fabs((double)n[1]) + fabs((double)n[2]);
+    if (!(N1 >= lo60 && N1 <= hi60)) return false;
+    if (!(D >= 9.5367431640625e-7 && D <= 1048576.0)) return false;
+    if (!(origin_max >= 0.0 && origin_max <= hi60)) return false;
+    const double E = u * (origin_max + 2.0 * D) * (1.0 + u);
+    const double margin = N1 * (E + 4.0 * u * (D + E) + D * 8.881784197001252e-16) * (1.0 + 9.5367431640625e-7);
+    const double dn = (double)d[0] * (double)n[0] + (double)d[1] * (double)n[1] + (double)d[2] * (double)n[2];
+    return dn >= margin;
+}
+
+void shadow_occluders(const float * normals, uint32_t n_tris, const float d[3], double origin_max, std::vector<uint32_t> * ids) {
+    ids->clear();
+    for (uint32_t t = 0; t < n_tris; ++t)
+        if (!shadow_tri_excluded(normals + 3 * (size_t)t, d, origin_max)) ids->push_back(t);
+}
+
+void make_empty_bvh(int width, BvhWide * out) {
+    if (width != 4 && width != 8) throw std::invalid_argument("make_empty_bvh: width must be 4 or 8");
+    *out = BvhWide();
+    const bool eight = width == 8;
+    const uint32_t one = 127u << 23;
+    out->node_dwords = eight ? BVH8_NODE_DWORDS : BVH4_NODE_DWORDS;
+    out->nodes.assign(out->node_dwords, 0u);
+    uint32_t * d = out->nodes.data();
+    if (eight) {
+        d[3] = d[6] = d[7] = one;
+        d[4] = 1u;
+        for (int k = 8; k < 14; ++k) d[k] = 0xFFFFFFFFu;
+    } else {
+        d[3] = d[14] = d[15] = one;
+        d[4] = d[5] = d[6] = 0xFFFFFFFFu;
+        for (int k = 0; k < 4; ++k) d[10 + k] = (uint32_t)~(int32_t)0;
+    }
+    out->node_count = 1;
+    out->max_depth = 1;
+    out->stack_bound = eight ? 3 : 5;
+}
+
+void rebase_bvh_nodes(const BvhWide & sub, uint32_t node_base, uint32_t tri_base, uint32_t * dst) {
+    memcpy(dst, sub.nodes.data(), sub.nodes.size() * sizeof(uint32_t));
+    for (uint32_t ni = 0; ni < sub.node_count; ++ni) {
+        uint32_t * d = dst + (size_t)ni * sub.node_dwords;
+        if (sub.node_dwords == BVH8_NODE_DWORDS) {
+            d[4] += node_base;
+            d[5] += tri_base;
+            continue;
+        }
+        for (int k = 0; k < 4; ++k) {
+            const int32_t link = (int32_t)d[10 + k];
+            if (link >= 0) { d[10 + k] = (uint32_t)link + node_base; continue; }
+            const uint32_t leaf = (uint32_t)~link;
+            d[10 + k] = (uint32_t)~(int32_t)((((leaf >> 2) + tri_base) << 2) | (leaf & 3u));
+        }
+    }
+}
+
+const char * append_shadow_tree(const ShadowTreeBuild & how, const float * verts, const float * normals, uint32_t n_tris, const float d[3], double origin_max,
+                                std::vector<uint32_t> * node_words, uint32_t node_base, uint32_t rec_base,
+                                std::vector<uint32_t> * rec_tri, ShadowTreeResult * r, BvhWide * built) {
+    *r = ShadowTreeResult();
+    *built = BvhWide();
+    rec_tri->clear();
+    std::vector<uint32_t> ids;
+    shadow_occluders(normals, n_tris, d, origin_max, &ids);
+    const uint32_t m = (uint32_t)ids.size();
+    r->triangle_count = m;
+    if ((uint64_t)m * 100u > (uint64_t)n_tris * how.ratio_percent) return nullptr;
+    BvhWide sub;
+    if (m) {
+        std::vector<float> sub_verts((size_t)m * 9);
+        for (uint32_t i = 0; i < m; ++i) memcpy(&sub_verts[(size_t)i * 9], verts + (size_t)ids[i] * 9, 36);
+        build_bvh_wide(how.width, sub_verts.data(), m, how.leaf_max, how.threads, &sub, how.trav_cost, how.opt);
+    } else {
+        make_empty_bvh(how.width, &sub);
+    }
+    if ((uint64_t)node_base + sub.node_count >= (1u << 26) || (uint64_t)rec_base + m + 1u >= (1u << 26)) return nullptr;
+    if (node_words->size() != (size_t)node_base * sub.node_dwords) return "shadow tree: the node array does not end at node_base";
+    node_words->resize(((size_t)node_base + sub.node_count) * sub.node_dwords);
+    rebase_bvh_nodes(sub, node_base, rec_base, &(*node_words)[(size_t)node_base * sub.node_dwords]);
+    for (uint32_t slot = 0; slot < m; ++slot) rec_tri->push_back(ids[sub.tri_order[slot]]);
+    rec_tri->push_back(0xFFFFFFFFu);
+    r->built = 1;
+    r->node_count = sub.node_count;
+    r->root = node_base;
+    r->stack_bound = sub.stack_bound;
+    built->nodes.swap(sub.nodes); built->tri_order.swap(sub.tri_order);
+    built->node_dwords = sub.node_dwords; built->node_count = sub.node_count; built->max_depth = sub.max_depth; built->stack_bound = sub.stack_bound;
+    return nullptr;
 }
 
 namespace {
diff --git a/par_raytracer_amd/csrc/bvh_build.h b/par_raytracer_amd/csrc/bvh_build.h
--- a/par_raytracer_amd/csrc/bvh_build.h
+++ b/par_raytracer_amd/csrc/bvh_build.h
@@ -29,6 +29,22 @@
                                     const uint32_t * first, const uint32_t * last, const float * node_box, const float * leaf_box,
                                     const uint32_t * sorted_ids, BvhWide * out, const BvhBuildOptions * opt = nullptr);
 
+bool shadow_tri_excluded(const float n[3], const float d[3], double origin_max);
+void shadow_occluders(const float * normals, uint32_t n_tris, const float d[3], double origin_max, std::vector<uint32_t> * ids);
+void make_empty_bvh(int width, BvhWide * out);
+void rebase_bvh_nodes(const BvhWide & sub, uint32_t node_base, uint32_t tri_base, uint32_t * dst);
+
+struct ShadowTreeBuild {
+    int width = 4;
+    uint32_t leaf_max = 4, threads = 1, ratio_percent = 75;
+    float trav_cost = 1.0f;
+    const BvhBuildOptions * opt = nullptr;
+};
+struct ShadowTreeResult { uint32_t built = 0, triangle_count = 0, node_count = 0, root = 0, stack_bound = 0; };
+const char * append_shadow_tree(const ShadowTreeBuild & how, const float * verts, const float * normals, uint32_t n_tris, const float d[3], double origin_max,
+                                std::vector<uint32_t> * node_words, uint32_t node_base, uint32_t rec_base,
+                                std::vector<uint32_t> * rec_tri, ShadowTreeResult * r, BvhWide * built);
+
 const char * validate_bvh_links(const BvhWide & bvh, uint32_t n_tris);
 
 void check_bvh_wide(const float * verts, uint32_t n_tris, const BvhWide & bvh, uint64_t * out);
diff --git a/par_raytracer_amd/csrc/dev_scene.h b/par_raytracer_amd/csrc/dev_scene.h
--- a/par_raytracer_amd/csrc/dev_scene.h
+++ b/par_raytracer_amd/csrc/dev_scene.h
@@ -32,6 +32,7 @@
     float facing[3];
     float pad;
 };
+PRT_D int light_shadow_root(const DevLight & L) { return __float_as_int(L.pad); }
 
 struct DevScene {
     const float4 * nodes;
diff --git a/par_raytracer_amd/csrc/dev_trace.h b/par_raytracer_amd/csrc/dev_trace.h
--- a/par_raytracer_amd/csrc/dev_trace.h
+++ b/par_raytracer_amd/csrc/dev_trace.h
@@ -9,7 +9,7 @@
 namespace prt {
 
 template <bool ANY_LENGTH, class STK>
-PRT_D void trav_start(TravRay & r, f3 o, f3 d, int kind, float pad, const STK & stk) {
+PRT_D void trav_start(TravRay & r, f3 o, f3 d, int kind, float pad, const STK & stk, int root = 0) {
     if (ANY_LENGTH) {
         f3 w = (o + d) - o;
         if (w.x == 0.0f && w.y == 0.0f && w.z == 0.0f) w = d;
@@ -23,11 +23,11 @@
         if (fabsf(w.x) < tiny) w.x = copysignf(tiny, w.x);
         if (fabsf(w.y) < tiny) w.y = copysignf(tiny, w.y);
         if (fabsf(w.z) < tiny) w.z = copysignf(tiny, w.z);
-        trav_init(r, o, w, kind, pad, stk);
+        trav_init(r, o, w, kind, pad, stk, root);
         r.d = d;
         return;
     }
-    trav_init(r, o, d, kind, pad, stk);
+    trav_init(r, o, d, kind, pad, stk, root);
 }
 
 template <class STK, bool COUNT, bool ANY_LENGTH = false>
@@ -90,9 +90,9 @@
 }
 
 template <class STK, bool COUNT, bool ANY_LENGTH = false>
-PRT_D HitRec trace_ray(const DevScene & sc, f3 o, f3 d, int kind, float pad, const STK & stk, TraceStats & st) {
+PRT_D HitRec trace_ray(const DevScene & sc, f3 o, f3 d, int kind, float pad, const STK & stk, TraceStats & st, int root = 0) {
     TravRay r;
-    trav_start<ANY_LENGTH>(r, o, d, kind, pad, stk);
+    trav_start<ANY_LENGTH>(r, o, d, kind, pad, stk, root);
     for (;;) {
         while (trav_walking(r)) trav_node_step<STK, COUNT>(sc, r, stk, st, pad);
         if (trav_done(r)) break;
diff --git a/par_raytracer_amd/csrc/dev_trace4.h b/par_raytracer_amd/csrc/dev_trace4.h
--- a/par_raytracer_amd/csrc/dev_trace4.h
+++ b/par_raytracer_amd/csrc/dev_trace4.h
@@ -92,7 +92,7 @@
 }
 
 template <class STK>
-PRT_D void trav_init(TravRay & r, f3 o, f3 d, int kind, float pad, const STK & stk) {
+PRT_D void trav_init(TravRay & r, f3 o, f3 d, int kind, float pad, const STK & stk, int root = 0) {
     r.o = o;
     r.d = d;
     const float tiny = 1e-30f;
@@ -107,7 +107,7 @@
     r.kind = kind;
     stk.push(0, TRAV_SENTINEL);
     r.sp = 1;
-    r.node = 0;
+    r.node = root;
 }
 
 PRT_D void cswap(float & ka, float & kb, int & la, int & lb) {
diff --git a/par_raytracer_amd/csrc/dev_trace8.h b/par_raytracer_amd/csrc/dev_trace8.h
--- a/par_raytracer_amd/csrc/dev_trace8.h
+++ b/par_raytracer_amd/csrc/dev_trace8.h
@@ -86,7 +86,7 @@
 }
 
 template <class STK>
-PRT_D void trav_init(TravRay & r, f3 o, f3 d, int kind, float pad, const STK & stk) {
+PRT_D void trav_init(TravRay & r, f3 o, f3 d, int kind, float pad, const STK & stk, int root = 0) {
     r.o = o;
     r.d = d;
     const float tiny = 1e-30f;
@@ -102,7 +102,7 @@
     r.kind = kind | oct << 4;
     stk.put(0, make_int2(TRAV_SENTINEL, 0));
     r.sp = 1;
-    r.node = 0;
+    r.node = root;
     r.tbase = 0u;
     r.tbits = 0u;
 }
diff --git a/par_raytracer_amd/csrc/kernels_pool.h b/par_raytracer_amd/csrc/kernels_pool.h
--- a/par_raytracer_amd/csrc/kernels_pool.h
+++ b/par_raytracer_amd/csrc/kernels_pool.h
@@ -405,7 +405,7 @@
                             if (payload.w < 0.0f) {
                                 const DevLight & L = lights[(unsigned int)(-payload.w) - 1u];
                                 const f3 lv = mk3(L.facing[0], L.facing[1], L.facing[2]) * -1.0f;
-                                rd = make_float4(lv.x, lv.y, lv.z, 0.0f);
+                                rd = make_float4(lv.x, lv.y, lv.z, L.pad);
                                 kind = WF_KIND_SHADOW_ANY;
                             } else {
                                 rd = sq_d[j];
@@ -415,7 +415,7 @@
                         sample = as_i(ro.w);
                         const f3 d = mk3(rd.x, rd.y, rd.z);
                         const f3 ob = mk3(ro.x, ro.y, ro.z) + d * P.ray_bias;
-                        trav_init(r, ob, d, kind == WF_KIND_SHADOW_ANY ? TRACE_ANY : TRACE_CLOSEST, P.box_pad, stack);
+                        trav_init(r, ob, d, kind == WF_KIND_SHADOW_ANY ? TRACE_ANY : TRACE_CLOSEST, P.box_pad, stack, kind == WF_KIND_SHADOW_ANY ? as_i(rd.w) : 0);
                         ray = (int)idx;
                     }
                     next += take;
@@ -822,7 +822,8 @@
         const int sample = as_i(ro.w);
         const f3 d = mk3(rd.x, rd.y, rd.z);
         const f3 ob = mk3(ro.x, ro.y, ro.z) + d * P.ray_bias;
-        const HitRec h = trace_ray<GlobalStack, COUNT>(sc, ob, d, pay.w < 0.0f ? TRACE_ANY : TRACE_CLOSEST, P.box_pad, slow, st);
+        const int root = pay.w < 0.0f ? light_shadow_root(sc.lights[(unsigned int)(-pay.w) - 1u]) : 0;
+        const HitRec h = trace_ray<GlobalStack, COUNT>(sc, ob, d, pay.w < 0.0f ? TRACE_ANY : TRACE_CLOSEST, P.box_pad, slow, st, root);
         if (shadow_lit(h, pay.w)) accum_add(A.B.accum + sample, mk3(pay.x, pay.y, pay.z));
     }
     if (COUNT) trace_stats_flush<false>(ctr, st);
diff --git a/par_raytracer_amd/csrc/kernels_wave.h b/par_raytracer_amd/csrc/kernels_wave.h
--- a/par_raytracer_amd/csrc/kernels_wave.h
+++ b/par_raytracer_amd/csrc/kernels_wave.h
@@ -63,14 +63,16 @@
     return slot;
 }
 
-PRT_D float4 shadow_entry_dir(const DevLight * lights, float4 payload, const float4 * sq_d, unsigned int j, int & kind) {
+PRT_D float4 shadow_entry_dir(const DevLight * lights, float4 payload, const float4 * sq_d, unsigned int j, int & kind, int & root) {
     if (payload.w < 0.0f) {
         const DevLight & L = lights[(unsigned int)(-payload.w) - 1u];
         const f3 lv = mk3(L.facing[0], L.facing[1], L.facing[2]) * -1.0f;
         kind = WF_KIND_SHADOW_ANY;
+        root = light_shadow_root(L);
         return make_float4(lv.x, lv.y, lv.z, 0.0f);
     }
     kind = WF_KIND_SHADOW_DIST;
+    root = 0;
     return sq_d[j];
 }
 PRT_D bool shadow_lit(const HitRec & h, float w) { return h.tri < 0 || (w >= 0.0f && h.t * h.t <= w); }
@@ -95,7 +97,7 @@
 
 struct TraceEntry {
     f3 ob, d;
-    int kind, sample;
+    int kind, sample, root;
 };
 PRT_D TraceEntry trace_entry(const DevScene & sc, const DevParams & P, const WaveBuffers & B, int cur, unsigned int n_closest,
                              unsigned int idx, float4 & payload) {
@@ -105,11 +107,12 @@
         ro = B.rq_o[cur][idx];
         rd = B.rq_d[cur][idx];
         e.kind = WF_KIND_CLOSEST;
+        e.root = 0;
     } else {
         const unsigned int j = idx - n_closest;
         ro = B.sq_o[j];
         payload = B.sq_c[j];
-        rd = shadow_entry_dir(sc.lights, payload, B.sq_d, j, e.kind);
+        rd = shadow_entry_dir(sc.lights, payload, B.sq_d, j, e.kind, e.root);
     }
     e.sample = as_i(ro.w);
     e.d = mk3(rd.x, rd.y, rd.z);
@@ -133,7 +136,7 @@
     PRT_D bool start(unsigned int idx, TravRay & r, const LdsStack<BLOCK> & stack) {
         const TraceEntry e = trace_entry(this->sc, P, B, cur, n_closest, idx, payload);
         sample = e.sample;
-        trav_init(r, e.ob, e.d, trace_entry_mode(e), this->pad, stack);
+        trav_init(r, e.ob, e.d, trace_entry_mode(e), this->pad, stack, e.root);
         return true;
     }
     PRT_D void finish(unsigned int idx, const TravRay & r, const LdsStack<BLOCK> & stack) const {
@@ -165,7 +168,7 @@
     exact_list_walk<COUNT>(B.overflow, B.counts[3], P.exact_stack, P.exact_stack_stride, ctr, [&](unsigned int idx, const GlobalStack & slow, TraceStats & st) {
         float4 payload = make_float4(0, 0, 0, 0);
         const TraceEntry e = trace_entry(sc, P, B, cur, n_closest, idx, payload);
-        const HitRec best = trace_ray<GlobalStack, COUNT>(sc, e.ob, e.d, trace_entry_mode(e), P.box_pad, slow, st);
+        const HitRec best = trace_ray<GlobalStack, COUNT>(sc, e.ob, e.d, trace_entry_mode(e), P.box_pad, slow, st, e.root);
         trace_entry_emit(B, n_closest, idx, best, payload, e.sample);
     });
 }
diff --git a/par_raytracer_amd/csrc/prt_api.hip b/par_raytracer_amd/csrc/prt_api.hip
--- a/par_raytracer_amd/csrc/prt_api.hip
+++ b/par_raytracer_amd/csrc/prt_api.hip
@@ -119,6 +119,10 @@
     DevBuf<unsigned int> tri_rank;
     DevBuf<DevMaterial> materials;
     DevBuf<DevLight> lights;
+    unsigned int light_stride = 1;
+    std::vector<prt_shadow_tree_info> shadow_info;
+    bool shadow_trees_fresh = false;
+    float shadow_bias_max = 0.0f, shadow_cam_max = 0.0f;
     DevScene scene;
     prt_scene_info info;
     float scene_abs_max = 0.0f;
@@ -735,6 +739,11 @@
     P.pixel_list = px.d_pixel_list;
     const PrtOptions & opt = ctx->opt;
     ctx->scene.tie_widen_max = (unsigned int)std::max(0ll, std::min(64ll, opt.tie_widen_max));
+    {
+        bool trees = opt.shadow_trees != 0 && ctx->shadow_trees_fresh && fabsf(params->ray_bias) <= ctx->shadow_bias_max;
+        for (int a = 0; a < 3; ++a) trees = trees && fabsf(cam_in->position[a]) <= ctx->shadow_cam_max;
+        ctx->scene.lights = ctx->lights.p + (trees ? 0u : ctx->light_stride);
+    }
     P.elide_dead_shadow_rays = opt.trace_dead_shadow_rays ? 0u : 1u;
     P.tile_pixels = 0;
     if (!px.d_pixel_list && width % 8u == 0u && !opt.no_tiles) {
@@ -1499,6 +1508,8 @@
     ctx->scene.ref_spheres = ref_spheres.empty() ? nullptr : ctx->ref_spheres.p;
     ctx->info.device_bytes = ctx->info.device_bytes - old_sphere_bytes + (ref_spheres.empty() ? 0 : ctx->ref_spheres.bytes());
     ctx->scene_abs_max = abs_max;
+    ctx->shadow_trees_fresh = false;
+    for (prt_shadow_tree_info & si : ctx->shadow_info) si.active = 0;
     ctx->tuned.clear();
     ctx->geom_generation++;
     if (info) { info->device_ms = ms; info->abs_max = abs_max; }
@@ -2267,14 +2278,20 @@
     std::vector<float4> tri_uv(textured ? (size_t)n_rec * 2 : 0, make_float4(0, 0, 0, 0));
     std::vector<float4> tri_tan(bumped ? (size_t)n_rec * 3 : 0, make_float4(0, 0, 0, 0));
     float abs_max = 0.0f;
-    for (uint32_t slot = 0; slot < n_tris; ++slot) {
-        const uint32_t t = bvh.tri_order[slot];
+    auto put_tri_record = [&](uint32_t t, size_t slot) {
         const f3 a = ld3(&verts[(size_t)t * 9]), b = ld3(&verts[(size_t)t * 9 + 3]), c = ld3(&verts[(size_t)t * 9 + 6]);
         const f3 ab = b - a, ac = c - a;
         const f3 n = cross3(ab, ac);
-        tris[(size_t)slot * 3 + 0] = make_float4(a.x, a.y, a.z, ab.x);
-        tris[(size_t)slot * 3 + 1] = make_float4(ab.y, ab.z, ac.x, ac.y);
-        tris[(size_t)slot * 3 + 2] = make_float4(ac.z, n.x, n.y, n.z);
+        tris[slot * 3 + 0] = make_float4(a.x, a.y, a.z, ab.x);
+        tris[slot * 3 + 1] = make_float4(ab.y, ab.z, ac.x, ac.y);
+        tris[slot * 3 + 2] = make_float4(ac.z, n.x, n.y, n.z);
+        return n;
+    };
+    std::vector<float> rec_normals((size_t)n_tris * 3);
+    for (uint32_t slot = 0; slot < n_tris; ++slot) {
+        const uint32_t t = bvh.tri_order[slot];
+        const f3 n = put_tri_record(t, slot);
+        { const float4 stored = tris[(size_t)slot * 3 + 2]; rec_normals[(size_t)t * 3] = stored.y; rec_normals[(size_t)t * 3 + 1] = stored.z; rec_normals[(size_t)t * 3 + 2] = stored.w; }
         const float * n0 = s->normals + 3 * (size_t)s->idx_normals[3 * t + 0];
         const float * n1 = s->normals + 3 * (size_t)s->idx_normals[3 * t + 1];
         const float * n2 = s->normals + 3 * (size_t)s->idx_normals[3 * t + 2];
@@ -2322,7 +2339,8 @@
         tex_fill_srgb_lut(lut);
     }
     ctx->kat_textures = dev_tex;
-    std::vector<DevLight> lights(std::max(1u, s->light_count));
+    const uint32_t light_stride = std::max(1u, s->light_count);
+    std::vector<DevLight> lights(2 * (size_t)light_stride);
     memset(lights.data(), 0, lights.size() * sizeof(DevLight));
     for (uint32_t l = 0; l < s->light_count; ++l) {
         const prt_light & pl = s->lights[l];
@@ -2336,9 +2354,48 @@
     std::vector<float4> ddirs(1024);
     for (uint32_t i = 0; i < 1024; ++i) ddirs[i] = diffuse_tangent_dir(i);
 
-    std::vector<float4> nodes4(bvh.nodes.size() / 4);
-    memcpy(nodes4.data(), bvh.nodes.data(), bvh.nodes.size() * sizeof(uint32_t));
-    ctx->stack_bound = bvh.stack_bound;
+    std::vector<uint32_t> node_words(bvh.nodes);
+    uint32_t all_nodes = bvh.node_count, all_recs = n_rec;
+    unsigned int stack_bound = bvh.stack_bound;
+    std::vector<prt_shadow_tree_info> shadow_info(s->light_count, prt_shadow_tree_info());
+    const double shadow_origin_max = 32.0 * (double)abs_max;
+    uint32_t shadow_trees = 0;
+    for (uint32_t l = 0; l < s->light_count && abs_max > 0.0f; ++l) {
+        if (s->lights[l].type != 0 || shadow_trees >= (uint32_t)PRT_MAX_SHADOW_TREES) continue;
+        prt_shadow_tree_info & si = shadow_info[l];
+        const auto ts = std::chrono::steady_clock::now();
+        const float dir[3] = { lights[l].facing[0] * -1.0f, lights[l].facing[1] * -1.0f, lights[l].facing[2] * -1.0f };
+        ShadowTreeBuild sb;
+        sb.width = BVH_WIDTH; sb.leaf_max = leaf_max; sb.threads = std::min(hw, 16u); sb.trav_cost = trav_cost; sb.opt = &ctx->opt.bvh;
+        sb.ratio_percent = (uint32_t)std::max(0ll, std::min(100ll, ctx->opt.shadow_tree_ratio));
+        ShadowTreeResult sr;
+        std::vector<uint32_t> rec_tri;
+        BvhWide sub;
+        const char * bad = append_shadow_tree(sb, verts.data(), rec_normals.data(), n_tris, dir, shadow_origin_max, &node_words, all_nodes, all_recs, &rec_tri, &sr, &sub);
+        if (!bad && sr.built) bad = validate_bvh_links(sub, sr.triangle_count);
+        if (bad) { ctx->error = std::string("prt_upload_scene: the builder produced a broken shadow tree - ") + bad; return -9; }
+        si.triangle_count = sr.triangle_count;
+        si.build_ms = std::chrono::duration<double, std::milli>(std::chrono::steady_clock::now() - ts).count();
+        if (!sr.built) continue;
+        tris.resize(((size_t)all_recs + rec_tri.size()) * 3, make_float4(0, 0, 0, 0));
+        for (size_t i = 0; i < rec_tri.size(); ++i)
+            if (rec_tri[i] != 0xFFFFFFFFu) put_tri_record(rec_tri[i], (size_t)all_recs + i);
+        si.built = si.active = 1;
+        si.node_count = sr.node_count;
+        si.root = sr.root;
+        si.stack_bound = sr.stack_bound;
+        si.device_bytes = (uint64_t)sr.node_count * BVH_NODE_BYTES + (uint64_t)rec_tri.size() * 48u;
+        const int root = (int)sr.root;
+        memcpy(&lights[l].pad, &root, 4);
+        all_nodes += sr.node_count;
+        all_recs += (uint32_t)rec_tri.size();
+        stack_bound = std::max(stack_bound, sr.stack_bound);
+        shadow_trees++;
+    }
+    for (uint32_t l = 0; l < light_stride; ++l) { lights[light_stride + l] = lights[l]; lights[light_stride + l].pad = 0.0f; }
+
+    std::vector<float4> nodes4(node_words.size() / 4);
+    memcpy(nodes4.data(), node_words.data(), node_words.size() * sizeof(uint32_t));
 
     HIP_TRY(ctx, ctx->nodes.upload(nodes4));
     HIP_TRY(ctx, ctx->tris.upload(tris));
@@ -2382,6 +2439,12 @@
     if (rc) return rc;
 
     ctx->scene_abs_max = abs_max;
+    ctx->stack_bound = stack_bound;
+    ctx->shadow_info.swap(shadow_info);
+    ctx->shadow_bias_max = abs_max;
+    ctx->shadow_cam_max = 4.0f * abs_max;
+    ctx->light_stride = light_stride;
+    ctx->shadow_trees_fresh = true;
     prt_scene_info & info = ctx->info;
     info.triangle_count = n_tris;
     info.bvh_node_count = bvh.node_count;
@@ -2420,6 +2483,15 @@
     PRT_API_CATCH_RC(nullptr, "prt_get_scene_info")
 }
 
+int prt_get_shadow_trees(const prt_ctx * ctx, prt_shadow_tree_info * out, uint32_t cap) {
+    PRT_API_TRY
+    if (!ctx || (!out && cap)) return -1;
+    if (!ctx->has_scene) return -2;
+    for (size_t l = 0; l < ctx->shadow_info.size() && l < cap; ++l) out[l] = ctx->shadow_info[l];
+    return (int)ctx->shadow_info.size();
+    PRT_API_CATCH_RC(nullptr, "prt_get_shadow_trees")
+}
+
 int prt_render_device(prt_ctx * ctx, const prt_camera * cam, const prt_params * params, uint32_t width, uint32_t height,
                       uint32_t start_idx, uint32_t end_idx, void * d_rgba_out, prt_counters * counters) {
     PRT_API_TRY
@@ -2851,6 +2923,8 @@
     c->any_translucent = src->any_translucent; c->point_lights = src->point_lights; c->textured = src->textured;
     c->kat_textures = src->kat_textures;
     c->stack_bound = src->stack_bound;
+    c->light_stride = src->light_stride; c->shadow_info = src->shadow_info; c->shadow_trees_fresh = src->shadow_trees_fresh;
+    c->shadow_bias_max = src->shadow_bias_max; c->shadow_cam_max = src->shadow_cam_max;
     c->pool_park_cap = src->pool_park_cap; c->pool_spark_cap = src->pool_spark_cap;
     c->has_scene = src->has_scene;
     c->scene_epoch = 1;
@@ -3038,6 +3112,7 @@
             c->ref_spheres.borrow(src->ref_spheres);
             c->scene.ref_spheres = src->scene.ref_spheres;
             c->scene_abs_max = src->scene_abs_max;
+            c->shadow_trees_fresh = src->shadow_trees_fresh; c->shadow_info = src->shadow_info;
             c->info = src->info;
             c->has_scene = src->has_scene;
             c->tuned.clear();
diff --git a/par_raytracer_amd/csrc/prt_options.h b/par_raytracer_amd/csrc/prt_options.h
--- a/par_raytracer_amd/csrc/prt_options.h
+++ b/par_raytracer_amd/csrc/prt_options.h
@@ -23,6 +23,8 @@
     long long bvh_builder_lbvh = 0;
     long long pool_exact = 0;
     long long tie_widen_max = 8;
+    long long shadow_trees = 1;
+    long long shadow_tree_ratio = 75;
     long long debug_util = 0, debug_rounds = 0;
     long long chunk_min = -1, trace_blocks_per_cu = -1, keep_min = -1, node_min = -1, node_frac = -1, chains = -1, shade_block = -1;
     long long pool_blocks_per_cu = -1, pool_cap = -1, pool_topup = -1, pool_max_samples = -1, pool_park_cap = -1;
@@ -51,6 +53,7 @@
     static const OptEntry table[] = {
         { "TRACE_DEAD_SHADOW_RAYS", &PrtOptions::trace_dead_shadow_rays, nullptr }, { "POOL_EXACT", &PrtOptions::pool_exact, nullptr },
         { "TIE_WIDEN_MAX", &PrtOptions::tie_widen_max, nullptr },
+        { "SHADOW_TREES", &PrtOptions::shadow_trees, nullptr }, { "SHADOW_TREE_RATIO", &PrtOptions::shadow_tree_ratio, nullptr },
         { "DEBUG_UTIL", &PrtOptions::debug_util, nullptr }, { "DEBUG_ROUNDS", &PrtOptions::debug_rounds, nullptr },
         { "CHUNK_MIN", &PrtOptions::chunk_min, nullptr }, { "TRACE_BLOCKS_PER_CU", &PrtOptions::trace_blocks_per_cu, nullptr },
         { "KEEP_MIN", &PrtOptions::keep_min, nullptr }, { "NODE_MIN", &PrtOptions::node_min, nullptr }, { "NODE_FRAC", &PrtOptions::node_frac, nullptr },
```
